# KKKSQJ/DeepLearning

Measured on AMD Instinct MI355X. Metric: images/sec, higher is better.
Workload: dtype bf16; 1 GPU; model=resnet50, global_batch=256, image_size=224, parallelism=dp1

## Files before the change

### csrc/batchnorm.hip

```cpp
#include "common.h"
#include "vec.h"

namespace dla {

__device__ __forceinline__ float bn_pre(float x, float sc, float sh) {
  return fmaf(x, sc, sh);
}

template <typename dev_t>
__global__ void bn_stats_kernel(const dev_t* __restrict__ x, float* __restrict__ sums,
                                int N, int C, int64_t HW) {
  __shared__ float smem[16];
  const int c = blockIdx.x;
  const int64_t total = (int64_t)N * HW;
  float sum = 0.f, sumsq = 0.f;
  for (int64_t m = (int64_t)blockIdx.y * blockDim.x + threadIdx.x; m < total;
       m += (int64_t)gridDim.y * blockDim.x) {
    const int64_t n = m / HW, hw = m % HW;
    const float f = to_f32(x[(n * C + c) * HW + hw]);
    sum += f;
    sumsq += f * f;
  }
  sum = block_reduce_sum(sum, smem);
  sumsq = block_reduce_sum(sumsq, smem);
  if (threadIdx.x == 0) {
    atomicAdd(&sums[c], sum);
    atomicAdd(&sums[C + c], sumsq);
  }
}

__device__ __forceinline__ void bn_finalize_channel(
    int c, float sum, float sumsq, const float* __restrict__ weight,
    const float* __restrict__ bias, float* __restrict__ mean,
    float* __restrict__ rstd, float* __restrict__ running_mean,
    float* __restrict__ running_var, float* __restrict__ scale,
    float* __restrict__ shift, float count, float eps, float momentum) {
  const float mu = sum / count;
  const float var = fmaxf(sumsq / count - mu * mu, 0.f);
  const float rs = rsqrtf(var + eps);
  mean[c] = mu;
  rstd[c] = rs;
  if (running_mean != nullptr && momentum > 0.f) {
    const float unbiased = var * count / fmaxf(count - 1.f, 1.f);
    running_mean[c] = (1.f - momentum) * running_mean[c] + momentum * mu;
    running_var[c] = (1.f - momentum) * running_var[c] + momentum * unbiased;
  }
  const float sc = weight[c] * rs;
  scale[c] = sc;
  shift[c] = bias[c] - mu * sc;
}

__global__ void bn_finalize_kernel(const float* __restrict__ sums,
                                   const float* __restrict__ weight,
                                   const float* __restrict__ bias,
                                   float* __restrict__ mean, float* __restrict__ rstd,
                                   float* __restrict__ running_mean,
                                   float* __restrict__ running_var,
                                   float* __restrict__ scale, float* __restrict__ shift,
                                   int C, float count, float eps, float momentum) {
  const int c = blockIdx.x * blockDim.x + threadIdx.x;
  if (c >= C) return;
  bn_finalize_channel(c, sums[c], sums[C + c], weight, bias, mean, rstd,
                      running_mean, running_var, scale, shift, count, eps,
                      momentum);
}

constexpr int kFinCh = 16, kFinRows = 64;

__global__ void __launch_bounds__(kFinCh * kFinRows)
bn_finalize_parts_kernel(const float* __restrict__ parts, int n_parts,
                         const float* __restrict__ weight,
                         const float* __restrict__ bias,
                         float* __restrict__ mean, float* __restrict__ rstd,
                         float* __restrict__ running_mean,
                         float* __restrict__ running_var,
                         float* __restrict__ scale, float* __restrict__ shift,
                         int C, float count, float eps, float momentum) {
  __shared__ float ls[2][kFinRows][kFinCh + 1];
  const int cl = threadIdx.x % kFinCh, rl = threadIdx.x / kFinCh;
  const int c = blockIdx.x * kFinCh + cl;
  float s = 0.f, q = 0.f;
  if (c < C) {
#pragma unroll 4
    for (int r = rl; r < n_parts; r += kFinRows) {
      const float* p = parts + (int64_t)r * 2 * C;
      s += p[c];
      q += p[C + c];
    }
  }
  ls[0][rl][cl] = s;
  ls[1][rl][cl] = q;
  __syncthreads();
  for (int h = kFinRows / 2; h > 0; h >>= 1) {
    if (rl < h) {
      ls[0][rl][cl] += ls[0][rl + h][cl];
      ls[1][rl][cl] += ls[1][rl + h][cl];
    }
    __syncthreads();
  }
  if (rl == 0 && c < C)
    bn_finalize_channel(c, ls[0][0][cl], ls[1][0][cl], weight, bias, mean,
                        rstd, running_mean, running_var, scale, shift, count,
                        eps, momentum);
}

template <typename dev_t, int V, bool RELU>
__global__ void bn_apply_kernel(const dev_t* __restrict__ x,
                                const float* __restrict__ scale,
                                const float* __restrict__ shift,
                                dev_t* __restrict__ y, int C, int64_t HW,
                                int64_t n_total) {
  const int64_t stride = (int64_t)gridDim.x * blockDim.x * V;
  for (int64_t i = ((int64_t)blockIdx.x * blockDim.x + threadIdx.x) * V;
       i < n_total; i += stride) {
    const int c = (int)((i / HW) % C);
    const float sc = scale[c], sh = shift[c];
    Vec<dev_t, V> xv = vload<dev_t, V>(x + i);
    Vec<dev_t, V> yv;
#pragma unroll
    for (int j = 0; j < V; ++j) {
      const float f = bn_pre(to_f32(xv.v[j]), sc, sh);
      yv.v[j] = from_f32<dev_t>(RELU ? fmaxf(f, 0.f) : f);
    }
    vstore<dev_t, V>(y + i, yv);
  }
}

template <typename dev_t, bool RELU>
__global__ void bn_bwd_stats_kernel(const dev_t* __restrict__ dy,
                                    const dev_t* __restrict__ x,
                                    const dev_t* __restrict__ y,
                                    const float* __restrict__ mean,
                                    const float* __restrict__ rstd,
                                    float* __restrict__ sums,
                                    int N, int C, int64_t HW) {
  __shared__ float smem[16];
  const int c = blockIdx.x;
  const float mu = mean[c], rs = rstd[c];
  const int64_t total = (int64_t)N * HW;
  float s_dy = 0.f, s_dyxh = 0.f;
  for (int64_t m = (int64_t)blockIdx.y * blockDim.x + threadIdx.x; m < total;
       m += (int64_t)gridDim.y * blockDim.x) {
    const int64_t n = m / HW, hw = m % HW;
    const int64_t idx = (n * C + c) * HW + hw;
    float g = to_f32(dy[idx]);
    if (RELU && to_f32(y[idx]) <= 0.f) g = 0.f;
    const float xh = (to_f32(x[idx]) - mu) * rs;
    s_dy += g;
    s_dyxh += g * xh;
  }
  s_dy = block_reduce_sum(s_dy, smem);
  s_dyxh = block_reduce_sum(s_dyxh, smem);
  if (threadIdx.x == 0) {
    atomicAdd(&sums[c], s_dy);
    atomicAdd(&sums[C + c], s_dyxh);
  }
}

template <typename dev_t, bool RELU>
__global__ void bn_bwd_dx_kernel(const dev_t* __restrict__ dy,
                                 const dev_t* __restrict__ x,
                                 const dev_t* __restrict__ y,
                                 const float* __restrict__ mean,
                                 const float* __restrict__ rstd,
                                 const float* __restrict__ weight,
                                 const float* __restrict__ sums,
                                 dev_t* __restrict__ dx, int C, int64_t HW,
                                 int64_t n_total, float inv_count) {
  const int64_t stride = (int64_t)gridDim.x * blockDim.x;
  for (int64_t i = (int64_t)blockIdx.x * blockDim.x + threadIdx.x; i < n_total;
       i += stride) {
    const int c = (int)((i / HW) % C);
    const float mu = mean[c], rs = rstd[c];
    float g = to_f32(dy[i]);
    if (RELU && to_f32(y[i]) <= 0.f) g = 0.f;
    const float xh = (to_f32(x[i]) - mu) * rs;
    const float m_dy = sums[c] * inv_count;
    const float m_dyxh = sums[C + c] * inv_count;
    dx[i] = from_f32<dev_t>(weight[c] * rs * (g - m_dy - xh * m_dyxh));
  }
}



inline int64_t nhwc_used_threads(int lanes_per_row, int64_t rows,
                                 int64_t target_lanes) {
  int64_t k = target_lanes / lanes_per_row;
  if (k > rows) k = rows;
  if (k < 1) k = 1;
  return (int64_t)lanes_per_row * k;
}

constexpr int kRedThreads = 256;
constexpr int kRedLanes = 32;
constexpr int kRedBlocks = 2048;
constexpr int kRedMaxParts = 512;
constexpr int kRedMinRows = 8;
constexpr int red_unroll(int tensors) { return tensors <= 2 ? 4 : 2; }

#define DLA_RED_KERNEL \
  __launch_bounds__(dla::kRedThreads) __attribute__((amdgpu_waves_per_eu(1, 4)))

struct NhwcRedTile {
  int bl, rb, chunks, parts;
};

inline NhwcRedTile nhwc_red_tile(int lanes_per_row, int64_t rows,
                                 int blocks = kRedBlocks,
                                 int max_parts = kRedMaxParts) {
  NhwcRedTile t;
  t.chunks = (lanes_per_row + kRedLanes - 1) / kRedLanes;
  t.bl = (lanes_per_row + t.chunks - 1) / t.chunks;
  t.rb = kRedThreads / t.bl;
  const int64_t per_part = (int64_t)t.rb * kRedMinRows;
  const int64_t by_rows = (rows + per_part - 1) / per_part;
  const int64_t p = std::min<int64_t>(
      std::min<int64_t>(blocks / t.chunks, max_parts), by_rows);
  t.parts = (int)std::max<int64_t>(p, 1);
  return t;
}

struct NhwcRedPos {
  int c0;
  int64_t row;
  int64_t rstride;
  bool active;
};

template <int V>
__device__ __forceinline__ NhwcRedPos nhwc_red_pos(int C, int bl, int rb) {
  const int lane = threadIdx.x % bl, rl = threadIdx.x / bl;
  const int gl = blockIdx.x * bl + lane;
  NhwcRedPos p;
  p.c0 = gl * V;
  p.row = (int64_t)blockIdx.y * rb + rl;
  p.rstride = (int64_t)gridDim.y * rb;
  p.active = rl < rb && gl < C / V;
  return p;
}

template <int U, typename L, typename A>
__device__ __forceinline__ void nhwc_red_rows(const NhwcRedPos& p,
                                              int64_t rows, L&& load, A&& add) {
  if (!p.active) return;
  using D = decltype(load(int64_t{}));
  int64_t r = p.row;
  for (; r + (U - 1) * p.rstride < rows; r += U * p.rstride) {
    D d[U];
#pragma unroll
    for (int u = 0; u < U; ++u) d[u] = load(r + u * p.rstride);
#pragma unroll
    for (int u = 0; u < U; ++u) add(r + u * p.rstride, d[u]);
  }
  for (; r < rows; r += p.rstride) add(r, load(r));
}

template <int V, int NS>
__device__ __forceinline__ void nhwc_red_tail(const float (&acc)[NS][V],
                                              float* __restrict__ slab, int C,
                                              int bl, int rb) {
  __shared__ __attribute__((aligned(16))) float ls[kRedThreads * V];
  const int W = bl * V;
  const int cbase = blockIdx.x * W;
  float* out = slab + (int64_t)blockIdx.y * NS * C;
#pragma unroll
  for (int s = 0; s < NS; ++s) {
    if (s) __syncthreads();
    if ((int)threadIdx.x < bl * rb) {
#pragma unroll
      for (int j = 0; j < V; ++j) ls[threadIdx.x * V + j] = acc[s][j];
    }
    __syncthreads();
    for (int col = threadIdx.x; col < W; col += kRedThreads) {
      if (cbase + col < C) {
        float sum = 0.f;
        for (int r = 0; r < rb; ++r) sum += ls[r * W + col];
        out[s * C + cbase + col] = sum;
      }
    }
  }
}

constexpr int kSlabCols = 32, kSlabRows = 32;

__global__ void __launch_bounds__(kSlabCols * kSlabRows)
bn_slab_reduce_kernel(const float* __restrict__ slab, int n_parts, int n_cols,
                      float* __restrict__ sums) {
  __shared__ float ls[kSlabRows][kSlabCols + 1];
  const int cl = threadIdx.x % kSlabCols, rl = threadIdx.x / kSlabCols;
  const int c = blockIdx.x * kSlabCols + cl;
  float s = 0.f;
  if (c < n_cols) {
#pragma unroll 4
    for (int r = rl; r < n_parts; r += kSlabRows)
      s += slab[(int64_t)r * n_cols + c];
  }
  ls[rl][cl] = s;
  __syncthreads();
  for (int h = kSlabRows / 2; h > 0; h >>= 1) {
    if (rl < h) ls[rl][cl] += ls[rl + h][cl];
    __syncthreads();
  }
  if (rl == 0 && c < n_cols) sums[c] = ls[0][cl];
}

template <typename dev_t, int V>
__global__ void DLA_RED_KERNEL
bn_stats_nhwc_kernel(const dev_t* __restrict__ x, float* __restrict__ slab,
                     int C, int64_t rows, int bl, int rb) {
  const NhwcRedPos p = nhwc_red_pos<V>(C, bl, rb);
  float acc[2][V];
#pragma unroll
  for (int j = 0; j < V; ++j) { acc[0][j] = 0.f; acc[1][j] = 0.f; }
  nhwc_red_rows<red_unroll(1)>(
      p, rows, [&](int64_t r) { return vload<dev_t, V>(x + r * C + p.c0); },
      [&](int64_t, const Vec<dev_t, V>& xv) {
#pragma unroll
        for (int j = 0; j < V; ++j) {
          const float f = to_f32(xv.v[j]);
          acc[0][j] += f;
          acc[1][j] += f * f;
        }
      });
  nhwc_red_tail<V, 2>(acc, slab, C, bl, rb);
}

template <typename dev_t, int V, bool RELU>
__global__ void bn_apply_nhwc_kernel(const dev_t* __restrict__ x,
                                     const float* __restrict__ scale,
                                     const float* __restrict__ shift,
                                     dev_t* __restrict__ y, int C, int64_t rows,
                                     int64_t used) {
  const int64_t t = (int64_t)blockIdx.x * blockDim.x + threadIdx.x;
  if (t >= used) return;
  const int lanes_per_row = C / V;
  const int c0 = (int)(t % lanes_per_row) * V;
  const int64_t rstride = used / lanes_per_row;
  float sc[V], sh[V];
#pragma unroll
  for (int j = 0; j < V; ++j) { sc[j] = scale[c0 + j]; sh[j] = shift[c0 + j]; }
  for (int64_t r = t / lanes_per_row; r < rows; r += rstride) {
    Vec<dev_t, V> xv = vload<dev_t, V>(x + r * C + c0);
    Vec<dev_t, V> yv;
#pragma unroll
    for (int j = 0; j < V; ++j) {
      const float f = bn_pre(to_f32(xv.v[j]), sc[j], sh[j]);
      yv.v[j] = from_f32<dev_t>(RELU ? fmaxf(f, 0.f) : f);
    }
    vstore<dev_t, V>(y + r * C + c0, yv);
  }
}

template <typename dev_t, int V, bool RELU, bool MASK_Y = false>
__global__ void DLA_RED_KERNEL
bn_bwd_stats_nhwc_kernel(const dev_t* __restrict__ dy,
                         const dev_t* __restrict__ x,
                         const dev_t* __restrict__ y,
                         const float* __restrict__ scale,
                         const float* __restrict__ shift,
                         const float* __restrict__ mean,
                         const float* __restrict__ rstd,
                         float* __restrict__ slab, int C, int64_t rows, int bl,
                         int rb) {
  const NhwcRedPos p = nhwc_red_pos<V>(C, bl, rb);
  float mu[V], rs[V], sc[V], sh[V];
  float acc[2][V];
#pragma unroll
  for (int j = 0; j < V; ++j) {
    mu[j] = p.active ? mean[p.c0 + j] : 0.f;
    rs[j] = p.active ? rstd[p.c0 + j] : 0.f;
    sc[j] = (p.active && RELU && !MASK_Y) ? scale[p.c0 + j] : 0.f;
    sh[j] = (p.active && RELU && !MASK_Y) ? shift[p.c0 + j] : 0.f;
    acc[0][j] = 0.f;
    acc[1][j] = 0.f;
  }
  struct Row {
    Vec<dev_t, V> dy, x, y;
  };
  nhwc_red_rows<red_unroll(MASK_Y ? 3 : 2)>(
      p, rows,
      [&](int64_t r) {
        const int64_t base = r * C + p.c0;
        Row d;
        d.dy = vload<dev_t, V>(dy + base);
        d.x = vload<dev_t, V>(x + base);
        if (RELU && MASK_Y) d.y = vload<dev_t, V>(y + base);
        return d;
      },
      [&](int64_t, const Row& d) {
#pragma unroll
        for (int j = 0; j < V; ++j) {
          float g = to_f32(d.dy.v[j]);
          const float xf = to_f32(d.x.v[j]);
          if (RELU && MASK_Y && to_f32(d.y.v[j]) <= 0.f) g = 0.f;
          if (RELU && !MASK_Y && !(bn_pre(xf, sc[j], sh[j]) > 0.f)) g = 0.f;
          const float xh = (xf - mu[j]) * rs[j];
          acc[0][j] += g;
          acc[1][j] += g * xh;
        }
      });
  nhwc_red_tail<V, 2>(acc, slab, C, bl, rb);
}

template <typename dev_t, int V, bool RELU, bool MASK_Y = false>
__global__ void bn_bwd_dx_nhwc_kernel(const dev_t* __restrict__ dy,
                                      const dev_t* __restrict__ x,
                                      const dev_t* __restrict__ y,
                                      const float* __restrict__ scale,
                                      const float* __restrict__ shift,
                                      const float* __restrict__ mean,
                                      const float* __restrict__ rstd,
                                      const float* __restrict__ weight,
                                      const float* __restrict__ sums,
                                      dev_t* __restrict__ dx, int C,
                                      int64_t rows, int64_t used,
                                      float inv_count) {
  const int64_t t = (int64_t)blockIdx.x * blockDim.x + threadIdx.x;
  if (t >= used) return;
  const int lanes_per_row = C / V;
  const int c0 = (int)(t % lanes_per_row) * V;
  const int64_t rstride = used / lanes_per_row;
  float mu[V], rs[V], wr[V], sc[V], sh[V], m_dy[V], m_dyxh[V];
#pragma unroll
  for (int j = 0; j < V; ++j) {
    mu[j] = mean[c0 + j];
    rs[j] = rstd[c0 + j];
    wr[j] = weight[c0 + j] * rs[j];
    sc[j] = (RELU && !MASK_Y) ? scale[c0 + j] : 0.f;
    sh[j] = (RELU && !MASK_Y) ? shift[c0 + j] : 0.f;
    m_dy[j] = sums[c0 + j] * inv_count;
    m_dyxh[j] = sums[C + c0 + j] * inv_count;
  }
  for (int64_t r = t / lanes_per_row; r < rows; r += rstride) {
    const int64_t base = r * C + c0;
    Vec<dev_t, V> dyv = vload<dev_t, V>(dy + base);
    Vec<dev_t, V> xv = vload<dev_t, V>(x + base);
    Vec<dev_t, V> yv;
    if (RELU && MASK_Y) yv = vload<dev_t, V>(y + base);
    Vec<dev_t, V> dxv;
#pragma unroll
    for (int j = 0; j < V; ++j) {
      float g = to_f32(dyv.v[j]);
      const float xf = to_f32(xv.v[j]);
      if (RELU && MASK_Y && to_f32(yv.v[j]) <= 0.f) g = 0.f;
      if (RELU && !MASK_Y && !(bn_pre(xf, sc[j], sh[j]) > 0.f)) g = 0.f;
      const float xh = (xf - mu[j]) * rs[j];
      dxv.v[j] = from_f32<dev_t>(wr[j] * (g - m_dy[j] - xh * m_dyxh[j]));
    }
    vstore<dev_t, V>(dx + r * C + c0, dxv);
  }
}

template <typename dev_t, int V, bool DUAL>
__global__ void bn_add_relu_nhwc_kernel(const dev_t* __restrict__ x,
                                        const float* __restrict__ scale,
                                        const float* __restrict__ shift,
                                        const dev_t* __restrict__ idn,
                                        const float* __restrict__ scale_d,
                                        const float* __restrict__ shift_d,
                                        dev_t* __restrict__ out, int C,
                                        int64_t rows, int64_t used) {
  const int64_t t = (int64_t)blockIdx.x * blockDim.x + threadIdx.x;
  if (t >= used) return;
  const int lanes_per_row = C / V;
  const int c0 = (int)(t % lanes_per_row) * V;
  const int64_t rstride = used / lanes_per_row;
  float sc[V], sh[V], scd[V];
#pragma unroll
  for (int j = 0; j < V; ++j) {
    sc[j] = scale[c0 + j];
    sh[j] = shift[c0 + j];
    if (DUAL) {
      scd[j] = scale_d[c0 + j];
      sh[j] += shift_d[c0 + j];
    }
  }
  for (int64_t r = t / lanes_per_row; r < rows; r += rstride) {
    const int64_t base = r * C + c0;
    Vec<dev_t, V> xv = vload<dev_t, V>(x + base);
    Vec<dev_t, V> iv = vload<dev_t, V>(idn + base);
    Vec<dev_t, V> ov;
#pragma unroll
    for (int j = 0; j < V; ++j) {
      float f = to_f32(xv.v[j]) * sc[j] + sh[j];
      f += DUAL ? to_f32(iv.v[j]) * scd[j] : to_f32(iv.v[j]);
      ov.v[j] = from_f32<dev_t>(fmaxf(f, 0.f));
    }
    vstore<dev_t, V>(out + base, ov);
  }
}

template <typename dev_t, int V, bool DUAL>
__global__ void DLA_RED_KERNEL
bn_join_bwd_stats_nhwc_kernel(
    const dev_t* __restrict__ dy, const dev_t* __restrict__ out,
    const dev_t* __restrict__ x, const float* __restrict__ mean,
    const float* __restrict__ rstd, const dev_t* __restrict__ xd,
    const float* __restrict__ mean_d, const float* __restrict__ rstd_d,
    dev_t* __restrict__ g_out, float* __restrict__ slab, int C, int64_t rows,
    int bl, int rb) {
  constexpr int NS = DUAL ? 3 : 2;
  const NhwcRedPos p = nhwc_red_pos<V>(C, bl, rb);
  float mu[V], rs[V], mud[V], rsd[V];
  float acc[NS][V];
#pragma unroll
  for (int j = 0; j < V; ++j) {
    mu[j] = p.active ? mean[p.c0 + j] : 0.f;
    rs[j] = p.active ? rstd[p.c0 + j] : 0.f;
    mud[j] = (p.active && DUAL) ? mean_d[p.c0 + j] : 0.f;
    rsd[j] = (p.active && DUAL) ? rstd_d[p.c0 + j] : 0.f;
#pragma unroll
    for (int s = 0; s < NS; ++s) acc[s][j] = 0.f;
  }
  struct Row {
    Vec<dev_t, V> dy, out, x, xd;
  };
  nhwc_red_rows<red_unroll(DUAL ? 4 : 3)>(
      p, rows,
      [&](int64_t r) {
        const int64_t base = r * C + p.c0;
        Row d;
        d.dy = vload<dev_t, V>(dy + base);
        d.out = vload<dev_t, V>(out + base);
        d.x = vload<dev_t, V>(x + base);
        if (DUAL) d.xd = vload<dev_t, V>(xd + base);
        return d;
      },
      [&](int64_t r, const Row& d) {
        Vec<dev_t, V> gv;
#pragma unroll
        for (int j = 0; j < V; ++j) {
          const bool on = to_f32(d.out.v[j]) > 0.f;
          gv.v[j] = on ? d.dy.v[j] : from_f32<dev_t>(0.f);
          const float g = on ? to_f32(d.dy.v[j]) : 0.f;
          acc[0][j] += g;
          acc[1][j] += g * ((to_f32(d.x.v[j]) - mu[j]) * rs[j]);
          if (DUAL)
            acc[NS - 1][j] += g * ((to_f32(d.xd.v[j]) - mud[j]) * rsd[j]);
        }
        vstore<dev_t, V>(g_out + r * C + p.c0, gv);
      });
  nhwc_red_tail<V, NS>(acc, slab, C, bl, rb);
}

template <typename dev_t, int V>
__global__ void bn_join_bwd_dx_dual_nhwc_kernel(
    const dev_t* __restrict__ g, const dev_t* __restrict__ x,
    const dev_t* __restrict__ xd, const float* __restrict__ mean,
    const float* __restrict__ rstd, const float* __restrict__ weight,
    const float* __restrict__ mean_d, const float* __restrict__ rstd_d,
    const float* __restrict__ weight_d, const float* __restrict__ sums,
    dev_t* __restrict__ dx, dev_t* __restrict__ dxd, int C, int64_t rows,
    int64_t used, float inv_count) {
  const int64_t t = (int64_t)blockIdx.x * blockDim.x + threadIdx.x;
  if (t >= used) return;
  const int lanes_per_row = C / V;
  const int c0 = (int)(t % lanes_per_row) * V;
  const int64_t rstride = used / lanes_per_row;
  float mu[V], rs[V], wr[V], mud[V], rsd[V], wrd[V], m_g[V], m_gxh[V],
      m_gxhd[V];
#pragma unroll
  for (int j = 0; j < V; ++j) {
    mu[j] = mean[c0 + j];
    rs[j] = rstd[c0 + j];
    wr[j] = weight[c0 + j] * rs[j];
    mud[j] = mean_d[c0 + j];
    rsd[j] = rstd_d[c0 + j];
    wrd[j] = weight_d[c0 + j] * rsd[j];
    m_g[j] = sums[c0 + j] * inv_count;
    m_gxh[j] = sums[C + c0 + j] * inv_count;
    m_gxhd[j] = sums[2 * C + c0 + j] * inv_count;
  }
  for (int64_t r = t / lanes_per_row; r < rows; r += rstride) {
    const int64_t base = r * C + c0;
    Vec<dev_t, V> gv = vload<dev_t, V>(g + base);
    Vec<dev_t, V> xv = vload<dev_t, V>(x + base);
    Vec<dev_t, V> xdv = vload<dev_t, V>(xd + base);
    Vec<dev_t, V> dxv, dxdv;
#pragma unroll
    for (int j = 0; j < V; ++j) {
      const float gg = to_f32(gv.v[j]) - m_g[j];
      const float xh = (to_f32(xv.v[j]) - mu[j]) * rs[j];
      const float xhd = (to_f32(xdv.v[j]) - mud[j]) * rsd[j];
      dxv.v[j] = from_f32<dev_t>(wr[j] * (gg - xh * m_gxh[j]));
      dxdv.v[j] = from_f32<dev_t>(wrd[j] * (gg - xhd * m_gxhd[j]));
    }
    vstore<dev_t, V>(dx + base, dxv);
    vstore<dev_t, V>(dxd + base, dxdv);
  }
}

inline bool is_nhwc(const torch::Tensor& t) {
  return t.dim() == 4 && t.is_contiguous(at::MemoryFormat::ChannelsLast) &&
         !t.is_contiguous();
}

struct BnFinalized {
  torch::Tensor mean, rstd, scale, shift;
};

inline BnFinalized bn_finalize_launch(
    const torch::Tensor& sums, const torch::Tensor& weight,
    const torch::Tensor& bias, c10::optional<torch::Tensor>& running_mean,
    c10::optional<torch::Tensor>& running_var, int C, int64_t rows,
    double momentum, double eps) {
  TORCH_CHECK(sums.is_cuda() && sums.scalar_type() == torch::kFloat &&
                  sums.is_contiguous(),
              "bn sums must be a contiguous fp32 GPU tensor");
  TORCH_CHECK((sums.dim() == 1 && sums.size(0) == 2 * C) ||
                  (sums.dim() == 2 && sums.size(0) >= 1 &&
                   sums.size(1) == 2 * C),
              "bn sums must be [2C] or [n_parts, 2C]");
  TORCH_CHECK(weight.numel() == C && bias.numel() == C,
              "bn weight/bias must have C elements");
  auto opts_f = sums.options();
  BnFinalized f{torch::empty({C}, opts_f), torch::empty({C}, opts_f),
                torch::empty({C}, opts_f), torch::empty({C}, opts_f)};
  auto w32 = weight.to(torch::kFloat).contiguous();
  auto b32 = bias.to(torch::kFloat).contiguous();
  float* rm = running_mean.has_value() ? running_mean->data_ptr<float>() : nullptr;
  float* rv = running_var.has_value() ? running_var->data_ptr<float>() : nullptr;
  const int n_parts = sums.dim() == 2 ? (int)sums.size(0) : 1;
  if (n_parts > 1) {
    hipLaunchKernelGGL(bn_finalize_parts_kernel, dim3((C + kFinCh - 1) / kFinCh),
                       dim3(kFinCh * kFinRows), 0, stream(),
                       sums.data_ptr<float>(), n_parts, w32.data_ptr<float>(),
                       b32.data_ptr<float>(), f.mean.data_ptr<float>(),
                       f.rstd.data_ptr<float>(), rm, rv,
                       f.scale.data_ptr<float>(), f.shift.data_ptr<float>(), C,
                       (float)rows, (float)eps, (float)momentum);
  } else {
    hipLaunchKernelGGL(bn_finalize_kernel, dim3((C + 255) / 256), dim3(256), 0,
                       stream(), sums.data_ptr<float>(), w32.data_ptr<float>(),
                       b32.data_ptr<float>(), f.mean.data_ptr<float>(),
                       f.rstd.data_ptr<float>(), rm, rv,
                       f.scale.data_ptr<float>(), f.shift.data_ptr<float>(), C,
                       (float)rows, (float)eps, (float)momentum);
  }
  return f;
}

inline torch::Tensor bn_param_grad(const torch::Tensor& sums, int64_t offset,
                                   int C, const torch::Tensor& weight) {
  return sums.narrow(0, offset, C).to(weight.scalar_type());
}

inline torch::Tensor bn_slab_reduce_launch(const torch::Tensor& slab) {
  const int n_parts = (int)slab.size(0), n_cols = (int)slab.size(1);
  auto sums = torch::empty({n_cols}, slab.options());
  hipLaunchKernelGGL(bn_slab_reduce_kernel,
                     dim3((n_cols + kSlabCols - 1) / kSlabCols),
                     dim3(kSlabCols * kSlabRows), 0, stream(),
                     slab.data_ptr<float>(), n_parts, n_cols,
                     sums.data_ptr<float>());
  return sums;
}

inline bool is_nhwc_rows(const torch::Tensor& t) {
  return t.dim() == 4 && t.is_contiguous(at::MemoryFormat::ChannelsLast);
}

}

std::vector<torch::Tensor> batchnorm_fwd(torch::Tensor x, torch::Tensor weight,
                                         torch::Tensor bias,
                                         c10::optional<torch::Tensor> running_mean,
                                         c10::optional<torch::Tensor> running_var,
                                         double momentum, double eps, bool relu) {
  DLA_CHECK_CUDA(x);
  TORCH_CHECK(x.dim() == 4, "batchnorm_fwd expects a 4D tensor");
  const bool nhwc = dla::is_nhwc(x);
  TORCH_CHECK(nhwc || x.is_contiguous(), "batchnorm_fwd: x must be contiguous "
              "(NCHW or channels_last)");
  const int N = (int)x.size(0), C = (int)x.size(1);
  const int64_t HW = x.size(2) * x.size(3);
  auto opts_f = x.options().dtype(torch::kFloat);
  auto sums = nhwc ? torch::Tensor() : torch::zeros({2 * C}, opts_f);
  auto mean = torch::empty({C}, opts_f);
  auto rstd = torch::empty({C}, opts_f);
  auto scale = torch::empty({C}, opts_f);
  auto shift = torch::empty({C}, opts_f);
  auto y = torch::empty_like(x);
  auto w32 = weight.to(torch::kFloat);
  auto b32 = bias.to(torch::kFloat);

  const int64_t rows = (int64_t)N * HW;
  const int ysplit = (int)std::min<int64_t>((rows + 65535) / 65536 + 1,
                                            std::max(1, 2048 / C));
  DLA_DISPATCH_FLOAT_TYPES(x.scalar_type(), "batchnorm_fwd", [&] {
    if (nhwc) {
      constexpr int VM = 16 / (int)sizeof(dev_t);
      auto stats = [&](auto vtag) {
        constexpr int V = decltype(vtag)::value;
        const auto t = dla::nhwc_red_tile(C / V, rows);
        sums = torch::empty({t.parts, 2 * C}, opts_f);
        hipLaunchKernelGGL((dla::bn_stats_nhwc_kernel<dev_t, V>),
                           dim3(t.chunks, t.parts), dim3(dla::kRedThreads), 0,
                           dla::stream(), (const dev_t*)x.data_ptr(),
                           sums.data_ptr<float>(), C, rows, t.bl, t.rb);
      };
      if (C % VM == 0) stats(std::integral_constant<int, VM>{});
      else if (C % 2 == 0) stats(std::integral_constant<int, 2>{});
      else stats(std::integral_constant<int, 1>{});
    } else {
      hipLaunchKernelGGL((dla::bn_stats_kernel<dev_t>), dim3(C, ysplit), dim3(256), 0,
                         dla::stream(), (const dev_t*)x.data_ptr(),
                         sums.data_ptr<float>(), N, C, HW);
    }
    float* rm = running_mean.has_value() ? running_mean->data_ptr<float>() : nullptr;
    float* rv = running_var.has_value() ? running_var->data_ptr<float>() : nullptr;
    if (sums.dim() == 2 && sums.size(0) > 1) {
      hipLaunchKernelGGL(dla::bn_finalize_parts_kernel,
                         dim3((C + dla::kFinCh - 1) / dla::kFinCh),
                         dim3(dla::kFinCh * dla::kFinRows), 0, dla::stream(),
                         sums.data_ptr<float>(), (int)sums.size(0),
                         w32.data_ptr<float>(), b32.data_ptr<float>(),
                         mean.data_ptr<float>(), rstd.data_ptr<float>(), rm, rv,
                         scale.data_ptr<float>(), shift.data_ptr<float>(), C,
                         (float)rows, (float)eps, (float)momentum);
    } else {
      hipLaunchKernelGGL(dla::bn_finalize_kernel, dim3((C + 255) / 256), dim3(256), 0,
                         dla::stream(), sums.data_ptr<float>(), w32.data_ptr<float>(),
                         b32.data_ptr<float>(), mean.data_ptr<float>(),
                         rstd.data_ptr<float>(), rm, rv,
                         scale.data_ptr<float>(), shift.data_ptr<float>(), C,
                         (float)rows, (float)eps, (float)momentum);
    }
    const int64_t n_total = x.numel();
    constexpr int VMAX = 16 / (int)sizeof(dev_t);
    auto launch = [&](auto vtag, auto rtag) {
      constexpr int V = decltype(vtag)::value;
      constexpr bool R = decltype(rtag)::value;
      if (nhwc) {
        const int lanes = C / V;
        const int64_t used = dla::nhwc_used_threads(lanes, rows, 524288);
        hipLaunchKernelGGL((dla::bn_apply_nhwc_kernel<dev_t, V, R>),
                           dim3((int)((used + 255) / 256)), dim3(256), 0,
                           dla::stream(), (const dev_t*)x.data_ptr(),
                           scale.data_ptr<float>(), shift.data_ptr<float>(),
                           (dev_t*)y.data_ptr(), C, rows, used);
        return;
      }
      const int grid = dla::grid_1d((n_total + V - 1) / V, 256);
      if (false) ;
      else
        hipLaunchKernelGGL((dla::bn_apply_kernel<dev_t, V, R>), dim3(grid), dim3(256),
                           0, dla::stream(), (const dev_t*)x.data_ptr(),
                           scale.data_ptr<float>(), shift.data_ptr<float>(),
                           (dev_t*)y.data_ptr(), C, HW, n_total);
    };
    const bool vec_ok = nhwc ? (C % VMAX == 0) : (HW % VMAX == 0);
    if (vec_ok) {
      if (relu) launch(std::integral_constant<int, VMAX>{}, std::true_type{});
      else launch(std::integral_constant<int, VMAX>{}, std::false_type{});
    } else {
      if (relu) launch(std::integral_constant<int, 1>{}, std::true_type{});
      else launch(std::integral_constant<int, 1>{}, std::false_type{});
    }
  });
  HIP_CHECK_ERR();
  return {y, mean, rstd, scale, shift};
}

std::vector<torch::Tensor> batchnorm_fwd_from_sums(
    torch::Tensor x, torch::Tensor weight, torch::Tensor bias,
    torch::Tensor sums, c10::optional<torch::Tensor> running_mean,
    c10::optional<torch::Tensor> running_var, double momentum, double eps,
    bool relu) {
  DLA_CHECK_CUDA(x);
  TORCH_CHECK(x.dim() == 4, "batchnorm_fwd_from_sums expects a 4D tensor");
  const bool nhwc = dla::is_nhwc(x);
  TORCH_CHECK(nhwc || x.is_contiguous(),
              "batchnorm_fwd_from_sums: x must be contiguous");
  const int N = (int)x.size(0), C = (int)x.size(1);
  const int64_t HW = x.size(2) * x.size(3);
  auto y = torch::empty_like(x);
  const int64_t rows = (int64_t)N * HW;
  auto fin = dla::bn_finalize_launch(sums, weight, bias, running_mean,
                                     running_var, C, rows, momentum, eps);
  auto& mean = fin.mean;
  auto& rstd = fin.rstd;
  auto& scale = fin.scale;
  auto& shift = fin.shift;
  DLA_DISPATCH_FLOAT_TYPES(x.scalar_type(), "batchnorm_fwd_from_sums", [&] {
    const int64_t n_total = x.numel();
    constexpr int VMAX = 16 / (int)sizeof(dev_t);
    auto launch = [&](auto vtag, auto rtag) {
      constexpr int V = decltype(vtag)::value;
      constexpr bool R = decltype(rtag)::value;
      if (nhwc) {
        const int lanes = C / V;
        const int64_t used = dla::nhwc_used_threads(lanes, rows, 524288);
        hipLaunchKernelGGL((dla::bn_apply_nhwc_kernel<dev_t, V, R>),
                           dim3((int)((used + 255) / 256)), dim3(256), 0,
                           dla::stream(), (const dev_t*)x.data_ptr(),
                           scale.data_ptr<float>(), shift.data_ptr<float>(),
                           (dev_t*)y.data_ptr(), C, rows, used);
        return;
      }
      const int grid = dla::grid_1d((n_total + V - 1) / V, 256);
      hipLaunchKernelGGL((dla::bn_apply_kernel<dev_t, V, R>), dim3(grid),
                         dim3(256), 0, dla::stream(),
                         (const dev_t*)x.data_ptr(), scale.data_ptr<float>(),
                         shift.data_ptr<float>(), (dev_t*)y.data_ptr(), C, HW,
                         n_total);
    };
    const bool vec_ok = nhwc ? (C % VMAX == 0) : (HW % VMAX == 0);
    if (vec_ok) {
      if (relu) launch(std::integral_constant<int, VMAX>{}, std::true_type{});
      else launch(std::integral_constant<int, VMAX>{}, std::false_type{});
    } else {
      if (relu) launch(std::integral_constant<int, 1>{}, std::true_type{});
      else launch(std::integral_constant<int, 1>{}, std::false_type{});
    }
  });
  HIP_CHECK_ERR();
  return {y, mean, rstd, scale, shift};
}

torch::Tensor bn_apply(torch::Tensor x, torch::Tensor scale, torch::Tensor shift,
                       bool relu) {
  DLA_CHECK_CUDA(x);
  TORCH_CHECK(x.dim() == 4, "bn_apply expects a 4D tensor");
  const bool nhwc = dla::is_nhwc(x);
  TORCH_CHECK(nhwc || x.is_contiguous(), "bn_apply: x must be contiguous");
  const int C = (int)x.size(1);
  const int64_t HW = x.size(2) * x.size(3);
  auto y = torch::empty_like(x);
  auto sc = scale.to(torch::kFloat).contiguous();
  auto sh = shift.to(torch::kFloat).contiguous();
  const int64_t n_total = x.numel();
  DLA_DISPATCH_FLOAT_TYPES(x.scalar_type(), "bn_apply", [&] {
    constexpr int VMAX = 16 / (int)sizeof(dev_t);
    auto launch = [&](auto vtag, auto rtag) {
      constexpr int V = decltype(vtag)::value;
      constexpr bool R = decltype(rtag)::value;
      if (nhwc) {
        const int64_t rows = n_total / C;
        const int lanes = C / V;
        const int64_t used = dla::nhwc_used_threads(lanes, rows, 524288);
        hipLaunchKernelGGL((dla::bn_apply_nhwc_kernel<dev_t, V, R>),
                           dim3((int)((used + 255) / 256)), dim3(256), 0,
                           dla::stream(), (const dev_t*)x.data_ptr(),
                           sc.data_ptr<float>(), sh.data_ptr<float>(),
                           (dev_t*)y.data_ptr(), C, rows, used);
        return;
      }
      const int grid = dla::grid_1d((n_total + V - 1) / V, 256);
      if (false) ;
      else
        hipLaunchKernelGGL((dla::bn_apply_kernel<dev_t, V, R>), dim3(grid), dim3(256),
                           0, dla::stream(), (const dev_t*)x.data_ptr(),
                           sc.data_ptr<float>(), sh.data_ptr<float>(),
                           (dev_t*)y.data_ptr(), C, HW, n_total);
    };
    const bool vec_ok = nhwc ? (C % VMAX == 0) : (HW % VMAX == 0);
    if (vec_ok) {
      if (relu) launch(std::integral_constant<int, VMAX>{}, std::true_type{});
      else launch(std::integral_constant<int, VMAX>{}, std::false_type{});
    } else {
      if (relu) launch(std::integral_constant<int, 1>{}, std::true_type{});
      else launch(std::integral_constant<int, 1>{}, std::false_type{});
    }
  });
  HIP_CHECK_ERR();
  return y;
}

bool bn_relu_mask_from_x(torch::Tensor x) { return dla::is_nhwc(x); }

std::vector<torch::Tensor> batchnorm_bwd_ex(
    torch::Tensor dy, torch::Tensor x, c10::optional<torch::Tensor> y,
    torch::Tensor weight, torch::Tensor mean, torch::Tensor rstd,
    c10::optional<torch::Tensor> scale, c10::optional<torch::Tensor> shift,
    bool relu) {
  DLA_CHECK_CUDA(dy); DLA_CHECK_CUDA(x);
  const bool nhwc = dla::is_nhwc(x);
  TORCH_CHECK(nhwc || x.is_contiguous(), "batchnorm_bwd: x must be contiguous");
  if (nhwc && !dla::is_nhwc(dy)) dy = dy.contiguous(at::MemoryFormat::ChannelsLast);
  if (!nhwc) dy = dy.contiguous();
  const int N = (int)x.size(0), C = (int)x.size(1);
  const int64_t HW = x.size(2) * x.size(3);
  const int64_t rows = (int64_t)N * HW;
  auto opts_f = x.options().dtype(torch::kFloat);
  auto sums = nhwc ? torch::Tensor() : torch::zeros({2 * C}, opts_f);
  auto dx = torch::empty_like(x);
  auto w32 = weight.to(torch::kFloat);
  const int ysplit = (int)std::min<int64_t>((rows + 65535) / 65536 + 1,
                                            std::max(1, 2048 / C));
  const bool mask_y = relu && y.has_value();
  if (relu && !mask_y) {
    TORCH_CHECK(bn_relu_mask_from_x(x) && scale.has_value() && shift.has_value(),
                "batchnorm_bwd: the relu mask needs y, or channels_last x "
                "with the forward's scale and shift");
    for (const auto* t : {&*scale, &*shift})
      TORCH_CHECK(t->is_cuda() && t->scalar_type() == torch::kFloat &&
                      t->is_contiguous() && t->numel() == C,
                  "batchnorm_bwd: scale/shift must be contiguous fp32 [C]");
  }
  if (mask_y)
    TORCH_CHECK(y->scalar_type() == x.scalar_type() && y->sizes() == x.sizes() &&
                    (nhwc ? dla::is_nhwc(*y) : y->is_contiguous()),
                "batchnorm_bwd: y must match x (shape, dtype, layout)");
  const float* scp = (relu && !mask_y) ? scale->data_ptr<float>() : nullptr;
  const float* shp = (relu && !mask_y) ? shift->data_ptr<float>() : nullptr;
  DLA_DISPATCH_FLOAT_TYPES(x.scalar_type(), "batchnorm_bwd", [&] {
    const dev_t* yp = mask_y ? (const dev_t*)y->data_ptr() : nullptr;
    auto with_mode = [&](auto f) {
      if (!relu) f(std::false_type{}, std::false_type{});
      else if (mask_y) f(std::true_type{}, std::true_type{});
      else f(std::true_type{}, std::false_type{});
    };
    with_mode([&](auto rtag, auto mtag) {
      constexpr bool R = decltype(rtag)::value;
      constexpr bool MY = decltype(mtag)::value;
      if (nhwc) {
        constexpr int VM = 16 / (int)sizeof(dev_t);
        auto stats = [&](auto vtag) {
          constexpr int V = decltype(vtag)::value;
          const auto t = dla::nhwc_red_tile(C / V, rows);
          auto slab = torch::empty({t.parts, 2 * C}, opts_f);
          hipLaunchKernelGGL((dla::bn_bwd_stats_nhwc_kernel<dev_t, V, R, MY>),
                             dim3(t.chunks, t.parts), dim3(dla::kRedThreads),
                             0, dla::stream(), (const dev_t*)dy.data_ptr(),
                             (const dev_t*)x.data_ptr(), yp, scp, shp,
                             mean.data_ptr<float>(), rstd.data_ptr<float>(),
                             slab.data_ptr<float>(), C, rows, t.bl, t.rb);
          sums = dla::bn_slab_reduce_launch(slab);
        };
        if (C % VM == 0) stats(std::integral_constant<int, VM>{});
        else if (C % 2 == 0) stats(std::integral_constant<int, 2>{});
        else stats(std::integral_constant<int, 1>{});
      } else if constexpr (!R || MY) {
        hipLaunchKernelGGL((dla::bn_bwd_stats_kernel<dev_t, R>), dim3(C, ysplit),
                           dim3(256), 0, dla::stream(), (const dev_t*)dy.data_ptr(),
                           (const dev_t*)x.data_ptr(), yp, mean.data_ptr<float>(),
                           rstd.data_ptr<float>(), sums.data_ptr<float>(), N, C, HW);
      }
    });

    const int64_t n_total = x.numel();
    const float inv_count = 1.f / (float)rows;
    constexpr int VMAX = 16 / (int)sizeof(dev_t);
    with_mode([&](auto rtag, auto mtag) {
      constexpr bool R = decltype(rtag)::value;
      constexpr bool MY = decltype(mtag)::value;
      if (nhwc) {
        auto dxk = [&](auto vtag) {
          constexpr int V = decltype(vtag)::value;
          const int lanes = C / V;
          const int64_t used = dla::nhwc_used_threads(lanes, rows, 524288);
          hipLaunchKernelGGL((dla::bn_bwd_dx_nhwc_kernel<dev_t, V, R, MY>),
                             dim3((int)((used + 255) / 256)), dim3(256), 0,
                             dla::stream(), (const dev_t*)dy.data_ptr(),
                             (const dev_t*)x.data_ptr(), yp, scp, shp,
                             mean.data_ptr<float>(), rstd.data_ptr<float>(),
                             w32.data_ptr<float>(), sums.data_ptr<float>(),
                             (dev_t*)dx.data_ptr(), C, rows, used, inv_count);
        };
        if (C % VMAX == 0) dxk(std::integral_constant<int, VMAX>{});
        else dxk(std::integral_constant<int, 1>{});
      } else if constexpr (!R || MY) {
        hipLaunchKernelGGL((dla::bn_bwd_dx_kernel<dev_t, R>), dim3(dla::grid_1d(n_total, 256)),
                           dim3(256), 0, dla::stream(), (const dev_t*)dy.data_ptr(),
                           (const dev_t*)x.data_ptr(), yp, mean.data_ptr<float>(),
                           rstd.data_ptr<float>(), w32.data_ptr<float>(),
                           sums.data_ptr<float>(), (dev_t*)dx.data_ptr(), C, HW,
                           n_total, inv_count);
      }
    });
  });
  HIP_CHECK_ERR();
  return {dx, dla::bn_param_grad(sums, C, C, weight),
          dla::bn_param_grad(sums, 0, C, weight)};
}

std::vector<torch::Tensor> batchnorm_bwd(torch::Tensor dy, torch::Tensor x,
                                         c10::optional<torch::Tensor> y,
                                         torch::Tensor weight, torch::Tensor mean,
                                         torch::Tensor rstd, bool relu) {
  TORCH_CHECK(!relu || y.has_value(), "batchnorm_bwd: relu mask needs y");
  return batchnorm_bwd_ex(dy, x, relu ? y : c10::nullopt, weight, mean, rstd,
                          c10::nullopt, c10::nullopt, relu);
}

namespace dla {

inline void join_check(const torch::Tensor& x, const torch::Tensor& other,
                       const char* what) {
  TORCH_CHECK(other.is_cuda() && other.scalar_type() == x.scalar_type() &&
                  other.sizes() == x.sizes() && is_nhwc_rows(other),
              "bn join: ", what, " must match x (shape, dtype, channels_last)");
}

inline int join_vec(const torch::Tensor& x) {
  const int vmax = 16 / (int)x.element_size();
  TORCH_CHECK(x.size(1) % vmax == 0,
              "bn join: C must be a multiple of ", vmax);
  return vmax;
}

}

std::vector<torch::Tensor> bn_add_relu_fwd_from_sums(
    torch::Tensor x, torch::Tensor weight, torch::Tensor bias,
    torch::Tensor sums, c10::optional<torch::Tensor> running_mean,
    c10::optional<torch::Tensor> running_var, double momentum, double eps,
    torch::Tensor identity) {
  DLA_CHECK_CUDA(x);
  TORCH_CHECK(dla::is_nhwc_rows(x), "bn_add_relu: x must be channels_last");
  dla::join_check(x, identity, "identity");
  dla::join_vec(x);
  const int C = (int)x.size(1);
  const int64_t rows = x.numel() / C;
  auto fin = dla::bn_finalize_launch(sums, weight, bias, running_mean,
                                     running_var, C, rows, momentum, eps);
  auto out = torch::empty_like(x);
  DLA_DISPATCH_FLOAT_TYPES(x.scalar_type(), "bn_add_relu_fwd_from_sums", [&] {
    constexpr int V = 16 / (int)sizeof(dev_t);
    const int64_t used = dla::nhwc_used_threads(C / V, rows, 524288);
    hipLaunchKernelGGL((dla::bn_add_relu_nhwc_kernel<dev_t, V, false>),
                       dim3((int)((used + 255) / 256)), dim3(256), 0,
                       dla::stream(), (const dev_t*)x.data_ptr(),
                       fin.scale.data_ptr<float>(), fin.shift.data_ptr<float>(),
                       (const dev_t*)identity.data_ptr(), nullptr, nullptr,
                       (dev_t*)out.data_ptr(), C, rows, used);
  });
  HIP_CHECK_ERR();
  return {out, fin.mean, fin.rstd};
}

std::vector<torch::Tensor> bn_add_relu_dual_fwd_from_sums(
    torch::Tensor x, torch::Tensor weight, torch::Tensor bias,
    torch::Tensor sums, c10::optional<torch::Tensor> running_mean,
    c10::optional<torch::Tensor> running_var, double momentum, double eps,
    torch::Tensor xd, torch::Tensor weight_d, torch::Tensor bias_d,
    torch::Tensor sums_d, c10::optional<torch::Tensor> running_mean_d,
    c10::optional<torch::Tensor> running_var_d, double momentum_d,
    double eps_d) {
  DLA_CHECK_CUDA(x);
  TORCH_CHECK(dla::is_nhwc_rows(x), "bn_add_relu_dual: x must be channels_last");
  dla::join_check(x, xd, "xd");
  dla::join_vec(x);
  const int C = (int)x.size(1);
  const int64_t rows = x.numel() / C;
  auto fin = dla::bn_finalize_launch(sums, weight, bias, running_mean,
                                     running_var, C, rows, momentum, eps);
  auto fd = dla::bn_finalize_launch(sums_d, weight_d, bias_d, running_mean_d,
                                    running_var_d, C, rows, momentum_d, eps_d);
  auto out = torch::empty_like(x);
  DLA_DISPATCH_FLOAT_TYPES(x.scalar_type(), "bn_add_relu_dual_fwd_from_sums", [&] {
    constexpr int V = 16 / (int)sizeof(dev_t);
    const int64_t used = dla::nhwc_used_threads(C / V, rows, 524288);
    hipLaunchKernelGGL((dla::bn_add_relu_nhwc_kernel<dev_t, V, true>),
                       dim3((int)((used + 255) / 256)), dim3(256), 0,
                       dla::stream(), (const dev_t*)x.data_ptr(),
                       fin.scale.data_ptr<float>(), fin.shift.data_ptr<float>(),
                       (const dev_t*)xd.data_ptr(), fd.scale.data_ptr<float>(),
                       fd.shift.data_ptr<float>(), (dev_t*)out.data_ptr(), C,
                       rows, used);
  });
  HIP_CHECK_ERR();
  return {out, fin.mean, fin.rstd, fd.mean, fd.rstd};
}

std::vector<torch::Tensor> bn_add_relu_bwd(torch::Tensor dy, torch::Tensor out,
                                           torch::Tensor x, torch::Tensor weight,
                                           torch::Tensor mean,
                                           torch::Tensor rstd) {
  DLA_CHECK_CUDA(x);
  TORCH_CHECK(dla::is_nhwc_rows(x), "bn_add_relu_bwd: x must be channels_last");
  dla::join_check(x, out, "out");
  if (!dla::is_nhwc_rows(dy)) dy = dy.contiguous(at::MemoryFormat::ChannelsLast);
  dla::join_check(x, dy, "dy");
  dla::join_vec(x);
  const int C = (int)x.size(1);
  const int64_t rows = x.numel() / C;
  TORCH_CHECK(mean.numel() == C && rstd.numel() == C && weight.numel() == C,
              "bn_add_relu_bwd: per-channel tensors must have C elements");
  torch::Tensor sums;
  auto g = torch::empty_like(x);
  auto dx = torch::empty_like(x);
  auto w32 = weight.to(torch::kFloat).contiguous();
  DLA_DISPATCH_FLOAT_TYPES(x.scalar_type(), "bn_add_relu_bwd", [&] {
    constexpr int V = 16 / (int)sizeof(dev_t);
    const int lanes = C / V;
    const auto t = dla::nhwc_red_tile(lanes, rows);
    auto slab = torch::empty({t.parts, 2 * C},
                             x.options().dtype(torch::kFloat));
    hipLaunchKernelGGL((dla::bn_join_bwd_stats_nhwc_kernel<dev_t, V, false>),
                       dim3(t.chunks, t.parts), dim3(dla::kRedThreads), 0,
                       dla::stream(),
                       (const dev_t*)dy.data_ptr(), (const dev_t*)out.data_ptr(),
                       (const dev_t*)x.data_ptr(), mean.data_ptr<float>(),
                       rstd.data_ptr<float>(), nullptr, nullptr, nullptr,
                       (dev_t*)g.data_ptr(), slab.data_ptr<float>(), C, rows,
                       t.bl, t.rb);
    sums = dla::bn_slab_reduce_launch(slab);
    const int64_t used = dla::nhwc_used_threads(lanes, rows, 524288);
    hipLaunchKernelGGL((dla::bn_bwd_dx_nhwc_kernel<dev_t, V, false>),
                       dim3((int)((used + 255) / 256)), dim3(256), 0,
                       dla::stream(), (const dev_t*)g.data_ptr(),
                       (const dev_t*)x.data_ptr(), nullptr, nullptr, nullptr,
                       mean.data_ptr<float>(), rstd.data_ptr<float>(),
                       w32.data_ptr<float>(), sums.data_ptr<float>(),
                       (dev_t*)dx.data_ptr(), C, rows, used,
                       1.f / (float)rows);
  });
  HIP_CHECK_ERR();
  return {g, dx, dla::bn_param_grad(sums, C, C, weight),
          dla::bn_param_grad(sums, 0, C, weight)};
}

std::vector<torch::Tensor> bn_add_relu_dual_bwd(
    torch::Tensor dy, torch::Tensor out, torch::Tensor x, torch::Tensor weight,
    torch::Tensor mean, torch::Tensor rstd, torch::Tensor xd,
    torch::Tensor weight_d, torch::Tensor mean_d, torch::Tensor rstd_d) {
  DLA_CHECK_CUDA(x);
  TORCH_CHECK(dla::is_nhwc_rows(x), "bn_add_relu_dual_bwd: x must be channels_last");
  dla::join_check(x, out, "out");
  dla::join_check(x, xd, "xd");
  if (!dla::is_nhwc_rows(dy)) dy = dy.contiguous(at::MemoryFormat::ChannelsLast);
  dla::join_check(x, dy, "dy");
  dla::join_vec(x);
  const int C = (int)x.size(1);
  const int64_t rows = x.numel() / C;
  TORCH_CHECK(mean.numel() == C && rstd.numel() == C && weight.numel() == C &&
                  mean_d.numel() == C && rstd_d.numel() == C &&
                  weight_d.numel() == C,
              "bn_add_relu_dual_bwd: per-channel tensors must have C elements");
  torch::Tensor sums;
  auto g = torch::empty_like(x);
  auto dx = torch::empty_like(x);
  auto dxd = torch::empty_like(x);
  auto w32 = weight.to(torch::kFloat).contiguous();
  auto wd32 = weight_d.to(torch::kFloat).contiguous();
  DLA_DISPATCH_FLOAT_TYPES(x.scalar_type(), "bn_add_relu_dual_bwd", [&] {
    constexpr int V = 16 / (int)sizeof(dev_t);
    const int lanes = C / V;
    const auto t = dla::nhwc_red_tile(lanes, rows);
    auto slab = torch::empty({t.parts, 3 * C},
                             x.options().dtype(torch::kFloat));
    hipLaunchKernelGGL((dla::bn_join_bwd_stats_nhwc_kernel<dev_t, V, true>),
                       dim3(t.chunks, t.parts), dim3(dla::kRedThreads), 0,
                       dla::stream(),
                       (const dev_t*)dy.data_ptr(), (const dev_t*)out.data_ptr(),
                       (const dev_t*)x.data_ptr(), mean.data_ptr<float>(),
                       rstd.data_ptr<float>(), (const dev_t*)xd.data_ptr(),
                       mean_d.data_ptr<float>(), rstd_d.data_ptr<float>(),
                       (dev_t*)g.data_ptr(), slab.data_ptr<float>(), C, rows,
                       t.bl, t.rb);
    sums = dla::bn_slab_reduce_launch(slab);
    const int64_t used = dla::nhwc_used_threads(lanes, rows, 524288);
    hipLaunchKernelGGL((dla::bn_join_bwd_dx_dual_nhwc_kernel<dev_t, V>),
                       dim3((int)((used + 255) / 256)), dim3(256), 0,
                       dla::stream(), (const dev_t*)g.data_ptr(),
                       (const dev_t*)x.data_ptr(), (const dev_t*)xd.data_ptr(),
                       mean.data_ptr<float>(), rstd.data_ptr<float>(),
                       w32.data_ptr<float>(), mean_d.data_ptr<float>(),
                       rstd_d.data_ptr<float>(), wd32.data_ptr<float>(),
                       sums.data_ptr<float>(), (dev_t*)dx.data_ptr(),
                       (dev_t*)dxd.data_ptr(), C, rows, used,
                       1.f / (float)rows);
  });
  HIP_CHECK_ERR();
  auto dbias = dla::bn_param_grad(sums, 0, C, weight);
  return {dx, dxd, dla::bn_param_grad(sums, C, C, weight), dbias,
          dla::bn_param_grad(sums, 2 * C, C, weight_d),
          dbias.to(weight_d.scalar_type()).clone()};
}

namespace dla {

constexpr int kPoolRun = 8;

template <typename dev_t, int V>
__global__ void __launch_bounds__(256)
bn_relu_maxpool_fwd_nhwc_kernel(const dev_t* __restrict__ x,
                                const float* __restrict__ scale,
                                const float* __restrict__ shift,
                                dev_t* __restrict__ out,
                                uint8_t* __restrict__ slots, int C, int H,
                                int W, int OH, int OW, int runs_per_img) {
  const int n = blockIdx.x / runs_per_img;
  const int oh0 = (blockIdx.x % runs_per_img) * kPoolRun;
  const int oh1 = min(oh0 + kPoolRun, OH);
  const int lanes = C / V;
  const int items = (oh1 - oh0) * OW * lanes;
  const dev_t* xn = x + (int64_t)n * H * W * C;
  const int64_t obase = ((int64_t)n * OH + oh0) * OW * C;
  for (int i = threadIdx.x; i < items; i += blockDim.x) {
    const int c0 = (i % lanes) * V;
    const int p = i / lanes;
    const int ow = p % OW, oh = oh0 + p / OW;
    float sc[V], sh[V], best[V];
    int slot[V];
#pragma unroll
    for (int j = 0; j < V; ++j) {
      sc[j] = scale[c0 + j];
      sh[j] = shift[c0 + j];
      best[j] = -INFINITY;
      slot[j] = 4;
    }
#pragma unroll
    for (int kh = 0; kh < 3; ++kh) {
      const int ih = 2 * oh - 1 + kh;
      if (ih < 0 || ih >= H) continue;
#pragma unroll
      for (int kw = 0; kw < 3; ++kw) {
        const int iw = 2 * ow - 1 + kw;
        if (iw < 0 || iw >= W) continue;
        Vec<dev_t, V> xv =
            vload<dev_t, V>(xn + ((int64_t)ih * W + iw) * C + c0);
#pragma unroll
        for (int j = 0; j < V; ++j) {
          const float f = bn_pre(to_f32(xv.v[j]), sc[j], sh[j]);
          const float y = to_f32(from_f32<dev_t>(fmaxf(f, 0.f)));
          if (y > best[j]) {
            best[j] = y;
            slot[j] = kh * 3 + kw;
          }
        }
      }
    }
    Vec<dev_t, V> ov;
    Vec<uint8_t, V> sv;
#pragma unroll
    for (int j = 0; j < V; ++j) {
      ov.v[j] = from_f32<dev_t>(best[j]);
      sv.v[j] = (uint8_t)slot[j];
    }
    const int64_t o = obase + (int64_t)p * C + c0;
    vstore<dev_t, V>(out + o, ov);
    vstore<uint8_t, V>(slots + o, sv);
  }
}

template <typename dev_t, int V>
__device__ __forceinline__ void stem_pool_grad(
    const dev_t* __restrict__ dpool, const uint8_t* __restrict__ slots,
    const Vec<dev_t, V>& xv, const float* sc, const float* sh, int n, int h,
    int w, int c0, int C, int OH, int OW, float* g) {
#pragma unroll
  for (int j = 0; j < V; ++j) g[j] = 0.f;
  const int oh_hi = min((h + 1) >> 1, OH - 1);
  const int ow_hi = min((w + 1) >> 1, OW - 1);
  for (int oh = h >> 1; oh <= oh_hi; ++oh) {
    const int kh = h - 2 * oh + 1;
    for (int ow = w >> 1; ow <= ow_hi; ++ow) {
      const int want = kh * 3 + (w - 2 * ow + 1);
      const int64_t o = (((int64_t)n * OH + oh) * OW + ow) * C + c0;
      Vec<uint8_t, V> sv = vload<uint8_t, V>(slots + o);
      Vec<dev_t, V> dv = vload<dev_t, V>(dpool + o);
#pragma unroll
      for (int j = 0; j < V; ++j)
        if ((int)sv.v[j] == want) g[j] += to_f32(dv.v[j]);
    }
  }
#pragma unroll
  for (int j = 0; j < V; ++j)
    if (!(bn_pre(to_f32(xv.v[j]), sc[j], sh[j]) > 0.f)) g[j] = 0.f;
}

constexpr int kStemRedBlocks = 1024;

template <typename dev_t, int V>
__global__ void __launch_bounds__(kRedThreads)
bn_relu_maxpool_bwd_stats_nhwc_kernel(
    const dev_t* __restrict__ dpool, const uint8_t* __restrict__ slots,
    const dev_t* __restrict__ x, const float* __restrict__ scale,
    const float* __restrict__ shift, const float* __restrict__ mean,
    const float* __restrict__ rstd, float* __restrict__ slab, int C, int H,
    int W, int OH, int OW, int64_t rows, int bl, int rb) {
  const NhwcRedPos p = nhwc_red_pos<V>(C, bl, rb);
  float mu[V], rs[V], sc[V], sh[V];
  float acc[2][V];
#pragma unroll
  for (int j = 0; j < V; ++j) {
    mu[j] = p.active ? mean[p.c0 + j] : 0.f;
    rs[j] = p.active ? rstd[p.c0 + j] : 0.f;
    sc[j] = p.active ? scale[p.c0 + j] : 0.f;
    sh[j] = p.active ? shift[p.c0 + j] : 0.f;
    acc[0][j] = 0.f;
    acc[1][j] = 0.f;
  }
  nhwc_red_rows<1>(
      p, rows, [&](int64_t r) { return vload<dev_t, V>(x + r * C + p.c0); },
      [&](int64_t r, const Vec<dev_t, V>& xv) {
        const uint32_t r32 = (uint32_t)r;
        const uint32_t q = r32 / (uint32_t)W;
        const int w = (int)(r32 - q * (uint32_t)W);
        const int n = (int)(q / (uint32_t)H);
        const int h = (int)(q - (uint32_t)n * (uint32_t)H);
        float g[V];
        stem_pool_grad<dev_t, V>(dpool, slots, xv, sc, sh, n, h, w, p.c0, C,
                                 OH, OW, g);
#pragma unroll
        for (int j = 0; j < V; ++j) {
          const float xh = (to_f32(xv.v[j]) - mu[j]) * rs[j];
          acc[0][j] += g[j];
          acc[1][j] += g[j] * xh;
        }
      });
  nhwc_red_tail<V, 2>(acc, slab, C, bl, rb);
}

template <typename dev_t, int V>
__global__ void bn_relu_maxpool_bwd_dx_nhwc_kernel(
    const dev_t* __restrict__ dpool, const uint8_t* __restrict__ slots,
    const dev_t* __restrict__ x, const float* __restrict__ scale,
    const float* __restrict__ shift, const float* __restrict__ mean,
    const float* __restrict__ rstd, const float* __restrict__ weight,
    const float* __restrict__ sums, dev_t* __restrict__ dx, int C, int H,
    int W, int OH, int OW, int64_t rows, int64_t used, float inv_count) {
  const int64_t t = (int64_t)blockIdx.x * blockDim.x + threadIdx.x;
  if (t >= used) return;
  const int lanes_per_row = C / V;
  const int c0 = (int)(t % lanes_per_row) * V;
  const int64_t rstride = used / lanes_per_row;
  float mu[V], rs[V], wr[V], sc[V], sh[V], m_g[V], m_gxh[V], g[V];
#pragma unroll
  for (int j = 0; j < V; ++j) {
    mu[j] = mean[c0 + j];
    rs[j] = rstd[c0 + j];
    wr[j] = weight[c0 + j] * rs[j];
    sc[j] = scale[c0 + j];
    sh[j] = shift[c0 + j];
    m_g[j] = sums[c0 + j] * inv_count;
    m_gxh[j] = sums[C + c0 + j] * inv_count;
  }
  for (int64_t r = t / lanes_per_row; r < rows; r += rstride) {
    const uint32_t r32 = (uint32_t)r;
    const uint32_t q = r32 / (uint32_t)W;
    const int w = (int)(r32 - q * (uint32_t)W);
    const int n = (int)(q / (uint32_t)H);
    const int h = (int)(q - (uint32_t)n * (uint32_t)H);
    Vec<dev_t, V> xv = vload<dev_t, V>(x + r * C + c0);
    stem_pool_grad<dev_t, V>(dpool, slots, xv, sc, sh, n, h, w, c0, C, OH, OW,
                             g);
    Vec<dev_t, V> dxv;
#pragma unroll
    for (int j = 0; j < V; ++j) {
      const float xh = (to_f32(xv.v[j]) - mu[j]) * rs[j];
      dxv.v[j] = from_f32<dev_t>(wr[j] * (g[j] - m_g[j] - xh * m_gxh[j]));
    }
    vstore<dev_t, V>(dx + r * C + c0, dxv);
  }
}

inline void stem_check(const torch::Tensor& x, const char* fn) {
  TORCH_CHECK(x.is_cuda() && x.dim() == 4 && is_nhwc_rows(x), fn,
              ": x must be a channels_last 4D GPU tensor");
  const int vmax = 16 / (int)x.element_size();
  TORCH_CHECK(x.size(1) % vmax == 0, fn, ": C must be a multiple of ", vmax);
  TORCH_CHECK(x.numel() > 0 && x.numel() / x.size(1) < (int64_t(1) << 31),
              fn, ": N*H*W must be in [1, 2^31)");
}

}

std::vector<torch::Tensor> bn_relu_maxpool_fwd(
    torch::Tensor x, torch::Tensor weight, torch::Tensor bias,
    c10::optional<torch::Tensor> running_mean,
    c10::optional<torch::Tensor> running_var, double momentum, double eps) {
  dla::stem_check(x, "bn_relu_maxpool_fwd");
  const int N = (int)x.size(0), C = (int)x.size(1);
  const int H = (int)x.size(2), W = (int)x.size(3);
  const int OH = (H - 1) / 2 + 1, OW = (W - 1) / 2 + 1;
  const int64_t rows = (int64_t)N * H * W;
  auto out_opts = x.options().memory_format(at::MemoryFormat::ChannelsLast);
  auto pooled = torch::empty({N, C, OH, OW}, out_opts);
  auto slots = torch::empty({N, C, OH, OW}, out_opts.dtype(torch::kByte));
  const int runs = (OH + dla::kPoolRun - 1) / dla::kPoolRun;
  TORCH_CHECK((int64_t)N * runs < (int64_t(1) << 31),
              "bn_relu_maxpool_fwd: too many blocks");
  dla::BnFinalized fin;
  DLA_DISPATCH_FLOAT_TYPES(x.scalar_type(), "bn_relu_maxpool_fwd", [&] {
    constexpr int V = 16 / (int)sizeof(dev_t);
    const auto t = dla::nhwc_red_tile(C / V, rows);
    auto sums = torch::empty({t.parts, 2 * C},
                             x.options().dtype(torch::kFloat));
    hipLaunchKernelGGL((dla::bn_stats_nhwc_kernel<dev_t, V>),
                       dim3(t.chunks, t.parts), dim3(dla::kRedThreads), 0,
                       dla::stream(), (const dev_t*)x.data_ptr(),
                       sums.data_ptr<float>(), C, rows, t.bl, t.rb);
    fin = dla::bn_finalize_launch(sums, weight, bias, running_mean,
                                  running_var, C, rows, momentum, eps);
    hipLaunchKernelGGL((dla::bn_relu_maxpool_fwd_nhwc_kernel<dev_t, V>),
                       dim3(N * runs), dim3(256), 0, dla::stream(),
                       (const dev_t*)x.data_ptr(), fin.scale.data_ptr<float>(),
                       fin.shift.data_ptr<float>(), (dev_t*)pooled.data_ptr(),
                       slots.data_ptr<uint8_t>(), C, H, W, OH, OW, runs);
  });
  HIP_CHECK_ERR();
  return {pooled, slots, fin.mean, fin.rstd, fin.scale, fin.shift};
}

std::vector<torch::Tensor> bn_relu_maxpool_bwd(
    torch::Tensor dpool, torch::Tensor x, torch::Tensor slots,
    torch::Tensor weight, torch::Tensor mean, torch::Tensor rstd,
    torch::Tensor scale, torch::Tensor shift) {
  dla::stem_check(x, "bn_relu_maxpool_bwd");
  const int N = (int)x.size(0), C = (int)x.size(1);
  const int H = (int)x.size(2), W = (int)x.size(3);
  const int OH = (H - 1) / 2 + 1, OW = (W - 1) / 2 + 1;
  const int64_t rows = (int64_t)N * H * W;
  DLA_CHECK_CUDA(dpool);
  if (!dla::is_nhwc_rows(dpool))
    dpool = dpool.contiguous(at::MemoryFormat::ChannelsLast);
  const std::vector<int64_t> pshape{N, C, OH, OW};
  TORCH_CHECK(dpool.scalar_type() == x.scalar_type() &&
                  dpool.sizes() == at::IntArrayRef(pshape),
              "bn_relu_maxpool_bwd: dpool must be [N, C, OH, OW] of x's dtype");
  TORCH_CHECK(slots.is_cuda() && slots.scalar_type() == torch::kByte &&
                  slots.sizes() == at::IntArrayRef(pshape) &&
                  dla::is_nhwc_rows(slots),
              "bn_relu_maxpool_bwd: slots must be channels_last uint8 "
              "[N, C, OH, OW]");
  for (const auto* t : {&mean, &rstd, &scale, &shift})
    TORCH_CHECK(t->is_cuda() && t->scalar_type() == torch::kFloat &&
                    t->is_contiguous() && t->numel() == C,
                "bn_relu_maxpool_bwd: per-channel tensors must be contiguous "
                "fp32 [C]");
  TORCH_CHECK(weight.numel() == C, "bn_relu_maxpool_bwd: weight must be [C]");
  torch::Tensor sums;
  auto dx = torch::empty_like(x);
  auto w32 = weight.to(torch::kFloat).contiguous();
  DLA_DISPATCH_FLOAT_TYPES(x.scalar_type(), "bn_relu_maxpool_bwd", [&] {
    constexpr int V = 16 / (int)sizeof(dev_t);
    const int lanes = C / V;
    const auto t = dla::nhwc_red_tile(lanes, rows, dla::kStemRedBlocks,
                                      dla::kStemRedBlocks);
    auto slab = torch::empty({t.parts, 2 * C},
                             x.options().dtype(torch::kFloat));
    hipLaunchKernelGGL((dla::bn_relu_maxpool_bwd_stats_nhwc_kernel<dev_t, V>),
                       dim3(t.chunks, t.parts), dim3(dla::kRedThreads), 0,
                       dla::stream(), (const dev_t*)dpool.data_ptr(),
                       slots.data_ptr<uint8_t>(), (const dev_t*)x.data_ptr(),
                       scale.data_ptr<float>(), shift.data_ptr<float>(),
                       mean.data_ptr<float>(), rstd.data_ptr<float>(),
                       slab.data_ptr<float>(), C, H, W, OH, OW, rows, t.bl,
                       t.rb);
    sums = dla::bn_slab_reduce_launch(slab);
    const int64_t used = dla::nhwc_used_threads(lanes, rows, 524288);
    hipLaunchKernelGGL((dla::bn_relu_maxpool_bwd_dx_nhwc_kernel<dev_t, V>),
                       dim3((int)((used + 255) / 256)), dim3(256), 0,
                       dla::stream(), (const dev_t*)dpool.data_ptr(),
                       slots.data_ptr<uint8_t>(), (const dev_t*)x.data_ptr(),
                       scale.data_ptr<float>(), shift.data_ptr<float>(),
                       mean.data_ptr<float>(), rstd.data_ptr<float>(),
                       w32.data_ptr<float>(), sums.data_ptr<float>(),
                       (dev_t*)dx.data_ptr(), C, H, W, OH, OW, rows, used,
                       1.f / (float)rows);
  });
  HIP_CHECK_ERR();
  return {dx, dla::bn_param_grad(sums, C, C, weight),
          dla::bn_param_grad(sums, 0, C, weight)};
}
```

### csrc/bindings.cpp

```cpp
#include <torch/extension.h>

std::vector<torch::Tensor> layernorm_fwd(torch::Tensor x, torch::Tensor w,
                                         torch::Tensor b, double eps);
std::vector<torch::Tensor> layernorm_bwd(torch::Tensor dy, torch::Tensor x,
                                         torch::Tensor w, torch::Tensor mean,
                                         torch::Tensor rstd);
torch::Tensor gelu_fwd(torch::Tensor x);
torch::Tensor gelu_bwd(torch::Tensor dy, torch::Tensor x);
torch::Tensor silu_fwd(torch::Tensor x);
torch::Tensor silu_bwd(torch::Tensor dy, torch::Tensor x);
torch::Tensor add_relu_fwd(torch::Tensor a, torch::Tensor b);
torch::Tensor relu_mask_bwd(torch::Tensor dy, torch::Tensor y);
std::vector<torch::Tensor> batchnorm_fwd(torch::Tensor x, torch::Tensor weight,
                                         torch::Tensor bias,
                                         c10::optional<torch::Tensor> running_mean,
                                         c10::optional<torch::Tensor> running_var,
                                         double momentum, double eps, bool relu);
torch::Tensor bn_apply(torch::Tensor x, torch::Tensor scale, torch::Tensor shift,
                       bool relu);
std::vector<torch::Tensor> batchnorm_bwd(torch::Tensor dy, torch::Tensor x,
                                         c10::optional<torch::Tensor> y,
                                         torch::Tensor weight, torch::Tensor mean,
                                         torch::Tensor rstd, bool relu);
bool bn_relu_mask_from_x(torch::Tensor x);
std::vector<torch::Tensor> batchnorm_bwd_ex(
    torch::Tensor dy, torch::Tensor x, c10::optional<torch::Tensor> y,
    torch::Tensor weight, torch::Tensor mean, torch::Tensor rstd,
    c10::optional<torch::Tensor> scale, c10::optional<torch::Tensor> shift,
    bool relu);
std::vector<torch::Tensor> bn_relu_maxpool_fwd(
    torch::Tensor x, torch::Tensor weight, torch::Tensor bias,
    c10::optional<torch::Tensor> running_mean,
    c10::optional<torch::Tensor> running_var, double momentum, double eps);
std::vector<torch::Tensor> bn_relu_maxpool_bwd(
    torch::Tensor dpool, torch::Tensor x, torch::Tensor slots,
    torch::Tensor weight, torch::Tensor mean, torch::Tensor rstd,
    torch::Tensor scale, torch::Tensor shift);
std::vector<torch::Tensor> batchnorm_fwd_from_sums(
    torch::Tensor x, torch::Tensor weight, torch::Tensor bias,
    torch::Tensor sums, c10::optional<torch::Tensor> running_mean,
    c10::optional<torch::Tensor> running_var, double momentum, double eps,
    bool relu);
std::vector<torch::Tensor> bn_add_relu_fwd_from_sums(
    torch::Tensor x, torch::Tensor weight, torch::Tensor bias,
    torch::Tensor sums, c10::optional<torch::Tensor> running_mean,
    c10::optional<torch::Tensor> running_var, double momentum, double eps,
    torch::Tensor identity);
std::vector<torch::Tensor> bn_add_relu_dual_fwd_from_sums(
    torch::Tensor x, torch::Tensor weight, torch::Tensor bias,
    torch::Tensor sums, c10::optional<torch::Tensor> running_mean,
    c10::optional<torch::Tensor> running_var, double momentum, double eps,
    torch::Tensor xd, torch::Tensor weight_d, torch::Tensor bias_d,
    torch::Tensor sums_d, c10::optional<torch::Tensor> running_mean_d,
    c10::optional<torch::Tensor> running_var_d, double momentum_d,
    double eps_d);
std::vector<torch::Tensor> bn_add_relu_bwd(torch::Tensor dy, torch::Tensor out,
                                           torch::Tensor x, torch::Tensor weight,
                                           torch::Tensor mean,
                                           torch::Tensor rstd);
std::vector<torch::Tensor> bn_add_relu_dual_bwd(
    torch::Tensor dy, torch::Tensor out, torch::Tensor x, torch::Tensor weight,
    torch::Tensor mean, torch::Tensor rstd, torch::Tensor xd,
    torch::Tensor weight_d, torch::Tensor mean_d, torch::Tensor rstd_d);
std::vector<torch::Tensor> conv1x1_fwd(torch::Tensor a, torch::Tensor b,
                                       c10::optional<torch::Tensor> bias,
                                       c10::optional<torch::Tensor> scale,
                                       c10::optional<torch::Tensor> shift,
                                       c10::optional<torch::Tensor> residual,
                                       bool relu, bool want_stats);
torch::Tensor conv1x1_wgrad(torch::Tensor dy, torch::Tensor x);
std::vector<torch::Tensor> conv3x3_fwd(torch::Tensor a, torch::Tensor w9,
                                       int64_t imgH, int64_t imgW,
                                       c10::optional<torch::Tensor> bias,
                                       c10::optional<torch::Tensor> scale,
                                       c10::optional<torch::Tensor> shift,
                                       c10::optional<torch::Tensor> residual,
                                       bool relu, bool want_stats);
torch::Tensor conv3x3_wgrad(torch::Tensor dy, torch::Tensor x, int64_t imgH,
                            int64_t imgW);
torch::Tensor dwconv_fwd(torch::Tensor x, torch::Tensor weight,
                         c10::optional<torch::Tensor> bias, int64_t stride);
torch::Tensor dwconv_dgrad(torch::Tensor dy, torch::Tensor weight, int64_t H,
                           int64_t W, int64_t stride);
std::vector<torch::Tensor> dwconv_wgrad(torch::Tensor dy, torch::Tensor x,
                                        int64_t K, int64_t stride,
                                        bool out_f32);
torch::Tensor transpose2d(torch::Tensor src);
torch::Tensor stride2_gather(torch::Tensor x);
torch::Tensor stride2_scatter(torch::Tensor dy, int64_t IH, int64_t IW);
std::vector<torch::Tensor> softmax_ce_fwd(torch::Tensor logits,
                                          c10::optional<torch::Tensor> target,
                                          c10::optional<torch::Tensor> soft_target,
                                          double smoothing, int64_t ignore_index);
torch::Tensor softmax_ce_bwd(torch::Tensor logits,
                             c10::optional<torch::Tensor> target,
                             c10::optional<torch::Tensor> soft_target,
                             torch::Tensor lse, double smoothing,
                             int64_t ignore_index, torch::Tensor grad_out,
                             torch::Tensor stats);
torch::Tensor focal_loss_fwd(torch::Tensor logits, torch::Tensor targets,
                             double alpha, double gamma);
torch::Tensor focal_loss_bwd(torch::Tensor dloss, torch::Tensor logits,
                             torch::Tensor targets, double alpha, double gamma);
torch::Tensor box_iou_gpu(torch::Tensor a, torch::Tensor b, bool giou);
torch::Tensor nms_gpu(torch::Tensor boxes_sorted, double iou_threshold);
torch::Tensor roialign_fwd(torch::Tensor input, torch::Tensor rois, int64_t PH,
                           int64_t PW, double spatial_scale,
                           int64_t sampling_ratio, bool aligned);
torch::Tensor roialign_bwd(torch::Tensor grad_out, torch::Tensor rois, int64_t N,
                           int64_t C, int64_t H, int64_t W, double spatial_scale,
                           int64_t sampling_ratio, bool aligned);
std::vector<torch::Tensor> attn_fwd(torch::Tensor qkv, int64_t num_heads,
                                    double scale,
                                    c10::optional<torch::Tensor> bias,
                                    c10::optional<torch::Tensor> mask,
                                    bool save_p, bool save_stats);
std::vector<torch::Tensor> attn_bwd(torch::Tensor qkv, torch::Tensor dout,
                                    torch::Tensor stats, torch::Tensor drow,
                                    int64_t num_heads, double scale);
std::vector<torch::Tensor> attn_fwd_cosine(torch::Tensor qkv, int64_t num_heads,
                              torch::Tensor logit_scale,
                              c10::optional<torch::Tensor> bias,
                              c10::optional<torch::Tensor> mask, bool save_p);
torch::Tensor mfma_probe(torch::Tensor A, torch::Tensor B);
torch::Tensor my_add(torch::Tensor a, torch::Tensor b);
std::vector<torch::Tensor> cocoeval_match_image(
    torch::Tensor det_boxes, torch::Tensor det_scores, torch::Tensor gt_boxes,
    torch::Tensor gt_crowd, torch::Tensor iou_thrs, int64_t max_dets,
    c10::optional<torch::Tensor> gt_extra_ignore);
torch::Tensor window_partition_fwd(torch::Tensor x, int64_t ws, int64_t shift);
torch::Tensor window_partition_bwd(torch::Tensor grad, int64_t B, int64_t H,
                                   int64_t W, int64_t ws, int64_t shift);
torch::Tensor window_merge_fwd(torch::Tensor windows, int64_t B, int64_t H,
                               int64_t W, int64_t ws, int64_t shift);
torch::Tensor window_merge_bwd(torch::Tensor grad, int64_t ws, int64_t shift);

PYBIND11_MODULE(TORCH_EXTENSION_NAME, m) {
  m.doc() = "deeplearning_amd gfx950 HIP kernels";
  m.def("layernorm_fwd", &layernorm_fwd);
  m.def("layernorm_bwd", &layernorm_bwd);
  m.def("gelu_fwd", &gelu_fwd);
  m.def("gelu_bwd", &gelu_bwd);
  m.def("silu_fwd", &silu_fwd);
  m.def("silu_bwd", &silu_bwd);
  m.def("add_relu_fwd", &add_relu_fwd);
  m.def("relu_mask_bwd", &relu_mask_bwd);
  m.def("batchnorm_fwd", &batchnorm_fwd);
  m.def("batchnorm_fwd_from_sums", &batchnorm_fwd_from_sums);
  m.def("bn_apply", &bn_apply);
  m.def("batchnorm_bwd", &batchnorm_bwd);
  m.def("batchnorm_bwd_ex", &batchnorm_bwd_ex);
  m.def("bn_relu_mask_from_x", &bn_relu_mask_from_x);
  m.def("bn_relu_maxpool_fwd", &bn_relu_maxpool_fwd);
  m.def("bn_relu_maxpool_bwd", &bn_relu_maxpool_bwd);
  m.def("bn_add_relu_fwd_from_sums", &bn_add_relu_fwd_from_sums);
  m.def("bn_add_relu_dual_fwd_from_sums", &bn_add_relu_dual_fwd_from_sums);
  m.def("bn_add_relu_bwd", &bn_add_relu_bwd);
  m.def("bn_add_relu_dual_bwd", &bn_add_relu_dual_bwd);
  m.def("conv1x1_fwd", &conv1x1_fwd, py::arg("a"), py::arg("b"),
        py::arg("bias") = py::none(), py::arg("scale") = py::none(),
        py::arg("shift") = py::none(), py::arg("residual") = py::none(),
        py::arg("relu") = false, py::arg("want_stats") = false);
  m.def("conv1x1_wgrad", &conv1x1_wgrad);
  m.def("conv3x3_fwd", &conv3x3_fwd, py::arg("a"), py::arg("w9"),
        py::arg("imgH"), py::arg("imgW"), py::arg("bias") = py::none(),
        py::arg("scale") = py::none(), py::arg("shift") = py::none(),
        py::arg("residual") = py::none(), py::arg("relu") = false,
        py::arg("want_stats") = false);
  m.def("conv3x3_wgrad", &conv3x3_wgrad);
  m.def("dwconv_fwd", &dwconv_fwd, py::arg("x"), py::arg("weight"),
        py::arg("bias") = py::none(), py::arg("stride") = 1);
  m.def("dwconv_dgrad", &dwconv_dgrad);
  m.def("dwconv_wgrad", &dwconv_wgrad);
  m.def("transpose2d", &transpose2d);
  m.def("stride2_gather", &stride2_gather);
  m.def("stride2_scatter", &stride2_scatter);
  m.def("softmax_ce_fwd", &softmax_ce_fwd);
  m.def("softmax_ce_bwd", &softmax_ce_bwd);
  m.def("focal_loss_fwd", &focal_loss_fwd);
  m.def("focal_loss_bwd", &focal_loss_bwd);
  m.def("box_iou", &box_iou_gpu);
  m.def("nms", &nms_gpu);
  m.def("roialign_fwd", &roialign_fwd);
  m.def("roialign_bwd", &roialign_bwd);
  m.def("attn_fwd", &attn_fwd, py::arg("qkv"), py::arg("num_heads"),
        py::arg("scale"), py::arg("bias") = py::none(),
        py::arg("mask") = py::none(), py::arg("save_p") = false,
        py::arg("save_stats") = false);
  m.def("attn_bwd", &attn_bwd);
  m.def("attn_fwd_cosine", &attn_fwd_cosine, py::arg("qkv"),
        py::arg("num_heads"), py::arg("logit_scale"),
        py::arg("bias") = py::none(), py::arg("mask") = py::none(),
        py::arg("save_p") = false);
  m.def("mfma_probe", &mfma_probe);
  m.def("cocoeval_match_image", &cocoeval_match_image, py::arg("det_boxes"),
        py::arg("det_scores"), py::arg("gt_boxes"), py::arg("gt_crowd"),
        py::arg("iou_thrs"), py::arg("max_dets"),
        py::arg("gt_extra_ignore") = py::none());
  m.def("my_add", &my_add);
  m.def("window_partition_fwd", &window_partition_fwd);
  m.def("window_partition_bwd", &window_partition_bwd);
  m.def("window_merge_fwd", &window_merge_fwd);
  m.def("window_merge_bwd", &window_merge_bwd);
}
```

### csrc/common.h

```cpp
#pragma once

#include <hip/hip_runtime.h>
#include <hip/hip_bf16.h>
#include <hip/hip_fp16.h>
#include <torch/extension.h>
#include <ATen/hip/HIPContext.h>

#define DLA_WAVE 64
#define DLA_CHECK_CUDA(x) TORCH_CHECK((x).is_cuda(), #x " must be a GPU tensor")
#define DLA_CHECK_CONTIG(x) TORCH_CHECK((x).is_contiguous(), #x " must be contiguous")
#define DLA_CHECK_INPUT(x) DLA_CHECK_CUDA(x); DLA_CHECK_CONTIG(x)
#define DLA_CHECK_DENSE(x)                                                     \
  DLA_CHECK_CUDA(x);                                                           \
  TORCH_CHECK((x).is_contiguous() ||                                           \
                  ((x).dim() == 4 &&                                           \
                   (x).is_contiguous(at::MemoryFormat::ChannelsLast)),         \
              #x " must be dense (contiguous or channels_last)")

#define HIP_CHECK_ERR()                                                        \
  do {                                                                         \
    hipError_t e = hipGetLastError();                                          \
    TORCH_CHECK(e == hipSuccess, "HIP kernel launch failed: ",                 \
                hipGetErrorString(e));                                         \
  } while (0)

namespace dla {

constexpr int kMaxGrid = 2048;

inline int grid_1d(int64_t n, int block) {
  int64_t g = (n + block - 1) / block;
  return (int)std::min<int64_t>(g, kMaxGrid);
}

inline hipStream_t stream() { return at::hip::getCurrentHIPStream().stream(); }

template <typename T> struct AccT { using type = float; };

__device__ __forceinline__ float to_f32(float x) { return x; }
__device__ __forceinline__ float to_f32(__hip_bfloat16 x) { return __bfloat162float(x); }
__device__ __forceinline__ float to_f32(__half x) { return __half2float(x); }

template <typename T> __device__ __forceinline__ T from_f32(float x);
template <> __device__ __forceinline__ float from_f32<float>(float x) { return x; }
template <> __device__ __forceinline__ __hip_bfloat16 from_f32<__hip_bfloat16>(float x) {
  return __float2bfloat16(x);
}
template <> __device__ __forceinline__ __half from_f32<__half>(float x) {
  return __float2half(x);
}

template <typename scalar_t> struct DevT { using type = scalar_t; };
template <> struct DevT<at::BFloat16> { using type = __hip_bfloat16; };
template <> struct DevT<at::Half> { using type = __half; };

__device__ __forceinline__ float wave_reduce_sum(float v) {
#pragma unroll
  for (int off = 32; off > 0; off >>= 1) v += __shfl_xor(v, off, 64);
  return v;
}

__device__ __forceinline__ float wave_reduce_max(float v) {
#pragma unroll
  for (int off = 32; off > 0; off >>= 1) v = fmaxf(v, __shfl_xor(v, off, 64));
  return v;
}

__device__ __forceinline__ float block_reduce_sum(float v, float* smem) {
  const int lane = threadIdx.x & 63;
  const int wid = threadIdx.x >> 6;
  v = wave_reduce_sum(v);
  if (lane == 0) smem[wid] = v;
  __syncthreads();
  const int nw = (blockDim.x + 63) >> 6;
  float r = (threadIdx.x < nw) ? smem[threadIdx.x] : 0.0f;
  r = wave_reduce_sum(r);
  if (threadIdx.x == 0) smem[0] = r;
  __syncthreads();
  r = smem[0];
  __syncthreads();
  return r;
}

__device__ __forceinline__ float block_reduce_max(float v, float* smem) {
  const int lane = threadIdx.x & 63;
  const int wid = threadIdx.x >> 6;
  v = wave_reduce_max(v);
  if (lane == 0) smem[wid] = v;
  __syncthreads();
  const int nw = (blockDim.x + 63) >> 6;
  float r = (threadIdx.x < nw) ? smem[threadIdx.x] : -INFINITY;
  r = wave_reduce_max(r);
  if (threadIdx.x == 0) smem[0] = r;
  __syncthreads();
  r = smem[0];
  __syncthreads();
  return r;
}

}

#define DLA_DISPATCH_FLOAT_TYPES(TYPE, NAME, ...)                              \
  [&] {                                                                        \
    switch (TYPE) {                                                            \
      case at::ScalarType::Float: {                                            \
        using scalar_t = float; using dev_t = float;                           \
        return __VA_ARGS__();                                                  \
      }                                                                        \
      case at::ScalarType::BFloat16: {                                         \
        using scalar_t = at::BFloat16; using dev_t = __hip_bfloat16;           \
        return __VA_ARGS__();                                                  \
      }                                                                        \
      case at::ScalarType::Half: {                                             \
        using scalar_t = at::Half; using dev_t = __half;                       \
        return __VA_ARGS__();                                                  \
      }                                                                        \
      default:                                                                 \
        TORCH_CHECK(false, #NAME ": unsupported dtype ", TYPE);                \
    }                                                                          \
  }()
```

### csrc/conv1x1.hip

```cpp
#include <cstdlib>

#include "common.h"
#include "vec.h"

namespace dla {

using bf16x8 = __attribute__((ext_vector_type(8))) short;
using f32x4 = __attribute__((ext_vector_type(4))) float;

using bf16 = __hip_bfloat16;

__device__ __forceinline__ void glds16(const bf16* gsrc, bf16* lds_dst) {
  __builtin_amdgcn_global_load_lds(
      (const __attribute__((address_space(1))) unsigned int*)gsrc,
      (__attribute__((address_space(3))) unsigned int*)lds_dst, 16, 0, 0);
}

template <int BN, bool STATS, int BK = 64, int TAPS = 1, int RING = 0>
__global__ __launch_bounds__((BN == 256) ? 512 : 256) void conv1x1_nt_kernel(
    const bf16* __restrict__ A, const bf16* __restrict__ B,
    bf16* __restrict__ C, const bf16* __restrict__ residual,
    const float* __restrict__ bias,
    const float* __restrict__ scale,
    const float* __restrict__ shift,
    float* __restrict__ sums,
    int64_t M, int K, int N, bool relu, int imgH = 0, int imgW = 0) {
  constexpr int BM = 128;
  constexpr int NWAVES = (BN == 256) ? 8 : 4;
  constexpr int WAVES_M = (BN == 64) ? 4 : 2;
  constexpr int WAVES_N = NWAVES / WAVES_M;
  constexpr int WM = BM / WAVES_M;
  constexpr int WN = BN / WAVES_N;
  constexpr int MFR = WM / 16, NFR = WN / 16;
  constexpr int ROWB = BK * 2;

  const int lane = threadIdx.x & 63;
  const int wave = threadIdx.x >> 6;
  const int64_t m0 = (int64_t)blockIdx.y * BM;
  const int n0 = blockIdx.x * BN;

  extern __shared__ __attribute__((aligned(16))) char lds_raw[];
  bf16* const lds16 = (bf16*)lds_raw;
  const int nk = K / BK;
  const bool direct_a = false;
  const int nbuf = RING > 0 ? RING : (nk > 1 ? 2 : 1);
  auto a_lds = [&](int buf) { return lds16 + buf * (BM * BK); };
  auto b_lds = [&](int buf) {
    return (direct_a ? lds16 : lds16 + nbuf * BM * BK) + buf * (BN * BK);
  };

  constexpr int RPP = 1024 / (BK * 2);
  constexpr int LPR = 64 / RPP;
  auto swz = [&](int row) {
    return BK == 64 ? (row & 7) << 4 : ((row ^ (row >> 2)) & 3) << 4;
  };
  const int CinK = K / TAPS;
  auto stage = [&](int buf, int kt) {
    const int k0b_all = kt * BK * 2;
    const int tap = TAPS == 1 ? 0 : (kt * BK) / CinK;
    const int k0b = TAPS == 1 ? k0b_all : ((kt * BK) % CinK) * 2;
    const int ky = tap / 3 - 1, kx = tap % 3 - 1;
    if (!direct_a) {
#pragma unroll
      for (int pp = 0; pp < (BM / RPP) / NWAVES; ++pp) {
        const int p = wave + pp * NWAVES;
        const int row = p * RPP + lane / LPR;
        const int b = (lane % LPR) * 16;
        if (TAPS == 1) {
          const int64_t rg = m0 + row < M ? m0 + row : M - 1;
          const char* src = (const char*)A + rg * (int64_t)CinK * 2 + k0b +
                            (b ^ swz(row));
          glds16((const bf16*)src, a_lds(buf) + p * 512);
        } else {
          const int64_t m = m0 + row < M ? m0 + row : M - 1;
          const int64_t img = m / ((int64_t)imgH * imgW);
          const int r = (int)(m - img * imgH * imgW);
          const int oh = r / imgW, ow = r % imgW;
          const int ih = oh + ky, iw = ow + kx;
          const bool valid = (unsigned)ih < (unsigned)imgH &&
                             (unsigned)iw < (unsigned)imgW &&
                             m0 + row < M;
          Vec<bf16, 8> v;
          if (valid) {
            const int64_t in_row = (img * imgH + ih) * imgW + iw;
            v = *(const Vec<bf16, 8>*)((const char*)A +
                                       in_row * (int64_t)CinK * 2 + k0b +
                                       (b ^ swz(row)));
          } else {
#pragma unroll
            for (int j = 0; j < 8; ++j) v.v[j] = from_f32<bf16>(0.f);
          }
          vstore<bf16, 8>(a_lds(buf) + p * 512 + (lane % LPR) * 8 +
                              (lane / LPR) * (BK),
                          v);
        }
      }
    }
#pragma unroll
    for (int pp = 0; pp < (BN / RPP) / NWAVES; ++pp) {
      const int p = wave + pp * NWAVES;
      const int row = p * RPP + lane / LPR;
      const int b = (lane % LPR) * 16;
      const char* src = (const char*)B + (int64_t)(n0 + row) * K * 2 +
                        k0b_all + (b ^ swz(row));
      glds16((const bf16*)src, b_lds(buf) + p * 512);
    }
  };

  const int wm_off = (wave / WAVES_N) * WM;
  const int wn_off = (wave % WAVES_N) * WN;

  f32x4 acc[MFR][NFR];
#pragma unroll
  for (int mi = 0; mi < MFR; ++mi)
#pragma unroll
    for (int ni = 0; ni < NFR; ++ni) acc[mi][ni] = f32x4{0.f, 0.f, 0.f, 0.f};

  auto compute_step = [&](const char* ab, const char* bb) {
#pragma unroll
    for (int ks = 0; ks < BK / 32; ++ks) {
      const int kbyte = (ks * 32 + (lane >> 4) * 8) * 2;
      bf16x8 af[MFR], bfr[NFR];
#pragma unroll
      for (int mi = 0; mi < MFR; ++mi) {
        const int row = wm_off + mi * 16 + (lane & 15);
        if (direct_a) {
          const int64_t rg = m0 + row < M ? m0 + row : M - 1;
          af[mi] = *(const bf16x8*)((const char*)A + rg * (int64_t)K * 2 +
                                    kbyte);
        } else {
          af[mi] =
              *(const bf16x8*)(ab + row * ROWB + (kbyte ^ swz(row)));
        }
      }
#pragma unroll
      for (int ni = 0; ni < NFR; ++ni) {
        const int row = wn_off + ni * 16 + (lane & 15);
        bfr[ni] = *(const bf16x8*)(bb + row * ROWB + (kbyte ^ swz(row)));
      }
#pragma unroll
      for (int mi = 0; mi < MFR; ++mi)
#pragma unroll
        for (int ni = 0; ni < NFR; ++ni)
          acc[mi][ni] = __builtin_amdgcn_mfma_f32_16x16x32_bf16(
              af[mi], bfr[ni], acc[mi][ni], 0, 0, 0);
    }
  };

  if constexpr (RING == 0) {
    stage(0, 0);
    __syncthreads();
    int cur = 0;
    for (int kt = 0; kt < nk; ++kt) {
      if (kt + 1 < nk) stage(cur ^ 1, kt + 1);
      compute_step((const char*)a_lds(cur), (const char*)b_lds(cur));
      __syncthreads();
      cur ^= 1;
    }
  } else {
    static_assert(RING == 4, "ring depth fixed at 4 (stage 2 ahead)");
    constexpr int G = ((BM / RPP) / NWAVES) + ((BN / RPP) / NWAVES);
    stage(0, 0);
    if (nk > 1) stage(1, 1);
    for (int kt = 0; kt < nk; ++kt) {
      if (kt + 2 < nk) {
        stage((kt + 2) % RING, kt + 2);
        asm volatile("s_waitcnt vmcnt(%0)" ::"n"(2 * G) : "memory");
      } else if (kt + 1 < nk) {
        asm volatile("s_waitcnt vmcnt(%0)" ::"n"(G) : "memory");
      } else {
        asm volatile("s_waitcnt vmcnt(0)" ::: "memory");
      }
      asm volatile("s_waitcnt lgkmcnt(0)" ::: "memory");
      __builtin_amdgcn_s_barrier();
      compute_step((const char*)a_lds(kt % RING),
                   (const char*)b_lds(kt % RING));
    }
    __syncthreads();
  }

  if (STATS) {
    float* sbuf = (float*)lds_raw;
    const int wm = wave / WAVES_N;
#pragma unroll
    for (int ni = 0; ni < NFR; ++ni) {
      const int c = wn_off + ni * 16 + (lane & 15);
      const float b = bias != nullptr ? bias[n0 + c] : 0.f;
      float s = 0.f, q = 0.f;
#pragma unroll
      for (int mi = 0; mi < MFR; ++mi)
#pragma unroll
        for (int r = 0; r < 4; ++r) {
          const int64_t gm = m0 + wm_off + mi * 16 + (lane >> 4) * 4 + r;
          if (gm < M) {
            const float raw = acc[mi][ni][r] + b;
            s += raw;
            q += raw * raw;
          }
        }
      s += __shfl_xor(s, 16, 64);
      s += __shfl_xor(s, 32, 64);
      q += __shfl_xor(q, 16, 64);
      q += __shfl_xor(q, 32, 64);
      if (lane < 16) {
        sbuf[wm * (2 * BN) + c] = s;
        sbuf[wm * (2 * BN) + BN + c] = q;
      }
    }
    __syncthreads();
    float* slab = sums + (int64_t)blockIdx.y * (2 * N);
    for (int t = threadIdx.x; t < 2 * BN; t += NWAVES * 64) {
      float tot = 0.f;
#pragma unroll
      for (int wmi = 0; wmi < WAVES_M; ++wmi) tot += sbuf[wmi * (2 * BN) + t];
      const int c = t < BN ? t : t - BN;
      slab[(t < BN ? 0 : N) + n0 + c] = tot;
    }
    __syncthreads();
  }

  constexpr int EROW = WN + 8;
  constexpr int EPC = (MFR >= 4) ? 2 : 1;
  constexpr int MFC = MFR / EPC;
  bf16* ep = (bf16*)lds_raw + wave * (MFC * 16) * EROW;
  const int c0 = (lane & 7) * 8;
  const int ng0 = n0 + wn_off + c0;
  const bool has_ss = scale != nullptr;
  float sc[8], sh[8];
  if (has_ss) {
#pragma unroll
    for (int j = 0; j < 8; ++j) { sc[j] = scale[ng0 + j]; sh[j] = shift[ng0 + j]; }
  }
  float bcol[NFR];
#pragma unroll
  for (int ni = 0; ni < NFR; ++ni)
    bcol[ni] = bias != nullptr ? bias[n0 + wn_off + ni * 16 + (lane & 15)]
                               : 0.f;
#pragma unroll
  for (int h = 0; h < EPC; ++h) {
#pragma unroll
    for (int mc = 0; mc < MFC; ++mc) {
      const int mi = h * MFC + mc;
#pragma unroll
      for (int ni = 0; ni < NFR; ++ni)
#pragma unroll
        for (int r = 0; r < 4; ++r) {
          const int row = mc * 16 + (lane >> 4) * 4 + r;
          const int col = ni * 16 + (lane & 15);
          ep[row * EROW + col] = from_f32<bf16>(acc[mi][ni][r] + bcol[ni]);
        }
    }
    __syncthreads();
#pragma unroll
    for (int i = 0; i < (MFC * 16) / 8; ++i) {
      const int r = (lane >> 3) + 8 * i;
      const int64_t gm = m0 + wm_off + h * (MFC * 16) + r;
      if (gm < M) {
        Vec<bf16, 8> v = vload<bf16, 8>(ep + r * EROW + c0);
        Vec<bf16, 8> res;
        if (residual != nullptr)
          res = vload<bf16, 8>(residual + gm * N + ng0);
        Vec<bf16, 8> out;
#pragma unroll
        for (int j = 0; j < 8; ++j) {
          float y = to_f32(v.v[j]);
          if (has_ss) y = y * sc[j] + sh[j];
          if (residual != nullptr) y += to_f32(res.v[j]);
          if (relu) y = fmaxf(y, 0.f);
          out.v[j] = from_f32<bf16>(y);
        }
        vstore<bf16, 8>(C + gm * N + ng0, out);
      }
    }
    if (h + 1 < EPC) __syncthreads();
  }
}

template <int BCO, int BCI, int TAPS = 1>
__global__ __launch_bounds__((BCO * BCI >= 8192) ? 512 : 256) void conv1x1_wgrad_kernel(
    const bf16* __restrict__ dy,
    const bf16* __restrict__ x,
    float* __restrict__ dW,
    int64_t M, int K, int N, int64_t chunk, int imgH = 0, int imgW = 0) {
  constexpr int KM = 64;
  constexpr int TR = 72;
  constexpr int NW = (BCO * BCI >= 8192) ? 8 : 4;
  constexpr int WGC = (BCO >= 128 && BCI == 64) ? 4 : 2;
  constexpr int WGI = NW / WGC;
  constexpr int WCO = BCO / WGC;
  constexpr int WCI = BCI / WGI;
  constexpr int FCO = WCO / 16, FCI = WCI / 16;
  const int lane = threadIdx.x & 63;
  const int wave = threadIdx.x >> 6;
  const int n0 = blockIdx.x * BCO;
  const int k0 = blockIdx.y * BCI;
  const int64_t m_begin = (int64_t)blockIdx.z * chunk;
  const int64_t m_end = m_begin + chunk < M ? m_begin + chunk : M;

  extern __shared__ __attribute__((aligned(16))) char lds_raw[];
  bf16* const lds16 = (bf16*)lds_raw;
  auto dyt = [&](int buf) { return lds16 + buf * (BCO * TR); };
  auto xt = [&](int buf) { return lds16 + 2 * BCO * TR + buf * (BCI * TR); };

  auto stage_t = [&](bf16* lds, const bf16* g, int stride_elems, int ch0g,
                     int64_t mt, int tap, auto bch_tag) {
    constexpr int BCH = decltype(bch_tag)::value;
#pragma unroll
    for (int it = 0; it < (KM * BCH / 8) / (NW * 64); ++it) {
      const int idx = (int)threadIdx.x + it * (NW * 64);
      const int m = idx / (BCH / 8);
      const int ch = (idx % (BCH / 8)) * 8;
      Vec<bf16, 8> v;
      bool valid = mt + m < m_end;
      int64_t src_row = mt + m;
      if (TAPS != 1 && tap >= 0 && valid) {
        const int ky = tap / 3 - 1, kx = tap % 3 - 1;
        const int64_t img = src_row / ((int64_t)imgH * imgW);
        const int r = (int)(src_row - img * imgH * imgW);
        const int oh = r / imgW, ow = r % imgW;
        const int ih = oh + ky, iw = ow + kx;
        valid = (unsigned)ih < (unsigned)imgH &&
                (unsigned)iw < (unsigned)imgW;
        src_row = (img * imgH + ih) * imgW + iw;
      }
      if (valid) {
        v = vload<bf16, 8>(g + src_row * (int64_t)stride_elems + ch0g + ch);
      } else {
#pragma unroll
        for (int j = 0; j < 8; ++j) v.v[j] = from_f32<bf16>(0.f);
      }
#pragma unroll
      for (int j = 0; j < 8; ++j) {
        const int c = ch + j;
        lds[c * TR + (m ^ (((c >> 3) & 7) << 3))] = v.v[j];
      }
    }
  };

  constexpr int KXN = (TAPS == 1) ? 1 : 3;
  f32x4 acc[KXN][FCO][FCI];
#pragma unroll
  for (int kx = 0; kx < KXN; ++kx)
#pragma unroll
    for (int mi = 0; mi < FCO; ++mi)
#pragma unroll
      for (int ni = 0; ni < FCI; ++ni)
        acc[kx][mi][ni] = f32x4{0.f, 0.f, 0.f, 0.f};

  const int wco = (wave / WGI) * WCO;
  const int wci = (wave % WGI) * WCI;

  const int CinK = K / TAPS;
  const int ky_idx = TAPS == 1 ? 0 : k0 / CinK;
  const int ci0 = TAPS == 1 ? k0 : k0 % CinK;
  auto tap_of = [&](int kx) { return TAPS == 1 ? -1 : ky_idx * 3 + kx; };

  stage_t(dyt(0), dy, N, n0, m_begin, -1, std::integral_constant<int, BCO>{});
  stage_t(xt(0), x, CinK, ci0, m_begin, tap_of(0),
          std::integral_constant<int, BCI>{});
  __syncthreads();
  int xbuf = 0, dybuf = 0;
  for (int64_t mt = m_begin; mt < m_end; mt += KM) {
#pragma unroll
    for (int kx = 0; kx < KXN; ++kx) {
      if (kx + 1 < KXN) {
        stage_t(xt(xbuf ^ 1), x, CinK, ci0, mt, tap_of(kx + 1),
                std::integral_constant<int, BCI>{});
      } else if (mt + KM < m_end) {
        stage_t(xt(xbuf ^ 1), x, CinK, ci0, mt + KM, tap_of(0),
                std::integral_constant<int, BCI>{});
        stage_t(dyt(dybuf ^ 1), dy, N, n0, mt + KM, -1,
                std::integral_constant<int, BCO>{});
      }
#pragma unroll
      for (int ks = 0; ks < 2; ++ks) {
        const int mm = ks * 32 + (lane >> 4) * 8;
        bf16x8 af[FCO], bfr[FCI];
#pragma unroll
        for (int mi = 0; mi < FCO; ++mi) {
          const int c = wco + mi * 16 + (lane & 15);
          af[mi] = *(const bf16x8*)(dyt(dybuf) + c * TR +
                                    (mm ^ (((c >> 3) & 7) << 3)));
        }
#pragma unroll
        for (int ni = 0; ni < FCI; ++ni) {
          const int c = wci + ni * 16 + (lane & 15);
          bfr[ni] = *(const bf16x8*)(xt(xbuf) + c * TR +
                                     (mm ^ (((c >> 3) & 7) << 3)));
        }
#pragma unroll
        for (int mi = 0; mi < FCO; ++mi)
#pragma unroll
          for (int ni = 0; ni < FCI; ++ni)
            acc[kx][mi][ni] = __builtin_amdgcn_mfma_f32_16x16x32_bf16(
                af[mi], bfr[ni], acc[kx][mi][ni], 0, 0, 0);
      }
      __syncthreads();
      xbuf ^= 1;
    }
    dybuf ^= 1;
  }

#pragma unroll
  for (int kx = 0; kx < KXN; ++kx)
#pragma unroll
    for (int mi = 0; mi < FCO; ++mi)
#pragma unroll
      for (int ni = 0; ni < FCI; ++ni)
#pragma unroll
        for (int r = 0; r < 4; ++r) {
          const int co = n0 + wco + mi * 16 + (lane >> 4) * 4 + r;
          const int ci_local = wci + ni * 16 + (lane & 15);
          const int kg = TAPS == 1
              ? k0 + ci_local
              : (ky_idx * 3 + kx) * CinK + ci0 + ci_local;
          atomicAdd(&dW[(int64_t)co * K + kg], acc[kx][mi][ni][r]);
        }
}

using bf16x4 = __attribute__((ext_vector_type(4))) short;

template <int BC>
__device__ __forceinline__ int wg_swz(int row) {
  static_assert(BC == 64 || BC == 128, "128 B or 256 B rows");
  if (BC == 64) return (((row >> 1) & 1) << 2) | (((row >> 3) & 1) << 1);
  return ((row & 3) << 2) | (((row >> 3) & 1) << 1);
}

template <int BCO, int BCI>
__global__ __launch_bounds__(256) void conv1x1_wgrad2_kernel(
    const bf16* __restrict__ dy,
    const bf16* __restrict__ x,
    float* __restrict__ out,
    int64_t M, int K, int N, int64_t chunk, int tiles, int total) {
  constexpr int KM = 64;
  constexpr int WGC = 2, WGI = 2;
  constexpr int WCO = BCO / WGC, WCI = BCI / WGI;
  constexpr int FCO = WCO / 16, FCI = WCI / 16;
  constexpr int IMG = KM * (BCO + BCI) * 2;
  const int lane = threadIdx.x & 63;
  const int wave = threadIdx.x >> 6;

  const int per = (int)gridDim.x >> 3;
  const int logical = ((int)blockIdx.x & 7) * per + ((int)blockIdx.x >> 3);
  if (logical >= total) return;
  const int split = logical / tiles;
  const int tile = logical - split * tiles;
  const int n0 = (tile % (N / BCO)) * BCO;
  const int k0 = (tile / (N / BCO)) * BCI;
  const int64_t m_begin = (int64_t)split * chunk;
  const int64_t m_end = m_begin + chunk < M ? m_begin + chunk : M;
  const int nfull = (int)((m_end - m_begin) / KM);
  const int nsteps = (int)((m_end - m_begin + KM - 1) / KM);

  extern __shared__ __attribute__((aligned(16))) char lds_raw[];
  auto dy_img = [&](int buf) { return lds_raw + buf * IMG; };
  auto x_img = [&](int buf) { return lds_raw + buf * IMG + KM * BCO * 2; };

  auto stage_op = [&](char* img, const bf16* g, int stride, int ch0,
                      int64_t mt, bool full, auto bc_tag) {
    constexpr int BC = decltype(bc_tag)::value;
    constexpr int LPR = BC / 8;
    constexpr int RPP = 64 / LPR;
    const char* base = (const char*)(g + mt * (int64_t)stride + ch0);
    if (full) {
#pragma unroll
      for (int pp = 0; pp < (KM / RPP) / 4; ++pp) {
        const int p = wave + pp * 4;
        const int row = p * RPP + lane / LPR;
        const int ch = (lane % LPR) ^ wg_swz<BC>(row);
        glds16((const bf16*)(base + (int64_t)row * stride * 2 + ch * 16),
               (bf16*)(img + p * 1024));
      }
    } else {
#pragma unroll
      for (int it = 0; it < (KM * LPR) / 256; ++it) {
        const int idx = (int)threadIdx.x + it * 256;
        const int row = idx / LPR;
        const int ch = (idx % LPR) ^ wg_swz<BC>(row);
        Vec<bf16, 8> v;
        if (mt + row < m_end) {
          v = vload<bf16, 8>(
              (const bf16*)(base + (int64_t)row * stride * 2 + ch * 16));
        } else {
#pragma unroll
          for (int j = 0; j < 8; ++j) v.v[j] = from_f32<bf16>(0.f);
        }
        vstore<bf16, 8>((bf16*)(img + idx * 16), v);
      }
    }
  };
  auto stage = [&](int buf, int s) {
    const int64_t mt = m_begin + (int64_t)s * KM;
    const bool full = s < nfull;
    stage_op(dy_img(buf), dy, N, n0, mt, full,
             std::integral_constant<int, BCO>{});
    stage_op(x_img(buf), x, K, k0, mt, full,
             std::integral_constant<int, BCI>{});
  };

  const int fg = lane >> 4, fq = (lane >> 2) & 3, fp = lane & 3;
  const int frow = 8 * fg + fq;
  int offa[FCO], offb[FCI];
#pragma unroll
  for (int mi = 0; mi < FCO; ++mi) {
    const int chunk16 = ((wave / WGI) * WCO + mi * 16) / 8 + (fp >> 1);
    offa[mi] = frow * (BCO * 2) + ((chunk16 ^ wg_swz<BCO>(frow)) << 4) +
               8 * (fp & 1);
  }
#pragma unroll
  for (int ni = 0; ni < FCI; ++ni) {
    const int chunk16 = ((wave % WGI) * WCI + ni * 16) / 8 + (fp >> 1);
    offb[ni] = frow * (BCI * 2) + ((chunk16 ^ wg_swz<BCI>(frow)) << 4) +
               8 * (fp & 1);
  }
  auto tr_frag = [&](const char* p, int rowb) {
    using lds_v4 = __attribute__((address_space(3))) bf16x4;
    const bf16x4 lo = __builtin_amdgcn_ds_read_tr16_b64_v4i16((lds_v4*)p);
    const bf16x4 hi =
        __builtin_amdgcn_ds_read_tr16_b64_v4i16((lds_v4*)(p + 4 * rowb));
    return __builtin_shufflevector(lo, hi, 0, 1, 2, 3, 4, 5, 6, 7);
  };

  f32x4 acc[FCO][FCI];
#pragma unroll
  for (int mi = 0; mi < FCO; ++mi)
#pragma unroll
    for (int ni = 0; ni < FCI; ++ni) acc[mi][ni] = f32x4{0.f, 0.f, 0.f, 0.f};

  stage(0, 0);
  for (int s = 0; s < nsteps; ++s) {
    __syncthreads();
    if (s + 1 < nsteps) stage((s + 1) & 1, s + 1);
    const char* da = dy_img(s & 1);
    const char* xa = x_img(s & 1);
#pragma unroll
    for (int ks = 0; ks < KM / 32; ++ks) {
      bf16x8 af[FCO], bfr[FCI];
#pragma unroll
      for (int mi = 0; mi < FCO; ++mi)
        af[mi] = tr_frag(da + ks * 32 * (BCO * 2) + offa[mi], BCO * 2);
#pragma unroll
      for (int ni = 0; ni < FCI; ++ni)
        bfr[ni] = tr_frag(xa + ks * 32 * (BCI * 2) + offb[ni], BCI * 2);
#pragma unroll
      for (int mi = 0; mi < FCO; ++mi)
#pragma unroll
        for (int ni = 0; ni < FCI; ++ni)
          acc[mi][ni] = __builtin_amdgcn_mfma_f32_16x16x32_bf16(
              af[mi], bfr[ni], acc[mi][ni], 0, 0, 0);
    }
  }

  float* o = out + (int64_t)split * N * K;
  const int wco = (wave / WGI) * WCO, wci = (wave % WGI) * WCI;
#pragma unroll
  for (int mi = 0; mi < FCO; ++mi)
#pragma unroll
    for (int ni = 0; ni < FCI; ++ni)
#pragma unroll
      for (int r = 0; r < 4; ++r) {
        const int co = n0 + wco + mi * 16 + (lane >> 4) * 4 + r;
        const int ci = k0 + wci + ni * 16 + (lane & 15);
        o[(int64_t)co * K + ci] = acc[mi][ni][r];
      }
}

__global__ __launch_bounds__(256) void wgrad_finalize_kernel(
    const float* __restrict__ slab, float* __restrict__ dW, int n4,
    int splits, int G, int per) {
  __shared__ f32x4 part[256];
  const int outs = 256 / G;
  const int g = threadIdx.x / outs, o = threadIdx.x % outs;
  const int i = blockIdx.x * outs + o;
  const f32x4* p = (const f32x4*)slab + i;
  const int z0 = g * per;
  const int z1 = z0 + per < splits ? z0 + per : splits;
  f32x4 s = f32x4{0.f, 0.f, 0.f, 0.f};
#pragma unroll 4
  for (int z = z0; z < z1; ++z) s += p[(int64_t)z * n4];
  if (G == 1) {
    ((f32x4*)dW)[i] = s;
    return;
  }
  part[threadIdx.x] = s;
  __syncthreads();
  if (g == 0) {
    for (int j = 1; j < G; ++j) s += part[j * outs + o];
    ((f32x4*)dW)[i] = s;
  }
}

}

std::vector<torch::Tensor> conv1x1_fwd(torch::Tensor a, torch::Tensor b,
                                       c10::optional<torch::Tensor> bias,
                                       c10::optional<torch::Tensor> scale,
                                       c10::optional<torch::Tensor> shift,
                                       c10::optional<torch::Tensor> residual,
                                       bool relu, bool want_stats) {
  DLA_CHECK_INPUT(a);
  DLA_CHECK_INPUT(b);
  TORCH_CHECK(a.scalar_type() == torch::kBFloat16 &&
                  b.scalar_type() == torch::kBFloat16,
              "conv1x1_fwd: bf16 only");
  const int64_t M = a.size(0);
  const int K = (int)a.size(1), N = (int)b.size(0);
  TORCH_CHECK((int)b.size(1) == K, "conv1x1_fwd: K mismatch");
  TORCH_CHECK(K % 64 == 0 && N % 64 == 0, "conv1x1_fwd: K,N must be %64");
  auto C = torch::empty({M, N}, a.options());
  auto opts_f = a.options().dtype(torch::kFloat);
  const int gx = (int)((M + 127) / 128);
  auto sums = want_stats ? torch::empty({gx, 2 * N}, opts_f)
                         : torch::empty({0}, opts_f);
  const dla::bf16* res_p =
      residual.has_value() ? (const dla::bf16*)residual->data_ptr() : nullptr;
  const float* bias_p = bias.has_value() ? bias->data_ptr<float>() : nullptr;
  const float* scale_p = scale.has_value() ? scale->data_ptr<float>() : nullptr;
  const float* shift_p = shift.has_value() ? shift->data_ptr<float>() : nullptr;
  float* sums_p = want_stats ? sums.data_ptr<float>() : nullptr;

  const int nk = K / 64;
  auto launch = [&](auto bntag, auto stag, auto bktag) {
    constexpr int BN = decltype(bntag)::value;
    constexpr bool ST = decltype(stag)::value;
    constexpr int BKT = decltype(bktag)::value;
    constexpr int NW = (BN == 256) ? 8 : 4;
    constexpr int WM = (BN == 64) ? 32 : 64;
    const int nbuf = K / BKT > 1 ? 2 : 1;
    const int lds_stage = (128 * BKT + BN * BKT) * 2 * nbuf;
    const int lds_ep = NW * (WM >= 64 ? WM / 2 : WM) * (64 + 8) * 2;
    const int lds_st = ST ? ((BN == 64) ? 4 : 2) * 2 * BN * 4 : 0;
    const int lds = std::max(std::max(lds_stage, lds_ep), lds_st);
    if (lds > 65536) {
      static bool done[2] = {false, false};
      if (!done[ST]) {
        (void)hipFuncSetAttribute(
            (const void*)&dla::conv1x1_nt_kernel<BN, ST, BKT>,
            hipFuncAttributeMaxDynamicSharedMemorySize, 163840);
        done[ST] = true;
      }
    }
    hipLaunchKernelGGL((dla::conv1x1_nt_kernel<BN, ST, BKT>), dim3(N / BN, gx),
                       dim3(NW * 64), lds, dla::stream(),
                       (const dla::bf16*)a.data_ptr(),
                       (const dla::bf16*)b.data_ptr(),
                       (dla::bf16*)C.data_ptr(), res_p, bias_p, scale_p,
                       shift_p, sums_p, M, K, N, relu);
  };
  static const bool bk32_force = []{
    const char* e = std::getenv("DLA_C1X1_BK32");
    return e != nullptr && e[0] == '1';
  }();
  static const bool ring_on = []{
    const char* e = std::getenv("DLA_C1X1_RING");
    return e != nullptr && e[0] == '1';
  }();
  const bool bk32 = bk32_force || nk == 2;
  auto launch_ring = [&](auto stag) {
    constexpr bool ST = decltype(stag)::value;
    constexpr int lds = 4 * (128 * 32 + 128 * 32) * 2;
    hipLaunchKernelGGL((dla::conv1x1_nt_kernel<128, ST, 32, 1, 4>),
                       dim3(N / 128, gx), dim3(256), lds, dla::stream(),
                       (const dla::bf16*)a.data_ptr(),
                       (const dla::bf16*)b.data_ptr(),
                       (dla::bf16*)C.data_ptr(), res_p, bias_p, scale_p,
                       shift_p, sums_p, M, K, N, relu);
  };
  auto pick = [&](auto bntag) {
    constexpr int BNv = decltype(bntag)::value;
    if (BNv == 128 && ring_on && K % 32 == 0 && K / 32 >= 4) {
      if (want_stats) launch_ring(std::true_type{});
      else launch_ring(std::false_type{});
      return;
    }
    if (BNv == 128 && bk32 && nk >= 2) {
      if (want_stats) launch(bntag, std::true_type{},
                             std::integral_constant<int, 32>{});
      else launch(bntag, std::false_type{}, std::integral_constant<int, 32>{});
      return;
    }
    if (want_stats) launch(bntag, std::true_type{},
                           std::integral_constant<int, 64>{});
    else launch(bntag, std::false_type{}, std::integral_constant<int, 64>{});
  };
  if (N % 256 == 0 && nk == 1) pick(std::integral_constant<int, 256>{});
  else if (N % 128 == 0) pick(std::integral_constant<int, 128>{});
  else pick(std::integral_constant<int, 64>{});
  HIP_CHECK_ERR();
  return {C, sums};
}

std::vector<torch::Tensor> conv3x3_fwd(torch::Tensor a, torch::Tensor w9,
                                       int64_t imgH, int64_t imgW,
                                       c10::optional<torch::Tensor> bias,
                                       c10::optional<torch::Tensor> scale,
                                       c10::optional<torch::Tensor> shift,
                                       c10::optional<torch::Tensor> residual,
                                       bool relu, bool want_stats) {
  DLA_CHECK_INPUT(a);
  DLA_CHECK_INPUT(w9);
  TORCH_CHECK(a.scalar_type() == torch::kBFloat16 &&
                  w9.scalar_type() == torch::kBFloat16,
              "conv3x3_fwd: bf16 only");
  const int64_t M = a.size(0);
  const int Cin = (int)a.size(1), N = (int)w9.size(0);
  const int K = 9 * Cin;
  TORCH_CHECK((int)w9.size(1) == K, "conv3x3_fwd: weight must be [Co, 9*Ci]");
  TORCH_CHECK(Cin % 64 == 0 && N % 64 == 0, "conv3x3_fwd: C must be %64");
  TORCH_CHECK(M % (imgH * imgW) == 0, "conv3x3_fwd: M != B*H*W");
  auto C = torch::empty({M, N}, a.options());
  auto opts_f = a.options().dtype(torch::kFloat);
  const int gx = (int)((M + 127) / 128);
  auto sums = want_stats ? torch::empty({gx, 2 * N}, opts_f)
                         : torch::empty({0}, opts_f);
  const dla::bf16* res_p =
      residual.has_value() ? (const dla::bf16*)residual->data_ptr() : nullptr;
  const float* bias_p = bias.has_value() ? bias->data_ptr<float>() : nullptr;
  const float* scale_p = scale.has_value() ? scale->data_ptr<float>() : nullptr;
  const float* shift_p = shift.has_value() ? shift->data_ptr<float>() : nullptr;
  float* sums_p = want_stats ? sums.data_ptr<float>() : nullptr;
  auto launch = [&](auto bntag, auto stag) {
    constexpr int BN = decltype(bntag)::value;
    constexpr bool ST = decltype(stag)::value;
    const int lds_stage = (128 * 64 + BN * 64) * 2 * 2;
    const int lds_ep = 4 * ((BN == 64) ? 32 : 64) / ((BN == 64) ? 1 : 2) *
                       (64 + 8) * 2;
    const int lds_st = ST ? ((BN == 64) ? 4 : 2) * 2 * BN * 4 : 0;
    const int lds = std::max(std::max(lds_stage, lds_ep), lds_st);
    hipLaunchKernelGGL((dla::conv1x1_nt_kernel<BN, ST, 64, 9>),
                       dim3(N / BN, gx), dim3(256), lds, dla::stream(),
                       (const dla::bf16*)a.data_ptr(),
                       (const dla::bf16*)w9.data_ptr(),
                       (dla::bf16*)C.data_ptr(), res_p, bias_p, scale_p,
                       shift_p, sums_p, M, K, N, relu, (int)imgH, (int)imgW);
  };
  auto pick = [&](auto bntag) {
    if (want_stats) launch(bntag, std::true_type{});
    else launch(bntag, std::false_type{});
  };
  if (N % 128 == 0) pick(std::integral_constant<int, 128>{});
  else pick(std::integral_constant<int, 64>{});
  HIP_CHECK_ERR();
  return {C, sums};
}

static torch::Tensor conv1x1_wgrad_v2(const torch::Tensor& dy,
                                      const torch::Tensor& x, int64_t M,
                                      int K, int N) {
  auto opts_f = x.options().dtype(torch::kFloat);
  if (M == 0) return torch::zeros({N, K}, opts_f);
  auto dW = torch::empty({N, K}, opts_f);
  auto launch = [&](auto cotag, auto citag) {
    constexpr int BCO = decltype(cotag)::value;
    constexpr int BCI = decltype(citag)::value;
    constexpr int lds = 2 * 64 * (BCO + BCI) * 2;
    constexpr int bpc = std::min(4, 163840 / lds);
    const int tiles = (N / BCO) * (K / BCI);
    int64_t s = std::max<int64_t>(1, (256 * bpc) / tiles);
    s = std::min<int64_t>(s, std::max<int64_t>(1, M / 256));
    s = std::min<int64_t>(
        s, std::max<int64_t>(1, M * (N + K) / (4 * (int64_t)N * K)));
    const int64_t chunk = (((M + s - 1) / s + 63) / 64) * 64;
    const int splits = (int)((M + chunk - 1) / chunk);
    const int total = tiles * splits;
    torch::Tensor slab;
    float* out = dW.data_ptr<float>();
    if (splits > 1) {
      slab = torch::empty({splits, N, K}, opts_f);
      out = slab.data_ptr<float>();
    }
    static_assert(lds <= 65536, "needs hipFuncSetAttribute above 64 KB");
    hipLaunchKernelGGL((dla::conv1x1_wgrad2_kernel<BCO, BCI>),
                       dim3(((total + 7) / 8) * 8), dim3(256), lds,
                       dla::stream(), (const dla::bf16*)dy.data_ptr(),
                       (const dla::bf16*)x.data_ptr(), out, M, K, N, chunk,
                       tiles, total);
    if (splits > 1) {
      const int n4 = N * K / 4;
      int G = 1;
      while (G < 64 && n4 * G < 65536 && splits >= 8 * G) G *= 2;
      hipLaunchKernelGGL(dla::wgrad_finalize_kernel, dim3(n4 / (256 / G)),
                         dim3(256), 0, dla::stream(), (const float*)out,
                         dW.data_ptr<float>(), n4, splits, G,
                         (splits + G - 1) / G);
    }
  };
  using std::integral_constant;
  const bool n128 = N % 128 == 0, k128 = K % 128 == 0;
  if (n128 && k128)
    launch(integral_constant<int, 128>{}, integral_constant<int, 128>{});
  else if (k128)
    launch(integral_constant<int, 64>{}, integral_constant<int, 128>{});
  else if (n128)
    launch(integral_constant<int, 128>{}, integral_constant<int, 64>{});
  else
    launch(integral_constant<int, 64>{}, integral_constant<int, 64>{});
  HIP_CHECK_ERR();
  return dW;
}

torch::Tensor conv1x1_wgrad(torch::Tensor dy, torch::Tensor x) {
  DLA_CHECK_INPUT(dy);
  DLA_CHECK_INPUT(x);
  TORCH_CHECK(dy.scalar_type() == torch::kBFloat16 &&
                  x.scalar_type() == torch::kBFloat16,
              "conv1x1_wgrad: bf16 only");
  const int64_t M = x.size(0);
  const int K = (int)x.size(1), N = (int)dy.size(1);
  TORCH_CHECK(dy.size(0) == M, "conv1x1_wgrad: M mismatch");
  TORCH_CHECK(K % 64 == 0 && N % 64 == 0, "conv1x1_wgrad: K,N must be %64");
  const char* v1 = std::getenv("DLA_C1X1_WGRAD_V1");
  if (v1 == nullptr || v1[0] != '1') return conv1x1_wgrad_v2(dy, x, M, K, N);
  auto dW = torch::zeros({N, K}, x.options().dtype(torch::kFloat));
  auto launch = [&](auto cotag, auto citag) {
    constexpr int BCO = decltype(cotag)::value;
    constexpr int BCI = decltype(citag)::value;
    const int tiles = (N / BCO) * (K / BCI);
    int splits = (int)std::min<int64_t>(
        std::max<int64_t>(1, 1024 / tiles),
        (M + 2047) / 2048);
    const int64_t chunk0 = (M + splits - 1) / splits;
    const int64_t chunk = ((chunk0 + 63) / 64) * 64;
    splits = (int)((M + chunk - 1) / chunk);
    const int lds = 2 * (BCO + BCI) * 72 * 2;
    if (lds > 65536) {
      static bool done = false;
      if (!done) {
        (void)hipFuncSetAttribute(
            (const void*)&dla::conv1x1_wgrad_kernel<BCO, BCI>,
            hipFuncAttributeMaxDynamicSharedMemorySize, 163840);
        done = true;
      }
    }
    hipLaunchKernelGGL((dla::conv1x1_wgrad_kernel<BCO, BCI>),
                       dim3(N / BCO, K / BCI, splits),
                       dim3(BCO * BCI >= 8192 ? 512 : 256), lds,
                       dla::stream(), (const dla::bf16*)dy.data_ptr(),
                       (const dla::bf16*)x.data_ptr(), dW.data_ptr<float>(),
                       M, K, N, chunk);
  };
  const bool n128 = N % 128 == 0, k128 = K % 128 == 0;
  if (n128 && k128)
    launch(std::integral_constant<int, 128>{}, std::integral_constant<int, 128>{});
  else if (k128)
    launch(std::integral_constant<int, 64>{}, std::integral_constant<int, 128>{});
  else if (n128)
    launch(std::integral_constant<int, 128>{}, std::integral_constant<int, 64>{});
  else
    launch(std::integral_constant<int, 64>{}, std::integral_constant<int, 64>{});
  HIP_CHECK_ERR();
  return dW;
}

torch::Tensor conv3x3_wgrad(torch::Tensor dy, torch::Tensor x, int64_t imgH,
                            int64_t imgW) {
  DLA_CHECK_INPUT(dy);
  DLA_CHECK_INPUT(x);
  TORCH_CHECK(dy.scalar_type() == torch::kBFloat16 &&
                  x.scalar_type() == torch::kBFloat16,
              "conv3x3_wgrad: bf16 only");
  const int64_t M = x.size(0);
  const int Cin = (int)x.size(1), N = (int)dy.size(1);
  const int K = 9 * Cin;
  TORCH_CHECK(dy.size(0) == M, "conv3x3_wgrad: M mismatch");
  TORCH_CHECK(Cin % 64 == 0 && N % 64 == 0, "conv3x3_wgrad: C must be %64");
  auto dW = torch::zeros({N, K}, x.options().dtype(torch::kFloat));
  auto launch = [&](auto cotag, auto citag) {
    constexpr int BCO = decltype(cotag)::value;
    constexpr int BCI = decltype(citag)::value;
    const int tiles = (N / BCO) * (3 * Cin / BCI);
    int splits = (int)std::min<int64_t>(
        std::max<int64_t>(1, 1024 / tiles),
        (M + 2047) / 2048);
    const int64_t chunk0 = (M + splits - 1) / splits;
    const int64_t chunk = ((chunk0 + 63) / 64) * 64;
    splits = (int)((M + chunk - 1) / chunk);
    const int lds = 2 * (BCO + BCI) * 72 * 2;
    if (lds > 65536) {
      static bool done = false;
      if (!done) {
        (void)hipFuncSetAttribute(
            (const void*)&dla::conv1x1_wgrad_kernel<BCO, BCI, 9>,
            hipFuncAttributeMaxDynamicSharedMemorySize, 163840);
        done = true;
      }
    }
    hipLaunchKernelGGL((dla::conv1x1_wgrad_kernel<BCO, BCI, 9>),
                       dim3(N / BCO, 3 * Cin / BCI, splits),
                       dim3(BCO * BCI >= 8192 ? 512 : 256), lds,
                       dla::stream(), (const dla::bf16*)dy.data_ptr(),
                       (const dla::bf16*)x.data_ptr(), dW.data_ptr<float>(),
                       M, K, N, chunk, (int)imgH, (int)imgW);
  };
  const bool n128 = N % 128 == 0, ci128 = Cin % 128 == 0;
  if (n128 && ci128)
    launch(std::integral_constant<int, 128>{}, std::integral_constant<int, 128>{});
  else if (ci128)
    launch(std::integral_constant<int, 64>{}, std::integral_constant<int, 128>{});
  else if (n128)
    launch(std::integral_constant<int, 128>{}, std::integral_constant<int, 64>{});
  else
    launch(std::integral_constant<int, 64>{}, std::integral_constant<int, 64>{});
  HIP_CHECK_ERR();
  return dW;
}
```

### deeplearning_amd/ops/batchnorm.py

```python
from __future__ import annotations

import os

import torch
import torch.nn as nn
import torch.nn.functional as F

from ._ext import dense, ext, use_hip


def _mask_from_y() -> bool:
    return os.environ.get("DLA_BN_MASK_FROM_Y", "0") == "1"


def save_bn_for_backward(ctx, x, y, weight, mean, rstd, scale, shift, relu):
    ctx.relu = relu
    ctx.mask_from_x = bool(relu and not _mask_from_y() and
                           ext().bn_relu_mask_from_x(x))
    if ctx.mask_from_x:
        ctx.save_for_backward(x, weight, mean, rstd, scale, shift)
    elif relu:
        ctx.save_for_backward(x, weight, mean, rstd, y)
    else:
        ctx.save_for_backward(x, weight, mean, rstd)


def bn_backward(ctx, dy):
    x, weight, mean, rstd, *rest = ctx.saved_tensors
    y = scale = shift = None
    if ctx.mask_from_x:
        scale, shift = rest
    elif ctx.relu:
        y, = rest
    return ext().batchnorm_bwd_ex(dy, x, y, weight, mean, rstd, scale, shift,
                                  ctx.relu)


class _BNFn(torch.autograd.Function):
    @staticmethod
    def forward(ctx, x, weight, bias, running_mean, running_var, momentum, eps, relu):
        x = dense(x)
        y, mean, rstd, scale, shift = ext().batchnorm_fwd(
            x, weight, bias, running_mean, running_var, momentum, eps, relu)
        save_bn_for_backward(ctx, x, y, weight, mean, rstd, scale, shift, relu)
        return y

    @staticmethod
    def backward(ctx, dy):
        dx, dw, db = bn_backward(ctx, dy)
        return dx, dw, db, None, None, None, None, None


class BatchNorm2d(nn.BatchNorm2d):

    def __init__(self, num_features, eps=1e-5, momentum=0.1, relu=False):
        super().__init__(num_features, eps=eps, momentum=momentum, affine=True,
                         track_running_stats=True)
        self.relu = relu

    def _eaf(self) -> float:
        if self.momentum is not None:
            return self.momentum
        if self.training and self.num_batches_tracked is not None:
            return 1.0 / float(max(int(self.num_batches_tracked), 1))
        return 0.0

    def forward(self, x):
        if not use_hip(x):
            if self.training and self.momentum is None and \
                    self.num_batches_tracked is not None:
                self.num_batches_tracked.add_(1)
            y = F.batch_norm(x, self.running_mean, self.running_var, self.weight,
                             self.bias, self.training, self._eaf(), self.eps)
            return torch.relu(y) if self.relu else y
        if self.running_mean.dtype != torch.float32:
            self.running_mean.data = self.running_mean.data.float()
            self.running_var.data = self.running_var.data.float()
        if self.training:
            if self.num_batches_tracked is not None:
                self.num_batches_tracked.add_(1)
            return _BNFn.apply(x, self.weight, self.bias, self.running_mean,
                               self.running_var, self._eaf(), self.eps,
                               self.relu)
        rstd = torch.rsqrt(self.running_var.float() + self.eps)
        scale = self.weight.float() * rstd
        shift = self.bias.float() - self.running_mean.float() * scale
        if torch.is_grad_enabled() and (x.requires_grad or self.weight.requires_grad):
            y = x * scale.reshape(1, -1, 1, 1).to(x.dtype) + shift.reshape(1, -1, 1, 1).to(x.dtype)
            return torch.relu(y) if self.relu else y
        return ext().bn_apply(dense(x), scale, shift, self.relu)


class FrozenBatchNorm2d(nn.Module):

    def __init__(self, num_features, eps=1e-5):
        super().__init__()
        self.eps = eps
        self.register_buffer("weight", torch.ones(num_features))
        self.register_buffer("bias", torch.zeros(num_features))
        self.register_buffer("running_mean", torch.zeros(num_features))
        self.register_buffer("running_var", torch.ones(num_features))

    def _load_from_state_dict(self, state_dict, prefix, *args, **kwargs):
        state_dict.pop(prefix + "num_batches_tracked", None)
        super()._load_from_state_dict(state_dict, prefix, *args, **kwargs)

    def forward(self, x):
        rstd = torch.rsqrt(self.running_var.float() + self.eps)
        scale = self.weight.float() * rstd
        shift = self.bias.float() - self.running_mean.float() * scale
        if use_hip(x) and not (torch.is_grad_enabled() and x.requires_grad):
            return ext().bn_apply(dense(x), scale, shift, False)
        sc = scale.reshape(1, -1, 1, 1).to(x.dtype)
        sh = shift.reshape(1, -1, 1, 1).to(x.dtype)
        return x * sc + sh
```

### deeplearning_amd/ops/conv1x1.py

```python
from __future__ import annotations

import os

import torch
import torch.nn.functional as F
from torch import nn

from ._ext import ext, use_hip
from .batchnorm import bn_backward, save_bn_for_backward


def _flatten_nhwc(x: torch.Tensor) -> torch.Tensor:
    B, C, H, W = x.shape
    return x.permute(0, 2, 3, 1).reshape(B * H * W, C)


def _unflatten_nhwc(y2d: torch.Tensor, B: int, H: int, W: int) -> torch.Tensor:
    return y2d.view(B, H, W, -1).permute(0, 3, 1, 2)


class _Conv1x1Fn(torch.autograd.Function):

    @staticmethod
    def forward(ctx, x2d, w, bias, scale, shift, residual, relu, want_stats,
                pass_input=False):
        xb = x2d if x2d.dtype == torch.bfloat16 else x2d.to(torch.bfloat16)
        wb = w if w.dtype == torch.bfloat16 else w.to(torch.bfloat16)
        wb = wb.contiguous()
        y2d, sums = ext().conv1x1_fwd(xb, wb, bias, scale, shift, residual,
                                      relu, want_stats)
        ctx.save_for_backward(xb, wb)
        ctx.x_dtype = x2d.dtype
        ctx.w_dtype = w.dtype
        ctx.pass_input = pass_input
        outs = (y2d,)
        if want_stats:
            ctx.mark_non_differentiable(sums)
            outs += (sums,)
        if pass_input:
            ctx.set_materialize_grads(False)
            outs += (x2d,)
        return outs if len(outs) > 1 else y2d

    @staticmethod
    def backward(ctx, dy2d, *rest):
        xb, wb = ctx.saved_tensors
        d_alias = rest[-1] if ctx.pass_input else None
        if d_alias is not None:
            d_alias = d_alias.contiguous()
        dx = dw = db = None
        if dy2d is None:
            if d_alias is not None and ctx.needs_input_grad[0]:
                dx = d_alias.to(ctx.x_dtype)
            return dx, None, None, None, None, None, None, None, None
        dy2d = dy2d.contiguous()
        if dy2d.dtype != torch.bfloat16:
            dy2d = dy2d.to(torch.bfloat16)
        if ctx.needs_input_grad[0]:
            wt = ext().transpose2d(wb)
            if d_alias is not None and d_alias.dtype != torch.bfloat16:
                d_alias = d_alias.to(torch.bfloat16)
            dx, _ = ext().conv1x1_fwd(dy2d, wt, None, None, None, d_alias,
                                      False, False)
            if dx.dtype != ctx.x_dtype:
                dx = dx.to(ctx.x_dtype)
        if ctx.needs_input_grad[1]:
            dw = ext().conv1x1_wgrad(dy2d, xb)
            if dw.dtype != ctx.w_dtype:
                dw = dw.to(ctx.w_dtype)
        if ctx.needs_input_grad[2]:
            db = dy2d.float().sum(0)
        return dx, dw, db, None, None, None, None, None, None


class _BNFromStatsFn(torch.autograd.Function):

    @staticmethod
    def forward(ctx, x, weight, bias, sums, running_mean, running_var,
                momentum, eps, relu):
        y, mean, rstd, scale, shift = ext().batchnorm_fwd_from_sums(
            x, weight, bias, sums, running_mean, running_var, momentum, eps,
            relu)
        save_bn_for_backward(ctx, x, y, weight, mean, rstd, scale, shift,
                             relu)
        return y

    @staticmethod
    def backward(ctx, dy):
        dx, dw, db = bn_backward(ctx, dy)
        return dx, dw, db, None, None, None, None, None, None


class _Stride2Fn(torch.autograd.Function):

    @staticmethod
    def forward(ctx, x):
        ctx.ihw = (x.shape[2], x.shape[3])
        return ext().stride2_gather(x)

    @staticmethod
    def backward(ctx, dy):
        if not dy.is_contiguous(memory_format=torch.channels_last):
            dy = dy.contiguous(memory_format=torch.channels_last)
        return ext().stride2_scatter(dy, *ctx.ihw)


def _conv1x1_disabled() -> bool:
    return os.environ.get("DLA_NO_CONV1X1", "0") == "1"


def can_fuse_conv1x1(x: torch.Tensor, conv: nn.Conv2d) -> bool:
    if _conv1x1_disabled() or not use_hip(x):
        return False
    if x.dtype != torch.bfloat16:
        return False
    if conv.kernel_size != (1, 1) or conv.groups != 1:
        return False
    if conv.padding != (0, 0) or conv.dilation != (1, 1):
        return False
    if conv.stride not in ((1, 1), (2, 2)):
        return False
    cin, cout = conv.in_channels, conv.out_channels
    if cin % 64 != 0 or cout % 64 != 0:
        return False
    return x.dim() == 4 and x.is_contiguous(memory_format=torch.channels_last)


def _prep(x: torch.Tensor, conv: nn.Conv2d):
    stride = conv.stride[0]
    if stride == 2:
        x = _Stride2Fn.apply(x)
    B, C, H, W = x.shape
    x2d = _flatten_nhwc(x)
    w2d = conv.weight.reshape(conv.weight.shape[0], conv.weight.shape[1])
    bias = conv.bias.float() if conv.bias is not None else None
    return x2d, w2d, bias, (B, H, W)


def conv1x1(x: torch.Tensor, conv: nn.Conv2d) -> torch.Tensor:
    x2d, wb, bias, (B, H, W) = _prep(x, conv)
    y2d = _Conv1x1Fn.apply(x2d, wb, bias, None, None, None, False, False)
    return _unflatten_nhwc(y2d, B, H, W)


def _fp32_running_stats(bn) -> None:
    if bn.running_mean.dtype != torch.float32:
        bn.running_mean.data = bn.running_mean.data.float()
        bn.running_var.data = bn.running_var.data.float()


def _conv1x1_train_stats(x: torch.Tensor, conv: nn.Conv2d, bn,
                         pass_input: bool = False):
    x2d, wb, bias, (B, H, W) = _prep(x, conv)
    _fp32_running_stats(bn)
    if bn.num_batches_tracked is not None:
        bn.num_batches_tracked.add_(1)
    momentum = bn._eaf() if hasattr(bn, "_eaf") else (bn.momentum or 0.0)
    outs = _Conv1x1Fn.apply(x2d, wb, bias, None, None, None, False, True,
                            pass_input)
    alias = _unflatten_nhwc(outs[2], B, H, W) if pass_input else None
    return _unflatten_nhwc(outs[0], B, H, W), outs[1], momentum, alias


def conv1x1_bn(x: torch.Tensor, conv: nn.Conv2d, bn,
               pass_input: bool = False):
    relu = bool(getattr(bn, "relu", False))
    if bn.training:
        y_raw, partials, momentum, alias = _conv1x1_train_stats(
            x, conv, bn, pass_input)
        y = _BNFromStatsFn.apply(y_raw, bn.weight, bn.bias, partials,
                                 bn.running_mean, bn.running_var, momentum,
                                 bn.eps, relu)
        return (y, alias) if pass_input else y
    if pass_input:
        raise ValueError("conv1x1_bn: pass_input needs train mode")

    x2d, wb, bias, (B, H, W) = _prep(x, conv)
    _fp32_running_stats(bn)

    if not bn.training:
        rstd = torch.rsqrt(bn.running_var + bn.eps)
        scale = bn.weight.float() * rstd
        shift = bn.bias.float() - bn.running_mean * scale
        if not (torch.is_grad_enabled() and
                (x.requires_grad or conv.weight.requires_grad or
                 bn.weight.requires_grad)):
            y2d, _ = ext().conv1x1_fwd(
                x2d.to(torch.bfloat16), wb.to(torch.bfloat16).contiguous(),
                bias, scale.contiguous(), shift.contiguous(), None, relu,
                False)
            return _unflatten_nhwc(y2d, B, H, W)
        y2d = _Conv1x1Fn.apply(x2d, wb, bias, None, None, None, False, False)
        y = _unflatten_nhwc(y2d, B, H, W)
        y = y * scale.reshape(1, -1, 1, 1).to(y.dtype) + \
            shift.reshape(1, -1, 1, 1).to(y.dtype)
        return torch.relu(y) if relu else y


class _BNJoinFn(torch.autograd.Function):

    @staticmethod
    def forward(ctx, x_raw, weight, bias, partials, running_mean,
                running_var, momentum, eps, identity):
        out, mean, rstd = ext().bn_add_relu_fwd_from_sums(
            x_raw, weight, bias, partials, running_mean, running_var,
            momentum, eps, identity)
        ctx.save_for_backward(x_raw, out, weight, mean, rstd)
        return out

    @staticmethod
    def backward(ctx, dy):
        x_raw, out, weight, mean, rstd = ctx.saved_tensors
        g, dx, dw, db = ext().bn_add_relu_bwd(dy, out, x_raw, weight, mean,
                                              rstd)
        return dx, dw, db, None, None, None, None, None, g


class _BNJoinDualFn(torch.autograd.Function):

    @staticmethod
    def forward(ctx, x_raw, weight, bias, partials, running_mean,
                running_var, momentum, eps, xd_raw, weight_d, bias_d,
                partials_d, running_mean_d, running_var_d, momentum_d, eps_d):
        out, mean, rstd, mean_d, rstd_d = \
            ext().bn_add_relu_dual_fwd_from_sums(
                x_raw, weight, bias, partials, running_mean, running_var,
                momentum, eps, xd_raw, weight_d, bias_d, partials_d,
                running_mean_d, running_var_d, momentum_d, eps_d)
        ctx.save_for_backward(x_raw, xd_raw, out, weight, mean, rstd,
                              weight_d, mean_d, rstd_d)
        return out

    @staticmethod
    def backward(ctx, dy):
        (x_raw, xd_raw, out, weight, mean, rstd, weight_d, mean_d,
         rstd_d) = ctx.saved_tensors
        dx, dxd, dw, db, dwd, dbd = ext().bn_add_relu_dual_bwd(
            dy, out, x_raw, weight, mean, rstd, xd_raw, weight_d, mean_d,
            rstd_d)
        return (dx, dw, db, None, None, None, None, None,
                dxd, dwd, dbd, None, None, None, None, None)


def _fused_join_disabled() -> bool:
    return os.environ.get("DLA_NO_FUSED_JOIN", "0") == "1"


def _join_bn_ok(conv: nn.Conv2d, bn) -> bool:
    from .batchnorm import BatchNorm2d

    return (type(bn) is BatchNorm2d and bn.training and
            not getattr(bn, "relu", False) and conv.bias is None)


def can_pass_input(x: torch.Tensor, conv: nn.Conv2d, bn) -> bool:
    from .batchnorm import BatchNorm2d

    return (not _fused_join_disabled() and can_fuse_conv1x1(x, conv) and
            conv.stride == (1, 1) and type(bn) is BatchNorm2d and
            bn.training and torch.is_grad_enabled() and x.requires_grad)


def can_fuse_join(x: torch.Tensor, conv: nn.Conv2d, bn, identity=None,
                  x_down=None, downsample=None) -> bool:
    if _fused_join_disabled() or not can_fuse_conv1x1(x, conv) or \
            not _join_bn_ok(conv, bn):
        return False
    if downsample is not None:
        if not (isinstance(downsample, nn.Sequential) and
                len(downsample) == 2 and
                isinstance(downsample[0], nn.Conv2d)):
            return False
        return (x_down is not None and
                can_fuse_conv1x1(x_down, downsample[0]) and
                _join_bn_ok(downsample[0], downsample[1]) and
                downsample[0].out_channels == conv.out_channels)
    return (identity is not None and use_hip(identity) and
            identity.dtype == torch.bfloat16 and identity.dim() == 4 and
            identity.is_contiguous(memory_format=torch.channels_last))


def conv_bn_add_relu(x: torch.Tensor, conv: nn.Conv2d, bn, identity=None,
                     x_down=None, downsample=None) -> torch.Tensor:
    if can_fuse_join(x, conv, bn, identity, x_down, downsample):
        y_raw, partials, momentum, _ = _conv1x1_train_stats(x, conv, bn)
        if downsample is None:
            if identity.shape != y_raw.shape:
                raise ValueError("conv_bn_add_relu: identity shape mismatch")
            return _BNJoinFn.apply(y_raw, bn.weight, bn.bias, partials,
                                   bn.running_mean, bn.running_var, momentum,
                                   bn.eps, identity)
        conv_d, bn_d = downsample[0], downsample[1]
        yd_raw, partials_d, momentum_d, _ = _conv1x1_train_stats(
            x_down, conv_d, bn_d)
        if yd_raw.shape != y_raw.shape:
            raise ValueError("conv_bn_add_relu: downsample shape mismatch")
        return _BNJoinDualFn.apply(
            y_raw, bn.weight, bn.bias, partials, bn.running_mean,
            bn.running_var, momentum, bn.eps, yd_raw, bn_d.weight, bn_d.bias,
            partials_d, bn_d.running_mean, bn_d.running_var, momentum_d,
            bn_d.eps)
    from .activations import add_relu

    out = conv_bn(x, conv, bn)
    if downsample is not None:
        if (isinstance(downsample, nn.Sequential) and len(downsample) == 2
                and isinstance(downsample[0], nn.Conv2d)):
            identity = conv_bn(x_down, downsample[0], downsample[1])
        else:
            identity = downsample(x_down)
    return add_relu(out, identity)


def conv_bn(x: torch.Tensor, conv: nn.Conv2d, bn) -> torch.Tensor:
    from .batchnorm import BatchNorm2d

    if isinstance(bn, BatchNorm2d):
        if can_fuse_conv1x1(x, conv):
            return conv1x1_bn(x, conv, bn)
        if can_fuse_conv3x3(x, conv):
            return conv3x3_bn(x, conv, bn)
    return bn(conv(x))


class _Conv3x3Fn(torch.autograd.Function):

    @staticmethod
    def forward(ctx, x4d, w, want_stats):
        B, C, H, W = x4d.shape
        xb = x4d if x4d.dtype == torch.bfloat16 else x4d.to(torch.bfloat16)
        wb = w if w.dtype == torch.bfloat16 else w.to(torch.bfloat16)
        a = _flatten_nhwc(xb)
        w9 = wb.permute(0, 2, 3, 1).reshape(w.shape[0], -1).contiguous()
        y2d, sums = ext().conv3x3_fwd(a, w9, H, W, None, None, None, None,
                                      False, want_stats)
        ctx.save_for_backward(xb, wb)
        ctx.w_dtype = w.dtype
        ctx.x_dtype = x4d.dtype
        y = _unflatten_nhwc(y2d, B, H, W)
        if want_stats:
            ctx.mark_non_differentiable(sums)
            return y, sums
        return y

    @staticmethod
    def backward(ctx, dy, *unused):
        xb, wb = ctx.saved_tensors
        B, C, H, W = xb.shape
        if not dy.is_contiguous(memory_format=torch.channels_last):
            dy = dy.contiguous(memory_format=torch.channels_last)
        if dy.dtype != torch.bfloat16:
            dy = dy.to(torch.bfloat16)
        dy2d = _flatten_nhwc(dy)
        dx = dw = None
        if ctx.needs_input_grad[0]:
            wd = wb.flip(2, 3).transpose(0, 1)
            wd9 = wd.permute(0, 2, 3, 1).reshape(C, -1).contiguous()
            dx2d, _ = ext().conv3x3_fwd(dy2d, wd9, H, W, None, None, None,
                                        None, False, False)
            dx = _unflatten_nhwc(dx2d, B, H, W)
            if dx.dtype != ctx.x_dtype:
                dx = dx.to(ctx.x_dtype)
        if ctx.needs_input_grad[1]:
            dw9 = ext().conv3x3_wgrad(dy2d, _flatten_nhwc(xb), H, W)
            dw = dw9.view(wb.shape[0], 3, 3, C).permute(0, 3, 1, 2)
            if dw.dtype != ctx.w_dtype:
                dw = dw.to(ctx.w_dtype)
            else:
                dw = dw.contiguous()
        return dx, dw, None


def _conv3x3_enabled() -> bool:
    return os.environ.get("DLA_CONV3X3", "0") == "1"


def can_fuse_conv3x3(x: torch.Tensor, conv: nn.Conv2d) -> bool:
    if _conv1x1_disabled() or not _conv3x3_enabled() or not use_hip(x):
        return False
    if x.dtype != torch.bfloat16:
        return False
    if conv.kernel_size != (3, 3) or conv.groups != 1:
        return False
    if conv.padding != (1, 1) or conv.dilation != (1, 1) or \
            conv.stride != (1, 1) or conv.bias is not None:
        return False
    if conv.in_channels % 64 != 0 or conv.out_channels % 64 != 0:
        return False
    return x.dim() == 4 and x.is_contiguous(memory_format=torch.channels_last)


def conv3x3_bn(x: torch.Tensor, conv: nn.Conv2d, bn) -> torch.Tensor:
    relu = bool(getattr(bn, "relu", False))
    B, C, H, W = x.shape
    if bn.running_mean.dtype != torch.float32:
        bn.running_mean.data = bn.running_mean.data.float()
        bn.running_var.data = bn.running_var.data.float()
    if not bn.training:
        rstd = torch.rsqrt(bn.running_var + bn.eps)
        scale = bn.weight.float() * rstd
        shift = bn.bias.float() - bn.running_mean * scale
        if not (torch.is_grad_enabled() and
                (x.requires_grad or conv.weight.requires_grad or
                 bn.weight.requires_grad)):
            xb = x.to(torch.bfloat16)
            wb = conv.weight.to(torch.bfloat16)
            w9 = wb.permute(0, 2, 3, 1).reshape(wb.shape[0], -1).contiguous()
            y2d, _ = ext().conv3x3_fwd(_flatten_nhwc(xb), w9, H, W, None,
                                       scale.contiguous(), shift.contiguous(),
                                       None, relu, False)
            return _unflatten_nhwc(y2d, B, H, W)
        y = _Conv3x3Fn.apply(x, conv.weight, False)
        y = y * scale.reshape(1, -1, 1, 1).to(y.dtype) + \
            shift.reshape(1, -1, 1, 1).to(y.dtype)
        return torch.relu(y) if relu else y
    if bn.num_batches_tracked is not None:
        bn.num_batches_tracked.add_(1)
    momentum = bn._eaf() if hasattr(bn, "_eaf") else (bn.momentum or 0.0)
    y_raw, partials = _Conv3x3Fn.apply(x, conv.weight, True)
    return _BNFromStatsFn.apply(y_raw, bn.weight, bn.bias, partials,
                                bn.running_mean, bn.running_var, momentum,
                                bn.eps, relu)
```

Measured before the change: 9656 images/s.

## Fuse BN backward stats reduction into the 1x1 dgrad GEMM epilogue

The 1x1 conv dgrad kernel gains an optional epilogue that applies the downstream ReLU/join mask, accumulates per-channel sum(g) and sum(g*xhat) partials into a slab, and writes the masked gradient. A link object connects the forward BN/ReLU node to the consuming conv, so the later BN backward can skip its own stats pass and only compute dx from the reduced slab. This removes a full read of dy/x for the BN backward reduction. The cost is extra epilogue loads, register pressure (waves_per_eu hint) and a hierarchical slab reduce for deep slabs.

```diff
diff --git a/csrc/batchnorm.hip b/csrc/batchnorm.hip
--- a/csrc/batchnorm.hip
+++ b/csrc/batchnorm.hip
@@ -3,9 +3,6 @@
 
 namespace dla {
 
-__device__ __forceinline__ float bn_pre(float x, float sc, float sh) {
-  return fmaf(x, sc, sh);
-}
 
 template <typename dev_t>
 __global__ void bn_stats_kernel(const dev_t* __restrict__ x, float* __restrict__ sums,
@@ -302,6 +299,32 @@
     __syncthreads();
   }
   if (rl == 0 && c < n_cols) sums[c] = ls[0][cl];
+}
+
+constexpr int kSlabGroup = 128;
+constexpr int kSlabDeep = kRedMaxParts;
+
+__global__ void __launch_bounds__(kSlabCols * kSlabRows)
+bn_slab_group_reduce_kernel(const float* __restrict__ slab, int n_parts,
+                            int n_cols, float* __restrict__ groups) {
+  __shared__ float ls[kSlabRows][kSlabCols + 1];
+  const int cl = threadIdx.x % kSlabCols, rl = threadIdx.x / kSlabCols;
+  const int c = blockIdx.x * kSlabCols + cl;
+  const int r0 = blockIdx.y * kSlabGroup;
+  const int r1 = r0 + kSlabGroup < n_parts ? r0 + kSlabGroup : n_parts;
+  float s = 0.f;
+  if (c < n_cols) {
+#pragma unroll 4
+    for (int r = r0 + rl; r < r1; r += kSlabRows)
+      s += slab[(int64_t)r * n_cols + c];
+  }
+  ls[rl][cl] = s;
+  __syncthreads();
+  for (int h = kSlabRows / 2; h > 0; h >>= 1) {
+    if (rl < h) ls[rl][cl] += ls[rl + h][cl];
+    __syncthreads();
+  }
+  if (rl == 0 && c < n_cols) groups[(int64_t)blockIdx.y * n_cols + c] = ls[0][cl];
 }
 
 template <typename dev_t, int V>
@@ -647,6 +670,16 @@
 
 inline torch::Tensor bn_slab_reduce_launch(const torch::Tensor& slab) {
   const int n_parts = (int)slab.size(0), n_cols = (int)slab.size(1);
+  if (n_parts > kSlabDeep) {
+    const int groups = (n_parts + kSlabGroup - 1) / kSlabGroup;
+    auto part = torch::empty({groups, n_cols}, slab.options());
+    hipLaunchKernelGGL(bn_slab_group_reduce_kernel,
+                       dim3((n_cols + kSlabCols - 1) / kSlabCols, groups),
+                       dim3(kSlabCols * kSlabRows), 0, stream(),
+                       slab.data_ptr<float>(), n_parts, n_cols,
+                       part.data_ptr<float>());
+    return bn_slab_reduce_launch(part);
+  }
   auto sums = torch::empty({n_cols}, slab.options());
   hipLaunchKernelGGL(bn_slab_reduce_kernel,
                      dim3((n_cols + kSlabCols - 1) / kSlabCols),
@@ -1163,6 +1196,100 @@
                        (dev_t*)dxd.data_ptr(), C, rows, used,
                        1.f / (float)rows);
   });
+  HIP_CHECK_ERR();
+  auto dbias = dla::bn_param_grad(sums, 0, C, weight);
+  return {dx, dxd, dla::bn_param_grad(sums, C, C, weight), dbias,
+          dla::bn_param_grad(sums, 2 * C, C, weight_d),
+          dbias.to(weight_d.scalar_type()).clone()};
+}
+
+namespace dla {
+
+inline void dx_only_check(const torch::Tensor& x, const torch::Tensor& g,
+                          const torch::Tensor& slab, int ns) {
+  TORCH_CHECK(is_nhwc_rows(x), "bn dx-only: x must be channels_last");
+  join_check(x, g, "g");
+  TORCH_CHECK(x.scalar_type() == torch::kBFloat16, "bn dx-only: bf16 only");
+  TORCH_CHECK(slab.is_cuda() && slab.scalar_type() == torch::kFloat &&
+                  slab.dim() == 2 && slab.is_contiguous() &&
+                  slab.size(0) >= 1 && slab.size(1) == ns * x.size(1),
+              "bn dx-only: slab must be fp32 [n_parts, ", ns, "*C]");
+}
+
+}
+
+torch::Tensor bn_slab_reduce(torch::Tensor slab) {
+  TORCH_CHECK(slab.is_cuda() && slab.scalar_type() == torch::kFloat &&
+                  slab.dim() == 2 && slab.is_contiguous() && slab.size(0) >= 1,
+              "bn_slab_reduce: slab must be a contiguous fp32 [n_parts, n_cols] "
+              "GPU tensor");
+  auto sums = dla::bn_slab_reduce_launch(slab);
+  HIP_CHECK_ERR();
+  return sums;
+}
+
+std::vector<torch::Tensor> bn_bwd_dx_from_slab(torch::Tensor g,
+                                               torch::Tensor slab,
+                                               torch::Tensor x,
+                                               torch::Tensor weight,
+                                               torch::Tensor mean,
+                                               torch::Tensor rstd) {
+  DLA_CHECK_CUDA(x);
+  dla::dx_only_check(x, g, slab, 2);
+  const int V = dla::join_vec(x);
+  const int C = (int)x.size(1);
+  const int64_t rows = x.numel() / C;
+  TORCH_CHECK(mean.numel() == C && rstd.numel() == C && weight.numel() == C,
+              "bn_bwd_dx_from_slab: per-channel tensors must have C elements");
+  auto dx = torch::empty_like(x);
+  auto w32 = weight.to(torch::kFloat).contiguous();
+  auto sums = dla::bn_slab_reduce_launch(slab);
+  using dev_t = __hip_bfloat16;
+  const int64_t used = dla::nhwc_used_threads(C / V, rows, 524288);
+  hipLaunchKernelGGL((dla::bn_bwd_dx_nhwc_kernel<dev_t, 8, false>),
+                     dim3((int)((used + 255) / 256)), dim3(256), 0,
+                     dla::stream(), (const dev_t*)g.data_ptr(),
+                     (const dev_t*)x.data_ptr(), nullptr, nullptr, nullptr,
+                     mean.data_ptr<float>(), rstd.data_ptr<float>(),
+                     w32.data_ptr<float>(), sums.data_ptr<float>(),
+                     (dev_t*)dx.data_ptr(), C, rows, used, 1.f / (float)rows);
+  HIP_CHECK_ERR();
+  return {dx, dla::bn_param_grad(sums, C, C, weight),
+          dla::bn_param_grad(sums, 0, C, weight)};
+}
+
+std::vector<torch::Tensor> bn_join_dual_bwd_dx_from_slab(
+    torch::Tensor g, torch::Tensor slab, torch::Tensor x, torch::Tensor weight,
+    torch::Tensor mean, torch::Tensor rstd, torch::Tensor xd,
+    torch::Tensor weight_d, torch::Tensor mean_d, torch::Tensor rstd_d) {
+  DLA_CHECK_CUDA(x);
+  dla::dx_only_check(x, g, slab, 3);
+  dla::join_check(x, xd, "xd");
+  const int V = dla::join_vec(x);
+  const int C = (int)x.size(1);
+  const int64_t rows = x.numel() / C;
+  TORCH_CHECK(mean.numel() == C && rstd.numel() == C && weight.numel() == C &&
+                  mean_d.numel() == C && rstd_d.numel() == C &&
+                  weight_d.numel() == C,
+              "bn_join_dual_bwd_dx_from_slab: per-channel tensors must have C "
+              "elements");
+  auto dx = torch::empty_like(x);
+  auto dxd = torch::empty_like(x);
+  auto w32 = weight.to(torch::kFloat).contiguous();
+  auto wd32 = weight_d.to(torch::kFloat).contiguous();
+  auto sums = dla::bn_slab_reduce_launch(slab);
+  using dev_t = __hip_bfloat16;
+  const int64_t used = dla::nhwc_used_threads(C / V, rows, 524288);
+  hipLaunchKernelGGL((dla::bn_join_bwd_dx_dual_nhwc_kernel<dev_t, 8>),
+                     dim3((int)((used + 255) / 256)), dim3(256), 0,
+                     dla::stream(), (const dev_t*)g.data_ptr(),
+                     (const dev_t*)x.data_ptr(), (const dev_t*)xd.data_ptr(),
+                     mean.data_ptr<float>(), rstd.data_ptr<float>(),
+                     w32.data_ptr<float>(), mean_d.data_ptr<float>(),
+                     rstd_d.data_ptr<float>(), wd32.data_ptr<float>(),
+                     sums.data_ptr<float>(), (dev_t*)dx.data_ptr(),
+                     (dev_t*)dxd.data_ptr(), C, rows, used,
+                     1.f / (float)rows);
   HIP_CHECK_ERR();
   auto dbias = dla::bn_param_grad(sums, 0, C, weight);
   return {dx, dxd, dla::bn_param_grad(sums, C, C, weight), dbias,
diff --git a/csrc/bindings.cpp b/csrc/bindings.cpp
--- a/csrc/bindings.cpp
+++ b/csrc/bindings.cpp
@@ -62,6 +62,23 @@
     torch::Tensor dy, torch::Tensor out, torch::Tensor x, torch::Tensor weight,
     torch::Tensor mean, torch::Tensor rstd, torch::Tensor xd,
     torch::Tensor weight_d, torch::Tensor mean_d, torch::Tensor rstd_d);
+torch::Tensor bn_slab_reduce(torch::Tensor slab);
+std::vector<torch::Tensor> bn_bwd_dx_from_slab(torch::Tensor g,
+                                               torch::Tensor slab,
+                                               torch::Tensor x,
+                                               torch::Tensor weight,
+                                               torch::Tensor mean,
+                                               torch::Tensor rstd);
+std::vector<torch::Tensor> bn_join_dual_bwd_dx_from_slab(
+    torch::Tensor g, torch::Tensor slab, torch::Tensor x, torch::Tensor weight,
+    torch::Tensor mean, torch::Tensor rstd, torch::Tensor xd,
+    torch::Tensor weight_d, torch::Tensor mean_d, torch::Tensor rstd_d);
+std::vector<torch::Tensor> conv1x1_dgrad_bwdstats(
+    torch::Tensor dy, torch::Tensor wt, c10::optional<torch::Tensor> residual,
+    int64_t mode, c10::optional<torch::Tensor> out, torch::Tensor x,
+    c10::optional<torch::Tensor> scale, c10::optional<torch::Tensor> shift,
+    torch::Tensor mean, torch::Tensor rstd, c10::optional<torch::Tensor> xd,
+    c10::optional<torch::Tensor> mean_d, c10::optional<torch::Tensor> rstd_d);
 std::vector<torch::Tensor> conv1x1_fwd(torch::Tensor a, torch::Tensor b,
                                        c10::optional<torch::Tensor> bias,
                                        c10::optional<torch::Tensor> scale,
@@ -161,6 +178,14 @@
         py::arg("bias") = py::none(), py::arg("scale") = py::none(),
         py::arg("shift") = py::none(), py::arg("residual") = py::none(),
         py::arg("relu") = false, py::arg("want_stats") = false);
+  m.def("conv1x1_dgrad_bwdstats", &conv1x1_dgrad_bwdstats, py::arg("dy"),
+        py::arg("wt"), py::arg("residual"), py::arg("mode"), py::arg("out"),
+        py::arg("x"), py::arg("scale"), py::arg("shift"), py::arg("mean"),
+        py::arg("rstd"), py::arg("xd") = py::none(),
+        py::arg("mean_d") = py::none(), py::arg("rstd_d") = py::none());
+  m.def("bn_slab_reduce", &bn_slab_reduce);
+  m.def("bn_bwd_dx_from_slab", &bn_bwd_dx_from_slab);
+  m.def("bn_join_dual_bwd_dx_from_slab", &bn_join_dual_bwd_dx_from_slab);
   m.def("conv1x1_wgrad", &conv1x1_wgrad);
   m.def("conv3x3_fwd", &conv3x3_fwd, py::arg("a"), py::arg("w9"),
         py::arg("imgH"), py::arg("imgW"), py::arg("bias") = py::none(),
diff --git a/csrc/common.h b/csrc/common.h
--- a/csrc/common.h
+++ b/csrc/common.h
@@ -53,6 +53,10 @@
 template <typename scalar_t> struct DevT { using type = scalar_t; };
 template <> struct DevT<at::BFloat16> { using type = __hip_bfloat16; };
 template <> struct DevT<at::Half> { using type = __half; };
+
+__device__ __forceinline__ float bn_pre(float x, float sc, float sh) {
+  return fmaf(x, sc, sh);
+}
 
 __device__ __forceinline__ float wave_reduce_sum(float v) {
 #pragma unroll
diff --git a/csrc/conv1x1.hip b/csrc/conv1x1.hip
--- a/csrc/conv1x1.hip
+++ b/csrc/conv1x1.hip
@@ -16,15 +16,36 @@
       (__attribute__((address_space(3))) unsigned int*)lds_dst, 16, 0, 0);
 }
 
-template <int BN, bool STATS, int BK = 64, int TAPS = 1, int RING = 0>
-__global__ __launch_bounds__((BN == 256) ? 512 : 256) void conv1x1_nt_kernel(
+enum BwdMode { BWD_NONE = 0, BWD_RELU_X = 1, BWD_JOIN = 2, BWD_JOIN_DUAL = 3 };
+
+struct BwdEpi {
+  const bf16* out;
+  const bf16* x;
+  const bf16* xd;
+  const float* scale;
+  const float* shift;
+  const float* mean;
+  const float* rstd;
+  const float* mean_d;
+  const float* rstd_d;
+  float* slab;
+};
+
+template <int BN, bool STATS, int BK = 64, int TAPS = 1, int RING = 0,
+          int BWD = BWD_NONE>
+__global__ __launch_bounds__((BN == 256) ? 512 : 256)
+__attribute__((amdgpu_waves_per_eu(BWD == BWD_NONE ? 1 : 3))) void
+conv1x1_nt_kernel(
     const bf16* __restrict__ A, const bf16* __restrict__ B,
     bf16* __restrict__ C, const bf16* __restrict__ residual,
     const float* __restrict__ bias,
     const float* __restrict__ scale,
     const float* __restrict__ shift,
     float* __restrict__ sums,
-    int64_t M, int K, int N, bool relu, int imgH = 0, int imgW = 0) {
+    int64_t M, int K, int N, bool relu, int imgH = 0, int imgW = 0,
+    BwdEpi be = BwdEpi{}) {
+  static_assert(BWD == BWD_NONE || (!STATS && TAPS == 1 && BN != 256),
+                "the backward-stats epilogue belongs to the 1x1 dgrad");
   constexpr int BM = 128;
   constexpr int NWAVES = (BN == 256) ? 8 : 4;
   constexpr int WAVES_M = (BN == 64) ? 4 : 2;
@@ -236,6 +257,26 @@
   for (int ni = 0; ni < NFR; ++ni)
     bcol[ni] = bias != nullptr ? bias[n0 + wn_off + ni * 16 + (lane & 15)]
                                : 0.f;
+  constexpr bool BDUAL = BWD == BWD_JOIN_DUAL;
+  constexpr int BNS = BWD == BWD_NONE ? 1 : (BDUAL ? 3 : 2);
+  float bacc[BNS][8], bmu[8], brs[8], bmud[8], brsd[8], bsc[8], bsh[8];
+  if constexpr (BWD != BWD_NONE) {
+#pragma unroll
+    for (int j = 0; j < 8; ++j) {
+      bmu[j] = be.mean[ng0 + j];
+      brs[j] = be.rstd[ng0 + j];
+      if constexpr (BDUAL) {
+        bmud[j] = be.mean_d[ng0 + j];
+        brsd[j] = be.rstd_d[ng0 + j];
+      }
+      if constexpr (BWD == BWD_RELU_X) {
+        bsc[j] = be.scale[ng0 + j];
+        bsh[j] = be.shift[ng0 + j];
+      }
+#pragma unroll
+      for (int s = 0; s < BNS; ++s) bacc[s][j] = 0.f;
+    }
+  }
 #pragma unroll
   for (int h = 0; h < EPC; ++h) {
 #pragma unroll
@@ -260,6 +301,12 @@
         Vec<bf16, 8> res;
         if (residual != nullptr)
           res = vload<bf16, 8>(residual + gm * N + ng0);
+        Vec<bf16, 8> bo, bx, bxd;
+        if constexpr (BWD == BWD_JOIN || BDUAL)
+          bo = vload<bf16, 8>(be.out + gm * N + ng0);
+        if constexpr (BWD != BWD_NONE)
+          bx = vload<bf16, 8>(be.x + gm * N + ng0);
+        if constexpr (BDUAL) bxd = vload<bf16, 8>(be.xd + gm * N + ng0);
         Vec<bf16, 8> out;
 #pragma unroll
         for (int j = 0; j < 8; ++j) {
@@ -268,11 +315,55 @@
           if (residual != nullptr) y += to_f32(res.v[j]);
           if (relu) y = fmaxf(y, 0.f);
           out.v[j] = from_f32<bf16>(y);
+          if constexpr (BWD != BWD_NONE) {
+            const float xf = to_f32(bx.v[j]);
+            const bool on = BWD == BWD_RELU_X
+                                ? bn_pre(xf, bsc[j], bsh[j]) > 0.f
+                                : to_f32(bo.v[j]) > 0.f;
+            if (!on) out.v[j] = from_f32<bf16>(0.f);
+            const float g = on ? to_f32(out.v[j]) : 0.f;
+            bacc[0][j] += g;
+            bacc[1][j] += g * ((xf - bmu[j]) * brs[j]);
+            if constexpr (BDUAL)
+              bacc[2][j] += g * ((to_f32(bxd.v[j]) - bmud[j]) * brsd[j]);
+          }
         }
         vstore<bf16, 8>(C + gm * N + ng0, out);
       }
     }
     if (h + 1 < EPC) __syncthreads();
+  }
+
+  if constexpr (BWD != BWD_NONE) {
+#pragma unroll
+    for (int s = 0; s < BNS; ++s)
+#pragma unroll
+      for (int j = 0; j < 8; ++j) {
+        float t = bacc[s][j];
+        t += __shfl_xor(t, 8, 64);
+        t += __shfl_xor(t, 16, 64);
+        t += __shfl_xor(t, 32, 64);
+        bacc[s][j] = t;
+      }
+    __syncthreads();
+    float* sbuf = (float*)lds_raw;
+    const int wm = wave / WAVES_N;
+    if (lane < 8) {
+#pragma unroll
+      for (int s = 0; s < BNS; ++s)
+#pragma unroll
+        for (int j = 0; j < 8; ++j)
+          sbuf[wm * (BNS * BN) + s * BN + wn_off + c0 + j] = bacc[s][j];
+    }
+    __syncthreads();
+    float* row = be.slab + (int64_t)blockIdx.y * (BNS * N);
+    for (int t = threadIdx.x; t < BNS * BN; t += NWAVES * 64) {
+      float tot = 0.f;
+#pragma unroll
+      for (int wmi = 0; wmi < WAVES_M; ++wmi)
+        tot += sbuf[wmi * (BNS * BN) + t];
+      row[(t / BN) * N + n0 + (t % BN)] = tot;
+    }
   }
 }
 
@@ -593,12 +684,11 @@
 
 }
 
-std::vector<torch::Tensor> conv1x1_fwd(torch::Tensor a, torch::Tensor b,
-                                       c10::optional<torch::Tensor> bias,
-                                       c10::optional<torch::Tensor> scale,
-                                       c10::optional<torch::Tensor> shift,
-                                       c10::optional<torch::Tensor> residual,
-                                       bool relu, bool want_stats) {
+static std::vector<torch::Tensor> conv1x1_run(
+    torch::Tensor a, torch::Tensor b, c10::optional<torch::Tensor> bias,
+    c10::optional<torch::Tensor> scale, c10::optional<torch::Tensor> shift,
+    c10::optional<torch::Tensor> residual, bool relu, bool want_stats,
+    int bwd, dla::BwdEpi be) {
   DLA_CHECK_INPUT(a);
   DLA_CHECK_INPUT(b);
   TORCH_CHECK(a.scalar_type() == torch::kBFloat16 &&
@@ -608,11 +698,17 @@
   const int K = (int)a.size(1), N = (int)b.size(0);
   TORCH_CHECK((int)b.size(1) == K, "conv1x1_fwd: K mismatch");
   TORCH_CHECK(K % 64 == 0 && N % 64 == 0, "conv1x1_fwd: K,N must be %64");
+  TORCH_CHECK(bwd == dla::BWD_NONE || !want_stats,
+              "conv1x1: forward and backward stats do not combine");
   auto C = torch::empty({M, N}, a.options());
   auto opts_f = a.options().dtype(torch::kFloat);
   const int gx = (int)((M + 127) / 128);
   auto sums = want_stats ? torch::empty({gx, 2 * N}, opts_f)
                          : torch::empty({0}, opts_f);
+  if (bwd != dla::BWD_NONE) {
+    sums = torch::empty({gx, (bwd == dla::BWD_JOIN_DUAL ? 3 : 2) * N}, opts_f);
+    be.slab = sums.data_ptr<float>();
+  }
   const dla::bf16* res_p =
       residual.has_value() ? (const dla::bf16*)residual->data_ptr() : nullptr;
   const float* bias_p = bias.has_value() ? bias->data_ptr<float>() : nullptr;
@@ -621,10 +717,11 @@
   float* sums_p = want_stats ? sums.data_ptr<float>() : nullptr;
 
   const int nk = K / 64;
-  auto launch = [&](auto bntag, auto stag, auto bktag) {
+  auto launch_mode = [&](auto bntag, auto stag, auto bktag, auto modetag) {
     constexpr int BN = decltype(bntag)::value;
     constexpr bool ST = decltype(stag)::value;
     constexpr int BKT = decltype(bktag)::value;
+    constexpr int MODE = decltype(modetag)::value;
     constexpr int NW = (BN == 256) ? 8 : 4;
     constexpr int WM = (BN == 64) ? 32 : 64;
     const int nbuf = K / BKT > 1 ? 2 : 1;
@@ -636,17 +733,41 @@
       static bool done[2] = {false, false};
       if (!done[ST]) {
         (void)hipFuncSetAttribute(
-            (const void*)&dla::conv1x1_nt_kernel<BN, ST, BKT>,
+            (const void*)&dla::conv1x1_nt_kernel<BN, ST, BKT, 1, 0, MODE>,
             hipFuncAttributeMaxDynamicSharedMemorySize, 163840);
         done[ST] = true;
       }
     }
-    hipLaunchKernelGGL((dla::conv1x1_nt_kernel<BN, ST, BKT>), dim3(N / BN, gx),
-                       dim3(NW * 64), lds, dla::stream(),
+    hipLaunchKernelGGL((dla::conv1x1_nt_kernel<BN, ST, BKT, 1, 0, MODE>),
+                       dim3(N / BN, gx), dim3(NW * 64), lds, dla::stream(),
                        (const dla::bf16*)a.data_ptr(),
                        (const dla::bf16*)b.data_ptr(),
                        (dla::bf16*)C.data_ptr(), res_p, bias_p, scale_p,
-                       shift_p, sums_p, M, K, N, relu);
+                       shift_p, sums_p, M, K, N, relu, 0, 0, be);
+  };
+  auto launch = [&](auto bntag, auto stag, auto bktag) {
+    using std::integral_constant;
+    if constexpr (decltype(stag)::value || decltype(bntag)::value == 256) {
+      launch_mode(bntag, stag, bktag, integral_constant<int, dla::BWD_NONE>{});
+    } else {
+      switch (bwd) {
+        case dla::BWD_RELU_X:
+          launch_mode(bntag, stag, bktag,
+                      integral_constant<int, dla::BWD_RELU_X>{});
+          break;
+        case dla::BWD_JOIN:
+          launch_mode(bntag, stag, bktag,
+                      integral_constant<int, dla::BWD_JOIN>{});
+          break;
+        case dla::BWD_JOIN_DUAL:
+          launch_mode(bntag, stag, bktag,
+                      integral_constant<int, dla::BWD_JOIN_DUAL>{});
+          break;
+        default:
+          launch_mode(bntag, stag, bktag,
+                      integral_constant<int, dla::BWD_NONE>{});
+      }
+    }
   };
   static const bool bk32_force = []{
     const char* e = std::getenv("DLA_C1X1_BK32");
@@ -669,7 +790,8 @@
   };
   auto pick = [&](auto bntag) {
     constexpr int BNv = decltype(bntag)::value;
-    if (BNv == 128 && ring_on && K % 32 == 0 && K / 32 >= 4) {
+    if (BNv == 128 && ring_on && bwd == dla::BWD_NONE && K % 32 == 0 &&
+        K / 32 >= 4) {
       if (want_stats) launch_ring(std::true_type{});
       else launch_ring(std::false_type{});
       return;
@@ -684,11 +806,75 @@
                            std::integral_constant<int, 64>{});
     else launch(bntag, std::false_type{}, std::integral_constant<int, 64>{});
   };
-  if (N % 256 == 0 && nk == 1) pick(std::integral_constant<int, 256>{});
+  if (N % 256 == 0 && nk == 1 && bwd == dla::BWD_NONE)
+    pick(std::integral_constant<int, 256>{});
   else if (N % 128 == 0) pick(std::integral_constant<int, 128>{});
   else pick(std::integral_constant<int, 64>{});
   HIP_CHECK_ERR();
   return {C, sums};
+}
+
+std::vector<torch::Tensor> conv1x1_fwd(torch::Tensor a, torch::Tensor b,
+                                       c10::optional<torch::Tensor> bias,
+                                       c10::optional<torch::Tensor> scale,
+                                       c10::optional<torch::Tensor> shift,
+                                       c10::optional<torch::Tensor> residual,
+                                       bool relu, bool want_stats) {
+  return conv1x1_run(a, b, bias, scale, shift, residual, relu, want_stats,
+                     dla::BWD_NONE, dla::BwdEpi{});
+}
+
+std::vector<torch::Tensor> conv1x1_dgrad_bwdstats(
+    torch::Tensor dy, torch::Tensor wt, c10::optional<torch::Tensor> residual,
+    int64_t mode, c10::optional<torch::Tensor> out, torch::Tensor x,
+    c10::optional<torch::Tensor> scale, c10::optional<torch::Tensor> shift,
+    torch::Tensor mean, torch::Tensor rstd, c10::optional<torch::Tensor> xd,
+    c10::optional<torch::Tensor> mean_d, c10::optional<torch::Tensor> rstd_d) {
+  TORCH_CHECK(mode >= dla::BWD_RELU_X && mode <= dla::BWD_JOIN_DUAL,
+              "conv1x1_dgrad_bwdstats: mode must be 1, 2 or 3");
+  const int64_t M = dy.size(0), N = wt.size(0);
+  auto rows_ok = [&](const torch::Tensor& t) {
+    return t.is_cuda() && t.scalar_type() == torch::kBFloat16 &&
+           t.numel() == M * N &&
+           (t.dim() == 2 ? t.is_contiguous() && t.size(1) == N
+                         : t.dim() == 4 && t.size(1) == N &&
+                               t.is_contiguous(at::MemoryFormat::ChannelsLast));
+  };
+  auto chan_ok = [&](const torch::Tensor& t) {
+    return t.is_cuda() && t.scalar_type() == torch::kFloat &&
+           t.is_contiguous() && t.numel() == N;
+  };
+  TORCH_CHECK(rows_ok(x), "conv1x1_dgrad_bwdstats: x must be [M,N] bf16 rows");
+  TORCH_CHECK(chan_ok(mean) && chan_ok(rstd),
+              "conv1x1_dgrad_bwdstats: mean/rstd must be fp32 [N]");
+  TORCH_CHECK(!residual.has_value() ||
+                  (rows_ok(*residual) && residual->dim() == 2),
+              "conv1x1_dgrad_bwdstats: residual must be [M,N] bf16");
+  dla::BwdEpi be{};
+  be.x = (const dla::bf16*)x.data_ptr();
+  be.mean = mean.data_ptr<float>();
+  be.rstd = rstd.data_ptr<float>();
+  if (mode == dla::BWD_RELU_X) {
+    TORCH_CHECK(scale.has_value() && shift.has_value() && chan_ok(*scale) &&
+                    chan_ok(*shift),
+                "conv1x1_dgrad_bwdstats: RELU_X needs fp32 [N] scale/shift");
+    be.scale = scale->data_ptr<float>();
+    be.shift = shift->data_ptr<float>();
+  } else {
+    TORCH_CHECK(out.has_value() && rows_ok(*out),
+                "conv1x1_dgrad_bwdstats: JOIN needs out as [M,N] bf16 rows");
+    be.out = (const dla::bf16*)out->data_ptr();
+  }
+  if (mode == dla::BWD_JOIN_DUAL) {
+    TORCH_CHECK(xd.has_value() && rows_ok(*xd) && mean_d.has_value() &&
+                    rstd_d.has_value() && chan_ok(*mean_d) && chan_ok(*rstd_d),
+                "conv1x1_dgrad_bwdstats: JOIN_DUAL needs xd, mean_d, rstd_d");
+    be.xd = (const dla::bf16*)xd->data_ptr();
+    be.mean_d = mean_d->data_ptr<float>();
+    be.rstd_d = rstd_d->data_ptr<float>();
+  }
+  return conv1x1_run(dy, wt, c10::nullopt, c10::nullopt, c10::nullopt,
+                     residual, false, false, (int)mode, be);
 }
 
 std::vector<torch::Tensor> conv3x3_fwd(torch::Tensor a, torch::Tensor w9,
diff --git a/deeplearning_amd/ops/batchnorm.py b/deeplearning_amd/ops/batchnorm.py
--- a/deeplearning_amd/ops/batchnorm.py
+++ b/deeplearning_amd/ops/batchnorm.py
@@ -25,8 +25,72 @@
         ctx.save_for_backward(x, weight, mean, rstd)
 
 
+RELU_X, JOIN, JOIN_DUAL = 1, 2, 3
+
+
+def bwd_stats_epilogue_disabled() -> bool:
+    return (os.environ.get("DLA_NO_BWD_STATS_EPILOGUE", "0") == "1" or
+            os.environ.get("DLA_NO_FUSED_JOIN", "0") == "1")
+
+
+class BwdStatsLink:
+
+    __slots__ = ("mode", "operands", "g", "slab", "g_version")
+
+    def __init__(self, mode, **operands):
+        self.mode = mode
+        self.operands = operands
+        self.g = self.slab = self.g_version = None
+
+    def take_operands(self):
+        ops, self.operands = self.operands, None
+        return ops
+
+    def offer(self, g, slab):
+        self.g, self.slab, self.g_version = g, slab, g._version
+
+    def claim(self, dy, like):
+        g, slab, version = self.g, self.slab, self.g_version
+        self.g = self.slab = self.g_version = None
+        if g is None or dy is None or not dy.is_cuda:
+            return None
+        same = (dy.dtype == g.dtype and dy.shape == like.shape and
+                dy.stride() == like.stride() and dy.storage_offset() == 0 and
+                dy.data_ptr() == g.data_ptr() and
+                dy.untyped_storage().data_ptr() ==
+                g.untyped_storage().data_ptr() and dy._version == version)
+        return slab if same else None
+
+
+def link_eligible(x) -> bool:
+    return (x.is_cuda and x.dtype == torch.bfloat16 and x.dim() == 4 and
+            x.shape[1] % 64 == 0 and
+            x.is_contiguous(memory_format=torch.channels_last))
+
+
+def relu_x_epilogue_enabled() -> bool:
+    return os.environ.get("DLA_BWD_STATS_RELU_X", "0") == "1"
+
+
+def attach_relu_link(y):
+    fn = y.grad_fn
+    if fn is None or not getattr(fn, "mask_from_x", False) or \
+            not relu_x_epilogue_enabled() or bwd_stats_epilogue_disabled():
+        return y
+    x, _, mean, rstd, scale, shift = fn.saved_tensors
+    if link_eligible(x):
+        fn.link = y._dla_bwd_link = BwdStatsLink(
+            RELU_X, x_raw=x, mean=mean, rstd=rstd, scale=scale, shift=shift)
+    return y
+
+
 def bn_backward(ctx, dy):
     x, weight, mean, rstd, *rest = ctx.saved_tensors
+    link = getattr(ctx, "link", None)
+    if link is not None:
+        slab = link.claim(dy, x)
+        if slab is not None:
+            return ext().bn_bwd_dx_from_slab(dy, slab, x, weight, mean, rstd)
     y = scale = shift = None
     if ctx.mask_from_x:
         scale, shift = rest
@@ -79,9 +143,10 @@
         if self.training:
             if self.num_batches_tracked is not None:
                 self.num_batches_tracked.add_(1)
-            return _BNFn.apply(x, self.weight, self.bias, self.running_mean,
-                               self.running_var, self._eaf(), self.eps,
-                               self.relu)
+            y = _BNFn.apply(x, self.weight, self.bias, self.running_mean,
+                            self.running_var, self._eaf(), self.eps,
+                            self.relu)
+            return attach_relu_link(y) if self.relu else y
         rstd = torch.rsqrt(self.running_var.float() + self.eps)
         scale = self.weight.float() * rstd
         shift = self.bias.float() - self.running_mean.float() * scale
diff --git a/deeplearning_amd/ops/conv1x1.py b/deeplearning_amd/ops/conv1x1.py
--- a/deeplearning_amd/ops/conv1x1.py
+++ b/deeplearning_amd/ops/conv1x1.py
@@ -7,7 +7,10 @@
 from torch import nn
 
 from ._ext import ext, use_hip
-from .batchnorm import bn_backward, save_bn_for_backward
+from .batchnorm import (JOIN, JOIN_DUAL, RELU_X, BwdStatsLink,
+                        attach_relu_link, bn_backward,
+                        bwd_stats_epilogue_disabled, link_eligible,
+                        save_bn_for_backward)
 
 
 def _flatten_nhwc(x: torch.Tensor) -> torch.Tensor:
@@ -23,8 +26,9 @@
 
     @staticmethod
     def forward(ctx, x2d, w, bias, scale, shift, residual, relu, want_stats,
-                pass_input=False):
+                pass_input=False, link=None):
         xb = x2d if x2d.dtype == torch.bfloat16 else x2d.to(torch.bfloat16)
+        ctx.link = link if xb is x2d else None
         wb = w if w.dtype == torch.bfloat16 else w.to(torch.bfloat16)
         wb = wb.contiguous()
         y2d, sums = ext().conv1x1_fwd(xb, wb, bias, scale, shift, residual,
@@ -52,7 +56,7 @@
         if dy2d is None:
             if d_alias is not None and ctx.needs_input_grad[0]:
                 dx = d_alias.to(ctx.x_dtype)
-            return dx, None, None, None, None, None, None, None, None
+            return dx, None, None, None, None, None, None, None, None, None
         dy2d = dy2d.contiguous()
         if dy2d.dtype != torch.bfloat16:
             dy2d = dy2d.to(torch.bfloat16)
@@ -60,8 +64,20 @@
             wt = ext().transpose2d(wb)
             if d_alias is not None and d_alias.dtype != torch.bfloat16:
                 d_alias = d_alias.to(torch.bfloat16)
-            dx, _ = ext().conv1x1_fwd(dy2d, wt, None, None, None, d_alias,
-                                      False, False)
+            link = ctx.link
+            ops = link.take_operands() if link is not None else None
+            if ops is not None and ops["x_raw"].numel() == xb.numel() and \
+                    ops["x_raw"].shape[1] == xb.shape[1]:
+                dx, slab = ext().conv1x1_dgrad_bwdstats(
+                    dy2d, wt, d_alias, link.mode,
+                    None if link.mode == RELU_X else xb, ops["x_raw"],
+                    ops.get("scale"), ops.get("shift"), ops["mean"],
+                    ops["rstd"], ops.get("xd_raw"), ops.get("mean_d"),
+                    ops.get("rstd_d"))
+                link.offer(dx, slab)
+            else:
+                dx, _ = ext().conv1x1_fwd(dy2d, wt, None, None, None,
+                                          d_alias, False, False)
             if dx.dtype != ctx.x_dtype:
                 dx = dx.to(ctx.x_dtype)
         if ctx.needs_input_grad[1]:
@@ -70,7 +86,7 @@
                 dw = dw.to(ctx.w_dtype)
         if ctx.needs_input_grad[2]:
             db = dy2d.float().sum(0)
-        return dx, dw, db, None, None, None, None, None, None
+        return dx, dw, db, None, None, None, None, None, None, None
 
 
 class _BNFromStatsFn(torch.autograd.Function):
@@ -151,13 +167,19 @@
 
 def _conv1x1_train_stats(x: torch.Tensor, conv: nn.Conv2d, bn,
                          pass_input: bool = False):
+    link = getattr(x, "_dla_bwd_link", None)
+    if link is not None and (
+            bwd_stats_epilogue_disabled() or conv.stride != (1, 1) or
+            x.dtype != torch.bfloat16 or
+            (link.mode != RELU_X and not pass_input)):
+        link = None
     x2d, wb, bias, (B, H, W) = _prep(x, conv)
     _fp32_running_stats(bn)
     if bn.num_batches_tracked is not None:
         bn.num_batches_tracked.add_(1)
     momentum = bn._eaf() if hasattr(bn, "_eaf") else (bn.momentum or 0.0)
     outs = _Conv1x1Fn.apply(x2d, wb, bias, None, None, None, False, True,
-                            pass_input)
+                            pass_input, link)
     alias = _unflatten_nhwc(outs[2], B, H, W) if pass_input else None
     return _unflatten_nhwc(outs[0], B, H, W), outs[1], momentum, alias
 
@@ -171,6 +193,8 @@
         y = _BNFromStatsFn.apply(y_raw, bn.weight, bn.bias, partials,
                                  bn.running_mean, bn.running_var, momentum,
                                  bn.eps, relu)
+        if relu:
+            attach_relu_link(y)
         return (y, alias) if pass_input else y
     if pass_input:
         raise ValueError("conv1x1_bn: pass_input needs train mode")
@@ -211,8 +235,15 @@
     @staticmethod
     def backward(ctx, dy):
         x_raw, out, weight, mean, rstd = ctx.saved_tensors
-        g, dx, dw, db = ext().bn_add_relu_bwd(dy, out, x_raw, weight, mean,
-                                              rstd)
+        link = getattr(ctx, "link", None)
+        slab = link.claim(dy, out) if link is not None else None
+        if slab is not None:
+            g = dy
+            dx, dw, db = ext().bn_bwd_dx_from_slab(g, slab, x_raw, weight,
+                                                   mean, rstd)
+        else:
+            g, dx, dw, db = ext().bn_add_relu_bwd(dy, out, x_raw, weight,
+                                                  mean, rstd)
         return dx, dw, db, None, None, None, None, None, g
 
 
@@ -235,15 +266,46 @@
     def backward(ctx, dy):
         (x_raw, xd_raw, out, weight, mean, rstd, weight_d, mean_d,
          rstd_d) = ctx.saved_tensors
-        dx, dxd, dw, db, dwd, dbd = ext().bn_add_relu_dual_bwd(
-            dy, out, x_raw, weight, mean, rstd, xd_raw, weight_d, mean_d,
-            rstd_d)
+        link = getattr(ctx, "link", None)
+        slab = link.claim(dy, out) if link is not None else None
+        if slab is not None:
+            dx, dxd, dw, db, dwd, dbd = \
+                ext().bn_join_dual_bwd_dx_from_slab(
+                    dy, slab, x_raw, weight, mean, rstd, xd_raw, weight_d,
+                    mean_d, rstd_d)
+        else:
+            dx, dxd, dw, db, dwd, dbd = ext().bn_add_relu_dual_bwd(
+                dy, out, x_raw, weight, mean, rstd, xd_raw, weight_d,
+                mean_d, rstd_d)
         return (dx, dw, db, None, None, None, None, None,
                 dxd, dwd, dbd, None, None, None, None, None)
 
 
 def _fused_join_disabled() -> bool:
     return os.environ.get("DLA_NO_FUSED_JOIN", "0") == "1"
+
+
+def _dual_epilogue_disabled() -> bool:
+    return os.environ.get("DLA_NO_BWD_STATS_DUAL", "0") == "1"
+
+
+def _attach_join_link(out: torch.Tensor) -> torch.Tensor:
+    fn = out.grad_fn
+    if fn is None or bwd_stats_epilogue_disabled():
+        return out
+    saved = fn.saved_tensors
+    if len(saved) == 5:
+        x_raw, _, _, mean, rstd = saved
+        if link_eligible(x_raw):
+            fn.link = out._dla_bwd_link = BwdStatsLink(
+                JOIN, x_raw=x_raw, mean=mean, rstd=rstd)
+    elif not _dual_epilogue_disabled():
+        x_raw, xd_raw, _, _, mean, rstd, _, mean_d, rstd_d = saved
+        if link_eligible(x_raw):
+            fn.link = out._dla_bwd_link = BwdStatsLink(
+                JOIN_DUAL, x_raw=x_raw, mean=mean, rstd=rstd, xd_raw=xd_raw,
+                mean_d=mean_d, rstd_d=rstd_d)
+    return out
 
 
 def _join_bn_ok(conv: nn.Conv2d, bn) -> bool:
@@ -287,19 +349,19 @@
         if downsample is None:
             if identity.shape != y_raw.shape:
                 raise ValueError("conv_bn_add_relu: identity shape mismatch")
-            return _BNJoinFn.apply(y_raw, bn.weight, bn.bias, partials,
-                                   bn.running_mean, bn.running_var, momentum,
-                                   bn.eps, identity)
+            return _attach_join_link(_BNJoinFn.apply(
+                y_raw, bn.weight, bn.bias, partials, bn.running_mean,
+                bn.running_var, momentum, bn.eps, identity))
         conv_d, bn_d = downsample[0], downsample[1]
         yd_raw, partials_d, momentum_d, _ = _conv1x1_train_stats(
             x_down, conv_d, bn_d)
         if yd_raw.shape != y_raw.shape:
             raise ValueError("conv_bn_add_relu: downsample shape mismatch")
-        return _BNJoinDualFn.apply(
+        return _attach_join_link(_BNJoinDualFn.apply(
             y_raw, bn.weight, bn.bias, partials, bn.running_mean,
             bn.running_var, momentum, bn.eps, yd_raw, bn_d.weight, bn_d.bias,
             partials_d, bn_d.running_mean, bn_d.running_var, momentum_d,
-            bn_d.eps)
+            bn_d.eps))
     from .activations import add_relu
 
     out = conv_bn(x, conv, bn)
```

Result: faster. 9928 images/s (median of 6 runs) (+2.8%).
